# andreaskoepf/faster-rcnn.torch

Hardware: AMD Instinct MI355X
Metric: images/sec (vgg_small 800x450 fwd+bwd) (higher is better)
Workload: dtype f32 (conv / Linear(13824,1024) operands as 2 x fp16 split planes: 22 significand bits, 3 MFMA partial products; fp32 accumulate)

## Files before the change

### faster-rcnn.torch_amd/_lib.py

```python
import ctypes as C
import os

_HERE = os.path.dirname(os.path.abspath(__file__))
SO_PATH = os.environ.get("FRCNN_LIB_PATH") or os.path.join(_HERE, "libfrcnn_hip.so")

KC_NAMES = ["conv_igemm_k3", "conv_igemm_other", "conv_wgrad_k3", "conv_wgrad_other", "gemm", "elemwise",
            "roi", "rpn", "nms", "optim", "image", "conv_x3", "conv_wgradx", "topk"]


class FrcnnError(RuntimeError):
    pass


class ModelDesc(C.Structure):
    _fields_ = [
        ("nblocks", C.c_int),
        ("filters", C.c_int * 8), ("ksize", C.c_int * 8), ("pad", C.c_int * 8), ("conv_steps", C.c_int * 8),
        ("dropout", C.c_float * 8),
        ("nheads", C.c_int),
        ("head_k", C.c_int * 8), ("head_n", C.c_int * 8), ("head_input", C.c_int * 8),
        ("ncls", C.c_int),
        ("cls_n", C.c_int * 8), ("cls_bn", C.c_int * 8),
        ("cls_dropout", C.c_float * 8),
        ("class_count", C.c_int),
        ("kh", C.c_int), ("kw", C.c_int),
    ]


vp = C.c_void_p
_SIGS = {
    "frcnn_version": ([], C.c_int),
    "frcnn_set_option": ([C.c_char_p, C.c_int], C.c_int),
    "frcnn_get_option": ([C.c_char_p, C.POINTER(C.c_int)], C.c_int),
    "frcnn_last_error": ([], C.c_char_p),
    "frcnn_device_count": ([C.POINTER(C.c_int)], C.c_int),
    "frcnn_set_device": ([C.c_int], C.c_int),
    "frcnn_device_name": ([C.c_char_p, C.c_int], C.c_int),
    "frcnn_malloc": ([C.POINTER(vp), C.c_size_t], C.c_int),
    "frcnn_free": ([vp], C.c_int),
    "frcnn_host_alloc": ([C.POINTER(vp), C.c_size_t], C.c_int),
    "frcnn_host_free": ([vp], C.c_int),
    "frcnn_memcpy_h2d": ([vp, vp, C.c_size_t, vp], C.c_int),
    "frcnn_memcpy_d2h": ([vp, vp, C.c_size_t, vp], C.c_int),
    "frcnn_memcpy_d2d": ([vp, vp, C.c_size_t, vp], C.c_int),
    "frcnn_stream_sync": ([vp], C.c_int),
    "frcnn_zero": ([vp, C.c_size_t, vp], C.c_int),
    "frcnn_scale": ([vp, C.c_longlong, C.c_float, vp], C.c_int),
    "frcnn_add": ([vp, vp, C.c_longlong, vp], C.c_int),
    "frcnn_prof_enable": ([C.c_int], C.c_int),
    "frcnn_prof_collect": ([vp, vp, vp, vp], C.c_int),
    "frcnn_nms_workspace_bytes": ([C.c_int], C.c_size_t),
    "frcnn_nms_device": ([vp, C.c_int, C.c_int, C.c_float, C.c_int, C.c_int, vp, vp, vp, C.c_size_t, vp], C.c_int),
    "frcnn_nms_device_classes": ([vp, C.c_int, C.c_int, C.c_float, C.c_int, C.c_int, vp, vp, vp, vp, C.c_size_t, vp], C.c_int),
    "frcnn_nms_device_n": ([vp, C.c_int, vp, C.c_int, C.c_float, C.c_int, C.c_int, vp, vp, vp, vp, C.c_size_t, vp], C.c_int),
    "frcnn_nms_batch_workspace_bytes": ([C.c_int, C.c_int], C.c_size_t),
    "frcnn_nms_device_batch": ([vp, C.c_int, C.c_longlong, C.c_int, vp, C.c_int, C.c_float, C.c_int, C.c_int, vp, vp, vp, vp, C.c_size_t,
                               vp], C.c_int),
    "frcnn_topk_select_workspace_bytes": ([C.c_int, C.c_int], C.c_size_t),
    "frcnn_topk_select": ([vp, C.c_int, C.c_longlong, C.c_int, vp, C.c_int, vp, C.c_longlong, vp, vp, C.c_size_t, vp], C.c_int),
    "frcnn_rpn_gather_rows": ([vp, vp, vp, vp, C.c_int, C.c_longlong, C.c_int, vp, C.c_longlong, vp, C.c_int, vp, vp, vp, vp, vp, vp,
                              C.c_longlong, vp], C.c_int),
    "frcnn_detect_gather_batch": ([vp, vp, C.c_int, C.c_int, vp, vp, vp, vp, vp, C.c_longlong, vp, vp, vp, vp, vp], C.c_int),
    "frcnn_roi_windows": ([vp, vp, C.c_int, vp, C.c_int, C.c_int, C.c_int, vp, vp], C.c_int),
    "frcnn_detect_post": ([vp, vp, vp, vp, vp, C.c_int, C.c_int, C.c_double, vp, vp, vp, vp, vp, vp], C.c_int),
    "frcnn_detect_gather": ([vp, vp, C.c_int, vp, vp, vp, vp, vp, vp, vp, vp, vp, vp], C.c_int),
    "frcnn_nms_host": ([vp, C.c_int, C.c_int, C.c_float, C.c_int, C.c_int, vp, vp], C.c_int),
    "frcnn_conv2d_forward": ([vp, C.c_int, C.c_int, C.c_int, vp, vp, vp, vp, C.c_int, C.c_int, C.c_int, vp, vp], C.c_int),
    "frcnn_conv2d_backward_input": ([vp, C.c_int, C.c_int, C.c_int, vp, C.c_int, C.c_int, C.c_int, vp, C.c_int, vp], C.c_int),
    "frcnn_conv2d_backward_weight": ([vp, C.c_int, C.c_int, C.c_int, vp, vp, vp, C.c_int, C.c_int, C.c_int, vp, vp, vp], C.c_int),
    "frcnn_maxpool_act_forward": ([vp, C.c_int, C.c_int, C.c_int, vp, vp, vp, vp, vp], C.c_int),
    "frcnn_maxpool_act_backward": ([vp, vp, vp, C.c_int, C.c_int, C.c_int, vp, vp, vp, vp, vp, vp], C.c_int),
    "frcnn_act_forward": ([vp, C.c_int, C.c_longlong, vp, vp, vp, vp], C.c_int),
    "frcnn_act_backward": ([vp, vp, C.c_int, C.c_longlong, vp, vp, vp, vp, vp, vp], C.c_int),
    "frcnn_roi_pool_forward": ([vp, C.c_int, C.c_int, C.c_int, vp, C.c_int, C.c_int, C.c_int, vp, vp, vp], C.c_int),
    "frcnn_roi_pool_backward": ([vp, C.c_int, C.c_int, C.c_int, vp, vp, C.c_int, C.c_int, C.c_int, vp], C.c_int),
    "frcnn_roi_align_forward": ([vp, C.c_int, C.c_int, C.c_int, vp, vp, C.c_int, C.c_double, C.c_double, C.c_int, C.c_int, C.c_int, vp,
                                 vp], C.c_int),
    "frcnn_roi_align_backward": ([vp, C.c_int, C.c_int, C.c_int, vp, vp, vp, C.c_int, C.c_double, C.c_double, C.c_int, C.c_int, C.c_int,
                                  vp], C.c_int),
    "frcnn_rpn_scan_workspace_bytes": ([vp, vp], C.c_size_t),
    "frcnn_rpn_scan": ([vp, vp, vp, vp, vp, C.c_double, C.c_double, C.c_double, C.c_int, vp, vp, vp, vp, vp, vp, C.c_size_t, vp], C.c_int),
    "frcnn_rpn_scan_batch_workspace_bytes": ([vp, vp, C.c_int], C.c_size_t),
    "frcnn_rpn_scan_batch": ([vp, vp, vp, C.c_int, C.c_longlong, vp, vp, C.c_double, C.c_double, C.c_double, C.c_int, vp, vp, vp, vp, vp,
                             vp, C.c_size_t, vp], C.c_int),
    "frcnn_rpn_loss": ([vp, vp, vp, vp, vp, vp, vp, vp, C.c_int, C.c_int, C.c_int, vp, vp, vp, vp], C.c_int),
    "frcnn_loss_accumulate": ([vp, C.c_int, vp, vp], C.c_int),
    "frcnn_linear_forward": ([vp, C.c_int, C.c_int, vp, vp, C.c_int, vp, vp], C.c_int),
    "frcnn_linear_backward": ([vp, vp, C.c_int, C.c_int, vp, C.c_int, vp, vp, vp, vp], C.c_int),
    "frcnn_rmsprop": ([vp, vp, vp, C.c_longlong, C.c_float, C.c_float, C.c_float, vp], C.c_int),
    "frcnn_scale_rmsprop": ([vp, vp, C.c_float, vp, C.c_longlong, C.c_float, C.c_float, C.c_float, vp], C.c_int),
    "frcnn_scale_rmsprop_dev": ([vp, vp, vp, vp, C.c_longlong, C.c_float, C.c_float, C.c_float, vp], C.c_int),
    "frcnn_scale_rmsprop_slice": ([vp, vp, C.c_float, vp, C.c_longlong, C.c_longlong, C.c_float, C.c_float, C.c_float, vp], C.c_int),
    "frcnn_sgd": ([vp, vp, vp, C.c_longlong, C.c_float, vp, C.c_float, C.c_float, C.c_float, C.c_float, C.c_int, C.c_int, vp], C.c_int),
    "frcnn_sgd_slice": ([vp, vp, vp, C.c_longlong, C.c_longlong, C.c_float, C.c_float, C.c_float, C.c_float, C.c_float, C.c_int, C.c_int,
                         vp], C.c_int),
    "frcnn_nag": ([vp, vp, vp, C.c_longlong, C.c_float, vp, C.c_float, C.c_float, C.c_float, C.c_int, vp], C.c_int),
    "frcnn_nag_slice": ([vp, vp, vp, C.c_longlong, C.c_longlong, C.c_float, C.c_float, C.c_float, C.c_float, C.c_int, vp], C.c_int),
    "frcnn_scale_rmsprop_slice_dev": ([vp, vp, vp, vp, C.c_longlong, C.c_longlong, C.c_float, C.c_float, C.c_float, vp], C.c_int),
    "frcnn_sgd_slice_dev": ([vp, vp, vp, C.c_longlong, C.c_longlong, vp, C.c_float, C.c_float, C.c_float, C.c_float, C.c_int, C.c_int,
                            vp], C.c_int),
    "frcnn_nag_slice_dev": ([vp, vp, vp, C.c_longlong, C.c_longlong, vp, C.c_float, C.c_float, C.c_float, C.c_int, vp], C.c_int),
    "frcnn_grad_clip_workspace_bytes": ([C.c_longlong], C.c_size_t),
    "frcnn_grad_clip": ([vp, C.c_longlong, vp, C.c_int, C.c_double, vp, C.c_double, vp, vp, C.c_size_t, vp], C.c_int),
    "frcnn_nag_lookahead": ([vp, vp, C.c_longlong, C.c_float, vp], C.c_int),
    "frcnn_nag_lookahead_slice": ([vp, vp, C.c_longlong, C.c_longlong, C.c_float, vp], C.c_int),
    "frcnn_model_update_stream": ([vp, C.POINTER(vp)], C.c_int),
    "frcnn_model_update_fork": ([vp, vp], C.c_int),
    "frcnn_model_update_join": ([vp, vp], C.c_int),
    "frcnn_pnet_wait_backward_begun": ([vp, vp], C.c_int),
    "frcnn_pnet_wait_heads_done": ([vp, vp], C.c_int),
    "frcnn_pnet_wait_block_done": ([vp, C.c_int, vp], C.c_int),
    "frcnn_pnet_refresh_packs": ([vp, vp, C.c_int, vp], C.c_int),
    "frcnn_pnet_invalidate_packs": ([vp], C.c_int),
    "frcnn_model_create": ([C.POINTER(ModelDesc), C.POINTER(vp)], C.c_int),
    "frcnn_model_destroy": ([vp], C.c_int),
    "frcnn_model_param_count": ([vp, C.POINTER(C.c_longlong), C.POINTER(C.c_longlong)], C.c_int),
    "frcnn_model_param_table": ([vp, vp, C.c_int, C.POINTER(C.c_int)], C.c_int),
    "frcnn_model_localizer_layers": ([vp, C.c_int, vp, C.c_int, C.POINTER(C.c_int)], C.c_int),
    "frcnn_model_set_trainable": ([vp, C.c_int, C.c_int, C.c_int], C.c_int),
    "frcnn_model_get_trainable": ([vp, C.POINTER(C.c_int), C.POINTER(C.c_int), C.POINTER(C.c_int)], C.c_int),
    "frcnn_model_debug_buffer": ([vp, C.c_int, C.c_int, C.POINTER(vp), C.POINTER(C.c_longlong)], C.c_int),
    "frcnn_pnet_forward": ([vp, vp, vp, C.c_int, C.c_int, C.c_int, vp, C.c_ulonglong, vp], C.c_int),
    "frcnn_pnet_forward_async_heads": ([vp, vp, vp, C.c_int, C.c_int, vp, C.c_ulonglong, vp], C.c_int),
    "frcnn_pnet_output": ([vp, C.c_int, C.POINTER(vp), C.POINTER(C.c_int), C.POINTER(C.c_int), C.POINTER(C.c_int)], C.c_int),
    "frcnn_pnet_delta": ([vp, C.c_int, C.POINTER(vp)], C.c_int),
    "frcnn_pnet_set_sparse_deltas": ([vp, C.c_int, vp, C.c_int], C.c_int),
    "frcnn_pnet_zero_deltas": ([vp, vp], C.c_int),
    "frcnn_pnet_backward_heads_begin": ([vp, vp, vp, vp], C.c_int),
    "frcnn_pnet_anchor_loss_begin": ([vp, vp, vp, vp, vp, vp, vp, C.c_int, C.c_int, C.c_int, vp, vp, vp, vp, vp], C.c_int),
    "frcnn_pnet_anchor_loss_wait": ([vp, vp], C.c_int),
    "frcnn_pnet_backward_heads_join": ([vp, vp, C.POINTER(C.c_int)], C.c_int),
    "frcnn_pnet_backward": ([vp, vp, vp, vp], C.c_int),
    "frcnn_pnet_wait_block_gradients": ([vp, C.c_int, vp], C.c_int),
    "frcnn_cnet_forward": ([vp, vp, vp, C.c_int, C.c_int, vp, C.c_ulonglong, vp, vp, vp, vp], C.c_int),
    "frcnn_cnet_backward": ([vp, vp, vp, vp, vp, vp, vp], C.c_int),
    "frcnn_cnet_backward_join": ([vp, vp], C.c_int),
    "frcnn_cnet_losses": ([vp, vp, vp, vp, C.c_int, C.c_int, C.c_int, vp, vp, vp, vp], C.c_int),
    "frcnn_cnet_decode": ([vp, C.c_int, C.c_int, vp, vp, vp], C.c_int),
    "frcnn_anchors_create": ([vp, vp, vp, vp, C.c_int, C.c_int, C.POINTER(vp)], C.c_int),
    "frcnn_anchors_destroy": ([vp], C.c_int),
    "frcnn_anchors_assemble": ([vp, vp, C.c_int, C.c_double, C.c_double, C.c_double, C.c_double, C.c_int, C.c_int, C.c_int, vp,
                               C.POINTER(C.c_int), vp, vp, C.c_int, C.POINTER(C.c_int), C.POINTER(C.c_int)], C.c_int),
    "frcnn_comm_get_unique_id": ([vp], C.c_int),
    "frcnn_comm_exchange_id_file": ([C.c_char_p, C.c_int, vp, C.c_int], C.c_int),
    "frcnn_comm_init_rank": ([C.POINTER(vp), C.c_int, C.c_int, vp], C.c_int),
    "frcnn_comm_init_rank_timeout": ([C.POINTER(vp), C.c_int, C.c_int, vp, C.c_int], C.c_int),
    "frcnn_comm_init_rank_file": ([C.POINTER(vp), C.c_int, C.c_int, C.c_char_p, C.c_int], C.c_int),
    "frcnn_comm_destroy": ([vp], C.c_int),
    "frcnn_comm_info": ([vp, C.POINTER(C.c_int), C.POINTER(C.c_int)], C.c_int),
    "frcnn_comm_query": ([vp, C.POINTER(C.c_int), C.POINTER(C.c_int), C.POINTER(C.c_int)], C.c_int),
    "frcnn_allreduce_f32": ([vp, vp, C.c_longlong, vp], C.c_int),
    "frcnn_allreduce_f64": ([vp, vp, C.c_longlong, vp], C.c_int),
    "frcnn_broadcast_f32": ([vp, vp, C.c_longlong, C.c_int, vp], C.c_int),
    "frcnn_image_rgb2yuv": ([vp, vp, C.c_int, C.c_int, vp], C.c_int),
    "frcnn_image_rgb2hsv": ([vp, vp, C.c_int, C.c_int, vp], C.c_int),
    "frcnn_image_rgb2lab": ([vp, vp, C.c_int, C.c_int, vp], C.c_int),
    "frcnn_image_scale": ([vp, C.c_int, C.c_int, C.c_int, vp, C.c_int, C.c_int, vp, C.c_int, vp], C.c_int),
    "frcnn_image_scale_u8": ([vp, C.c_int, C.c_int, vp, C.c_int, C.c_int, vp, C.c_int, vp], C.c_int),
    "frcnn_image_crop_flip": ([vp, C.c_int, C.c_int, C.c_int, C.c_int, C.c_int, C.c_int, C.c_int, C.c_int, C.c_int, vp, vp], C.c_int),
    "frcnn_image_normalize_workspace_bytes": ([C.c_int], C.c_size_t),
    "frcnn_image_normalize": ([vp, C.c_int, C.c_int, C.c_int, C.c_int, C.c_int, vp, C.c_size_t, vp], C.c_int),
    "frcnn_image_contrastive_norm": ([vp, C.c_int, C.c_int, vp, C.c_int, C.c_float, vp, vp, vp], C.c_int),
}

_lib = None


def exported_symbols():
    return sorted(_SIGS.keys())


def load():
    global _lib
    if _lib is not None:
        return _lib
    if not os.path.exists(SO_PATH):
        raise FrcnnError(
            "libfrcnn_hip.so not found at %s -- build it with `python -c 'import __graft_entry__ as g; g.build()'` "
            "(there is no CPU fallback for the product path)" % SO_PATH)
    try:
        import torch
    except ImportError:
        pass
    L = C.CDLL(SO_PATH)
    for name, (args, res) in _SIGS.items():
        fn = getattr(L, name)
        fn.argtypes = args
        fn.restype = res
    _lib = L
    return L


def check(rc):
    if rc != 0:
        raise FrcnnError("libfrcnn_hip: %s (code %d)" % (load().frcnn_last_error().decode("utf-8", "replace"), rc))


def call(name, *args):
    check(getattr(load(), name)(*args))
```

### faster-rcnn.torch_amd/csrc/amax.h

```cpp
#pragma once
#include <hip/hip_runtime.h>

#include "kernels.h"

namespace frcnn {

__device__ __forceinline__ void amax_store_block(float m, float* rec) {
  __shared__ float amax_part[16];
#pragma unroll
  for (int o = 32; o > 0; o >>= 1) m = fmaxf(m, __shfl_xor(m, o));
  if ((threadIdx.x & 63) == 0) amax_part[threadIdx.x >> 6] = m;
  __syncthreads();
  if (threadIdx.x == 0) {
    const int nw = (blockDim.x + 63) >> 6;
    for (int i = 1; i < nw; ++i) m = fmaxf(m, amax_part[i]);
    rec[1 + blockIdx.x] = m;
    if (blockIdx.x == 0) rec[0] = __builtin_bit_cast(float, (int)gridDim.x);
  }
}

__device__ __forceinline__ float amax_load_block(const float* __restrict__ rec) {
  __shared__ float amax_all[16];
  const int n = __builtin_bit_cast(int, rec[0]);
  float m = 0.f;
  for (int i = threadIdx.x; i < n; i += blockDim.x) m = fmaxf(m, rec[1 + i]);
#pragma unroll
  for (int o = 32; o > 0; o >>= 1) m = fmaxf(m, __shfl_xor(m, o));
  if ((threadIdx.x & 63) == 0) amax_all[threadIdx.x >> 6] = m;
  __syncthreads();
  const int nw = (blockDim.x + 63) >> 6;
  m = amax_all[0];
  for (int i = 1; i < nw; ++i) m = fmaxf(m, amax_all[i]);
  __syncthreads();
  return m;
}

}
```

### faster-rcnn.torch_amd/csrc/api.cpp

```cpp
#include <cmath>
#include <cstring>
#include <vector>
#include <mutex>

#include "kernels.h"

namespace frcnn {

static thread_local std::string g_err;

void set_error(const char* fmt, ...) {
  char buf[1024];
  va_list ap;
  va_start(ap, fmt);
  vsnprintf(buf, sizeof(buf), fmt, ap);
  va_end(ap);
  g_err = buf;
}

struct ProfRec { int klass; double flops, bytes; hipEvent_t a, b; hipStream_t s; };
static hipEvent_t g_prof_base = nullptr;
static unsigned g_prof_mask = 0;
static std::vector<ProfRec> g_recs;
static std::vector<hipEvent_t> g_pool;
// ... 241 lines not shown
  (void)hipFree(wf);
  return rc;
}
int frcnn_conv2d_backward_input(const float* gout, int O, int Ho, int Wo, const float* weight, int C, int k,
                                int pad, float* gin, int accumulate, void* stream) {
  float* wd = nullptr;
  if (conv_x3_eligible(O, C, k)) {
    FR_HIP(hipMalloc((void**)&wd, conv_x3_pack_bytes(O, C, k)));
    float* am = nullptr;
    int rcx = x3_f16_records(&am);
    float* const amw = am ? am + AMAX_REC : nullptr;
    float* const aws = am ? am + 2 * AMAX_REC : nullptr;
    if (am && rcx == FRCNN_OK) {
      rcx = tensor_absmax(gout, (long)O * Ho * Wo, am, S(stream));
      if (rcx == FRCNN_OK) rcx = tensor_absmax(weight, (long)O * C * k * k, amw, S(stream));
    }
    if (rcx == FRCNN_OK) rcx = conv_x3_pack(weight, O, C, k, 1, wd, S(stream), Ho + 2 * (k - 1 - pad) - k + 1, Wo + 2 * (k - 1 - pad) - k + 1, amw, aws);
    if (rcx == FRCNN_OK) rcx = conv_x3(gout, O, Ho, Wo, nullptr, nullptr, wd, nullptr, C, k, k - 1 - pad, gin, accumulate ? OUT_ADD : OUT_STORE, 0, S(stream), 0, nullptr, am, aws);
    (void)hipStreamSynchronize(S(stream));
    (void)hipFree(wd); (void)hipFree(am);
    return rcx;
  }
  FR_HIP(hipMalloc((void**)&wd, conv_pack_floats(O, C, k) * 4));
  int rc = conv_pack_weights(weight, O, C, k, nullptr, wd, S(stream));
  if (rc == FRCNN_OK)
    rc = conv_igemm(gout, O, Ho, Wo, nullptr, nullptr, wd, nullptr, C, k, k - 1 - pad, gin,
                    accumulate ? OUT_ADD : OUT_STORE, 0, S(stream));
  (void)hipStreamSynchronize(S(stream));
  (void)hipFree(wd);
  return rc;
}
int frcnn_conv2d_backward_weight(const float* in, int C, int H, int W, const float* in_slope,
                                 const float* in_scale, const float* gout, int O, int k, int pad,
                                 float* gweight, float* gbias, void* stream) {
  size_t wsb = conv_wgrad_workspace_bytes(C, H, W, O, k, pad);
  void* ws = nullptr;
  FR_HIP(hipMalloc(&ws, wsb));
  int rc = FRCNN_OK;
  float* am = nullptr;
  bool unit = true;
  rc = scale_fits_f16_form(in_scale, C, S(stream), &unit);
  if (rc == FRCNN_OK && unit && k == 3 && conv_wgradx_eligible(C, O, k)) rc = x3_f16_records(&am);
  if (am && rc == FRCNN_OK) {
    rc = tensor_absmax(in, (long)C * H * W, am, S(stream));
    if (rc == FRCNN_OK) rc = tensor_absmax(gout, (long)O * (H + 2 * pad - k + 1) * (W + 2 * pad - k + 1), am + AMAX_REC, S(stream));
  }
  if (rc == FRCNN_OK)
    rc = conv_wgrad(in, C, H, W, in_slope, in_scale, gout, O, k, pad, gweight, ws, wsb, S(stream), nullptr, am, am ? am + AMAX_REC : nullptr);
  (void)hipStreamSynchronize(S(stream));
  (void)hipFree(ws); (void)hipFree(am);
  FR_TRY(rc);
  if (gbias) {
    int Ho = H + 2 * pad - k + 1, Wo = W + 2 * pad - k + 1;
    FR_TRY(channel_sum(gout, O, (long)Ho * Wo, gbias, S(stream)));
  }
  return FRCNN_OK;
}

int frcnn_maxpool_act_forward(const float* x, int C, int H, int W, const float* slope, const float* scale,
                              float* out, unsigned char* idx, void* stream) {
  return maxpool_act_forward(x, C, H, W, slope, scale, out, idx, S(stream));
}
int frcnn_maxpool_act_backward(const float* gpool, const unsigned char* idx, const float* x, int C, int H, int W,
                               const float* slope, const float* scale, float* gx, float* gbias, float* gslope,
                               void* stream) {
  return maxpool_act_backward(gpool, idx, x, C, H, W, slope, scale, gx, gbias, gslope, S(stream));
}
int frcnn_act_forward(const float* x, int C, long long hw, const float* slope, const float* scale, float* y,
                      void* stream) {
  return act_forward(x, C, hw, slope, scale, y, S(stream));
}
int frcnn_act_backward(const float* gy, const float* x, int C, long long hw, const float* slope,
                       const float* scale, float* gx, float* gbias, float* gslope, void* stream) {
  return act_backward(gy, x, C, hw, slope, scale, gx, gbias, gslope, S(stream));
}

int frcnn_roi_pool_forward(const float* fmap, int C, int H, int W, const int* wins, int R, int kh, int kw,
                           float* out, int* idx, void* stream) {
  return roi_pool_forward(fmap, C, H, W, wins, R, kh, kw, out, idx, S(stream));
}
int frcnn_roi_pool_backward(float* gmap, int C, int H, int W, const float* gout, const int* idx, int R, int kh,
                            int kw, void* stream) {
  return roi_pool_backward(gmap, C, H, W, gout, idx, R, kh, kw, S(stream));
}

static int roi_align_check(const char* who, const void* map, int C, int H, int W, const void* rows, const double* rect, int kh, int kw,
                           int g) {
  FR_CHECK(map && rows && rect, "%s: NULL argument", who);
  FR_CHECK(C >= 1 && H >= 1 && W >= 1 && kh >= 1 && kw >= 1, "%s: map %d x %d x %d, grid %d x %d", who, C, H, W, kh, kw);
  FR_CHECK((long)H * W < (1L << 31), "%s: a plane of %d x %d cells", who, H, W);
  FR_CHECK(g >= 1 && g <= 4, "%s: sampling ratio %d outside 1..4", who, g);
  return FRCNN_OK;
}
int frcnn_roi_align_forward(const float* fmap, int C, int H, int W, const double* rect, const long long* pick, int R, double inv_sx,
                            double inv_sy, int kh, int kw, int g, float* out, void* stream) {
  if (R <= 0) return FRCNN_OK;
  FR_TRY(roi_align_check("frcnn_roi_align_forward", fmap, C, H, W, out, rect, kh, kw, g));
  return roi_align_forward(fmap, C, H, W, rect, pick, R, inv_sx, inv_sy, kh, kw, g, out, S(stream));
}
int frcnn_roi_align_backward(float* gmap, int C, int H, int W, const float* gout, const double* rect, const long long* pick, int R,
                             double inv_sx, double inv_sy, int kh, int kw, int g, void* stream) {
  if (R <= 0) return FRCNN_OK;
  FR_TRY(roi_align_check("frcnn_roi_align_backward", gmap, C, H, W, gout, rect, kh, kw, g));
  return roi_align_backward(gmap, C, H, W, gout, rect, pick, R, inv_sx, inv_sy, kh, kw, g, S(stream));
}

static void to_layers(const float* const* maps, const int* H, const int* W, RpnLayers* L) {
  for (int l = 0; l < 4; ++l) { L->map[l] = maps ? maps[l] : nullptr; L->H[l] = H[l]; L->W[l] = W[l]; }
}
size_t frcnn_rpn_scan_workspace_bytes(const int* H, const int* W) {
  RpnLayers L;
  to_layers(nullptr, H, W, &L);
  return rpn_scan_workspace_bytes(L);
}
int frcnn_rpn_scan(const float* const* maps, const int* H, const int* W, const float* anchor_w,
                   const float* anchor_h, double img_w, double img_h, double p_threshold, int cap,
                   float* match_p, int* match_idx, double* match_rect, float* match_box, int* count,
                   void* ws, size_t ws_bytes, void* stream) {
  RpnLayers L;
  to_layers(maps, H, W, &L);
  return rpn_scan(L, anchor_w, anchor_h, img_w, img_h, p_threshold, cap, match_p, match_idx, match_rect,
                  match_box, count, ws, ws_bytes, S(stream));
}
size_t frcnn_rpn_scan_batch_workspace_bytes(const int* H, const int* W, int B) {
  RpnLayers L;
  to_layers(nullptr, H, W, &L);
  return rpn_scan_batch_workspace_bytes(L, B);
}
int frcnn_rpn_scan_batch(const float* const* maps, const int* H, const int* W, int B, long long slot_stride, const float* anchor_w,
                         const float* anchor_h, double img_w, double img_h, double p_threshold, int cap, float* match_p,
                         int* match_idx, double* match_rect, float* match_box, int* count, void* ws, size_t ws_bytes,
                         void* stream) {
  FR_CHECK(maps && H && W, "frcnn_rpn_scan_batch: NULL argument");
  RpnLayers L;
  to_layers(maps, H, W, &L);
  return rpn_scan_batch(L, B, (long)slot_stride, anchor_w, anchor_h, img_w, img_h, p_threshold, cap, match_p, match_idx,
                        match_rect, match_box, count, ws, ws_bytes, S(stream));
}
int frcnn_rpn_loss(const float* const* maps, float* const* deltas, const int* H, const int* W, const int* ex_idx,
                   const double* ex_anchor, const double* ex_roi, const int* ex_class, int npos, int nneg,
                   int bgclass, double* ex_loss, float* crtarget, float* cctarget, void* stream) {
  RpnLayers L;
  to_layers(maps, H, W, &L);
  return rpn_loss(L, deltas, ex_idx, ex_anchor, ex_roi, ex_class, npos, nneg, bgclass, ex_loss, crtarget,
                  cctarget, S(stream));
}

int frcnn_loss_accumulate(const double* ex_loss, int E, double* acc, void* stream) {
  return loss_accumulate(ex_loss, E, acc, S(stream));
}

int frcnn_linear_forward(const float* x, int R, int I, const float* weight, const float* bias, int O, float* y,
                         void* stream) {
  if (linear_x_eligible(1, R, I, O)) {
    void* xp = nullptr;
    FR_HIP(hipMalloc(&xp, (size_t)3 * R * I * 2));
    float* am = nullptr;
    int rc = x3_f16_records(&am);
    if (am && rc == FRCNN_OK) {
      rc = tensor_absmax(x, (long)R * I, am, S(stream));
      if (rc == FRCNN_OK) rc = tensor_absmax(weight, (long)O * I, am + AMAX_REC, S(stream));
    }
    if (rc == FRCNN_OK) rc = split_planes(x, R, I, xp, nullptr, S(stream), am);
    if (rc == FRCNN_OK) rc = linear_x_forward(xp, R, I, weight, bias, O, y, S(stream), 0, nullptr, am, am ? am + AMAX_REC : nullptr);
    (void)hipStreamSynchronize(S(stream));
    (void)hipFree(xp); (void)hipFree(am);
// ... 151 lines not shown
```

### faster-rcnn.torch_amd/csrc/cnet.hip

```cpp
#include "kernels.h"

namespace frcnn {

#define BN_EPS 1e-5
#define BN_MOM 0.1

#define BN_CB 16
#define BN_RG 64
template <int CB = BN_CB, int RG = BN_RG>
__device__ __forceinline__ double bn_reduce(double v, double* sh, int tx, int ty) {
  sh[ty * CB + tx] = v;
  __syncthreads();
  for (int stride = RG / 2; stride > 0; stride >>= 1) {
    if (ty < stride) sh[ty * CB + tx] += sh[(ty + stride) * CB + tx];
    __syncthreads();
  }
  const double s = sh[tx];
  __syncthreads();
  return s;
}
template <int NV>
__device__ __forceinline__ void fb_reduce(double (&v)[NV], double* sh, int tx, int ty) {
  const int tid = ty * 4 + tx, lane = tid & 63, wave = tid >> 6;
#pragma unroll
  for (int k = 0; k < NV; ++k) {
#pragma unroll
    for (int o = 4; o < 64; o <<= 1) v[k] += __shfl_xor(v[k], o, 64);
    if (lane < 4) sh[(k * 16 + wave) * 4 + lane] = v[k];
  }
  __syncthreads();
#pragma unroll
  for (int k = 0; k < NV; ++k) {
    double t = 0.0;
#pragma unroll
    for (int w = 0; w < 16; ++w) t += sh[(k * 16 + w) * 4 + tx];
    v[k] = t;
  }
  __syncthreads();
}
#define FB_CB 4
#define FB_RG 256
#define FB_KEEP 4

__global__ __launch_bounds__(1024) void bn_forward_kernel(const float* __restrict__ x, int R, int n,
                                                          const float* __restrict__ gamma, const float* __restrict__ beta,
                                                          float* running, int training, float* __restrict__ xhat,
                                                          float* __restrict__ invstd, float* __restrict__ y) {
  __shared__ double sh[BN_RG * BN_CB];
  const int tx = threadIdx.x, ty = threadIdx.y;
  const int j = blockIdx.x * BN_CB + tx;
  const bool ok = j < n;
  double mean, var;
  if (training) {
    double s = 0.0;
    if (ok) for (int r = ty; r < R; r += BN_RG) s += x[(size_t)r * n + j];
    mean = bn_reduce(s, sh, tx, ty) / R;
    double q = 0.0;
    if (ok) for (int r = ty; r < R; r += BN_RG) { double d = x[(size_t)r * n + j] - mean; q += d * d; }
    var = bn_reduce(q, sh, tx, ty);
    const double unb = R > 1 ? var / (R - 1) : var / R;
    var /= R;
    if (running && ok && ty == 0) {
      running[j] = (float)((1.0 - BN_MOM) * running[j] + BN_MOM * mean);
      running[n + j] = (float)((1.0 - BN_MOM) * running[n + j] + BN_MOM * unb);
    }
  } else {
    mean = ok ? running[j] : 0.0;
    var = ok ? running[n + j] : 1.0;
  }
  if (!ok) return;
  const double is = 1.0 / sqrt(var + BN_EPS);
  if (ty == 0) invstd[j] = (float)is;
  const double g = gamma[j], b = beta[j];
  for (int r = ty; r < R; r += BN_RG) {
    const double xh = (x[(size_t)r * n + j] - mean) * is;
    xhat[(size_t)r * n + j] = (float)xh;
    y[(size_t)r * n + j] = (float)(xh * g + b);
  }
}
int bn_forward(const float* x, int R, int n, const float* gamma, const float* beta, float* running,
               int training, float* xhat, float* invstd, float* y, hipStream_t s) {
  FR_CHECK(training || running, "bn_forward: evaluate mode needs running statistics");
  FR_LAUNCH(KC_ELEMWISE, 0, (double)R * n * 16.0, s, bn_forward_kernel, dim3(cdiv(n, BN_CB)), dim3(BN_CB, BN_RG), 0, x, R, n,
// ... 111 lines not shown
    }
    if (!ok) return;
    is = 1.0 / sqrt(var + BN_EPS);
    if (ty == 0) invstd[j] = (float)is;
    g = gamma[j]; b = beta[j];
  }
  if (!ok) return;
  const float a = *slope;
  auto emit = [&](size_t idx, float y) {
    if (bn) {
      const double xh = ((double)y - mean) * is;
      xhat[idx] = (float)xh;
      y = (float)(xh * g + b);
      pre[idx] = y;
    }
    y = y > 0.f ? y : a * y;
    if (GEN) {
      const float mk = frcnn_keep_mask(seed, (unsigned long long)idx, p);
      mask[idx] = mk;
      y = y * (mk * inv_keep);
    } else if (mask) {
      y = y * (mask[idx] * inv_keep);
    }
    post[idx] = y;
  };
  if (keep) {
#pragma unroll
    for (int i = 0; i < FB_KEEP; ++i)
      if (ty + i * FB_RG < R) emit((size_t)(ty + i * FB_RG) * n + j, xv[i]);
  } else {
    for (int r = ty; r < R; r += FB_RG) emit((size_t)r * n + j, v[(size_t)r * n + j]);
  }
}
template <bool GEN>
__global__ void cnet_act_forward_flat_kernel(const float* __restrict__ x, GemmFold src, long total, int n, float* __restrict__ lin,
                                             const float* slope, float* __restrict__ mask, float inv_keep, float p,
                                             unsigned long long seed, float* __restrict__ post) {
  const float a = *slope;
  for (long i = (long)blockIdx.x * blockDim.x + threadIdx.x; i < total; i += (long)gridDim.x * blockDim.x) {
    float y = fold_value(x, src, (size_t)total, (size_t)i, (int)(i % n));
    if (src.nSplit) lin[i] = y;
    y = y > 0.f ? y : a * y;
    if (GEN) {
      const float mk = frcnn_keep_mask(seed, (unsigned long long)i, p);
      mask[i] = mk;
      y = y * (mk * inv_keep);
    } else if (mask) {
      y = y * (mask[i] * inv_keep);
    }
    post[i] = y;
  }
}
int cnet_act_forward(const float* x, GemmFold src, int R, int n, const float* gamma, const float* beta, float* running,
                     int training, float* lin, float* xhat, float* invstd, float* pre, const float* slope, float* mask, bool gen,
                     float inv_keep, float p, unsigned long long seed, float* post, hipStream_t s) {
  FR_CHECK(!gamma || training || running, "cnet_act_forward: evaluate mode needs running statistics");
  if (!gamma) {
    const long total = (long)R * n;
    const int grid = (int)std::min<long>(std::max<long>(1, cdivl(total, 256)), 2048);
    if (gen)
      FR_LAUNCH(KC_ELEMWISE, 0, total * 16.0, s, cnet_act_forward_flat_kernel<true>, dim3(grid), dim3(256), 0, x, src, total, n, lin, slope,
                mask, inv_keep, p, seed, post);
    else
      FR_LAUNCH(KC_ELEMWISE, 0, total * 16.0, s, cnet_act_forward_flat_kernel<false>, dim3(grid), dim3(256), 0, x, src, total, n, lin, slope,
                mask, inv_keep, p, seed, post);
    FR_LAUNCH_CHECK();
    return FRCNN_OK;
  }
  if (gen)
    FR_LAUNCH(KC_ELEMWISE, 0, (double)R * n * 20.0, s, cnet_act_forward_kernel<true>, dim3(cdiv(n, FB_CB)), dim3(FB_CB, FB_RG), 0, x,
              src, R, n, gamma, beta, running, training, lin, xhat, invstd, pre, slope, mask, inv_keep, p, seed, post);
  else
    FR_LAUNCH(KC_ELEMWISE, 0, (double)R * n * 20.0, s, cnet_act_forward_kernel<false>, dim3(cdiv(n, FB_CB)), dim3(FB_CB, FB_RG), 0, x,
              src, R, n, gamma, beta, running, training, lin, xhat, invstd, pre, slope, mask, inv_keep, p, seed, post);
  FR_LAUNCH_CHECK();
  return FRCNN_OK;
}

__global__ __launch_bounds__(1024) void cnet_act_bn_backward_kernel(const float* __restrict__ gy, GemmFold src,
                                                                    const float* __restrict__ pre, const float* __restrict__ xhat,
                                                                    const float* __restrict__ invstd, const float* __restrict__ gamma,
                                                                    const float* slope, const float* __restrict__ mask, float inv_keep,
                                                                    int R, int n, int training, float* __restrict__ gx, float* ggamma,
                                                                    float* gbeta, float* gslope, float* part) {
  __shared__ double sh[FB_RG * FB_CB];
  __shared__ float shs[16];
  const int tx = threadIdx.x, ty = threadIdx.y;
  const int j = blockIdx.x * FB_CB + tx;
  const bool ok = j < n;
  const size_t total = (size_t)R * n;
  const float a = *slope;
  double sg = 0.0, sgx = 0.0;
  float sa = 0.f;
  const bool keep = R <= FB_RG * FB_KEEP;
  float tv[FB_KEEP], xh[FB_KEEP];
  auto first = [&](size_t idx, float& t, float& xhv) {
    float g = fold_value(gy, src, total, idx, j);
    if (mask) g = g * (mask[idx] * inv_keep);
    const float xv = pre[idx];
    t = g;
    if (!(xv > 0.f)) { t = a * g; sa += xv * g; }
    xhv = xhat[idx];
    sg += t;
    sgx += (double)t * xhv;
  };
  if (ok && keep) {
#pragma unroll
    for (int i = 0; i < FB_KEEP; ++i) {
      tv[i] = 0.f; xh[i] = 0.f;
      if (ty + i * FB_RG < R) first((size_t)(ty + i * FB_RG) * n + j, tv[i], xh[i]);
    }
  } else if (ok) {
    for (int r = ty; r < R; r += FB_RG) {
      const size_t idx = (size_t)r * n + j;
      float t, xhv;
      first(idx, t, xhv);
      gx[idx] = t;
    }
  }
  { double t[2] = {sg, sgx}; fb_reduce(t, sh, tx, ty); sg = t[0]; sgx = t[1]; }
  {
    const int tid = ty * FB_CB + tx;
#pragma unroll
    for (int o = 32; o > 0; o >>= 1) sa += __shfl_down(sa, o, 64);
    if ((tid & 63) == 0) shs[tid >> 6] = sa;
    __syncthreads();
    if (tid == 0) {
      float t = 0.f;
      for (int i = 0; i < 16; ++i) t += shs[i];
      if (part) part[blockIdx.x] = t; else unsafeAtomicAdd(gslope, t);
    }
  }
  if (!ok) return;
  if (ty == 0) {
    ggamma[j] = (float)((double)ggamma[j] + sgx);
    gbeta[j] = (float)((double)gbeta[j] + sg);
  }
  const double is = invstd[j], gm = gamma[j];
  auto second = [&](size_t idx, double g, double xhv) {
    const double v = training ? (g - sg / R - xhv * sgx / R) * gm * is : g * gm * is;
    gx[idx] = (float)v;
  };
  if (keep) {
#pragma unroll
    for (int i = 0; i < FB_KEEP; ++i)
      if (ty + i * FB_RG < R) second((size_t)(ty + i * FB_RG) * n + j, tv[i], xh[i]);
  } else {
    for (int r = ty; r < R; r += FB_RG) {
      const size_t idx = (size_t)r * n + j;
      second(idx, gx[idx], xhat[idx]);
    }
  }
}
__global__ void slope_fold_kernel(const float* __restrict__ part, int n, float* gslope);
int cnet_act_bn_backward(const float* gy, GemmFold src, const float* pre, const float* xhat, const float* invstd,
                         const float* gamma, const float* slope, const float* mask, float inv_keep, int R, int n, int training,
                         float* gx, float* ggamma, float* gbeta, float* gslope, hipStream_t s) {
  const int grid = cdiv(n, FB_CB);
  float* part = nullptr;
  if (deterministic()) FR_TRY(det_workspace(s, (size_t)grid, &part));
  FR_LAUNCH(KC_ELEMWISE, 0, (double)R * n * 28.0, s, cnet_act_bn_backward_kernel, dim3(grid), dim3(FB_CB, FB_RG), 0, gy, src, pre, xhat,
            invstd, gamma, slope, mask, inv_keep, R, n, training, gx, ggamma, gbeta, gslope, part);
  if (part) FR_LAUNCH(KC_ELEMWISE, 0, grid * 4.0, s, slope_fold_kernel, dim3(1), dim3(1), 0, (const float*)part, grid, gslope);
  FR_LAUNCH_CHECK();
  return FRCNN_OK;
}

template <bool GEN>
__global__ void prelu_dropout_forward_kernel(const float* __restrict__ x, long n, const float* slope,
                                             float* __restrict__ mask, float inv_keep, float p,
                                             unsigned long long seed, float* __restrict__ y) {
  const float a = *slope;
  for (long i = (long)blockIdx.x * blockDim.x + threadIdx.x; i < n; i += (long)gridDim.x * blockDim.x) {
    float v = x[i];
    v = v > 0.f ? v : a * v;
    if (GEN) {
      const float mk = frcnn_keep_mask(seed, (unsigned long long)i, p);
      mask[i] = mk;
      v = v * (mk * inv_keep);
    } else if (mask) {
      v = v * (mask[i] * inv_keep);
    }
    y[i] = v;
  }
}
int prelu_dropout_forward(const float* x, long n, const float* slope, const float* mask, float inv_keep,
                          float* y, hipStream_t s) {
  int grid = (int)std::min<long>(std::max<long>(1, cdivl(n, 256)), 1024);
  FR_LAUNCH(KC_ELEMWISE, 0, n * 12.0, s, prelu_dropout_forward_kernel<false>, dim3(grid), dim3(256), 0, x, n, slope,
            const_cast<float*>(mask), inv_keep, 0.f, 0ull, y);
  FR_LAUNCH_CHECK();
  return FRCNN_OK;
}
int prelu_dropout_forward_gen(const float* x, long n, const float* slope, float* mask_out, float p,
                              unsigned long long seed, float* y, hipStream_t s) {
  int grid = (int)std::min<long>(std::max<long>(1, cdivl(n, 256)), 1024);
  FR_LAUNCH(KC_ELEMWISE, 0, n * 12.0, s, prelu_dropout_forward_kernel<true>, dim3(grid), dim3(256), 0, x, n, slope,
            mask_out, 1.0f / (1.0f - p), p, seed, y);
  FR_LAUNCH_CHECK();
  return FRCNN_OK;
}

__global__ void prelu_dropout_backward_kernel(const float* __restrict__ gy, const float* __restrict__ x, long n,
                                              const float* slope, const float* __restrict__ mask,
                                              float inv_keep, float* __restrict__ gx, float* gslope, float* part) {
  __shared__ float sh[4];
  const float a = *slope;
  float sa = 0.f;
  for (long i = (long)blockIdx.x * blockDim.x + threadIdx.x; i < n; i += (long)gridDim.x * blockDim.x) {
    float g = gy[i];
    if (mask) g = g * (mask[i] * inv_keep);
    const float xv = x[i];
    float r = g;
    if (!(xv > 0.f)) { r = a * g; sa += xv * g; }
    gx[i] = r;
  }
#pragma unroll
  for (int o = 32; o > 0; o >>= 1) sa += __shfl_down(sa, o, 64);
  if ((threadIdx.x & 63) == 0) sh[threadIdx.x >> 6] = sa;
  __syncthreads();
  if (threadIdx.x == 0) {
    const float t = sh[0] + sh[1] + sh[2] + sh[3];
    if (part) part[blockIdx.x] = t;
    else unsafeAtomicAdd(gslope, t);
  }
}
__global__ void slope_fold_kernel(const float* __restrict__ part, int n, float* gslope) {
  float v = 0.f;
  for (int i = 0; i < n; ++i) v += part[i];
  *gslope += v;
}
int prelu_dropout_backward(const float* gy, const float* x, long n, const float* slope,
                           const float* mask, float inv_keep, float* gx, float* gslope, hipStream_t s) {
  int grid = (int)std::min<long>(std::max<long>(1, cdivl(n, 256)), 256);
  float* part = nullptr;
  if (deterministic()) FR_TRY(det_workspace(s, (size_t)grid, &part));
  FR_LAUNCH(KC_ELEMWISE, 0, n * 16.0, s, prelu_dropout_backward_kernel, dim3(grid), dim3(256), 0, gy, x, n,
            slope, mask, inv_keep, gx, gslope, part);
  if (part) FR_LAUNCH(KC_ELEMWISE, 0, grid * 4.0, s, slope_fold_kernel, dim3(1), dim3(1), 0, (const float*)part, grid, gslope);
  FR_LAUNCH_CHECK();
  return FRCNN_OK;
}

__device__ __forceinline__ double wave_sum_f64(double v) {
#pragma unroll
  for (int o = 32; o > 0; o >>= 1) v += __shfl_xor(v, o, 64);
  return v;
}
__device__ __forceinline__ double wave_max_f64(double v) {
#pragma unroll
  for (int o = 32; o > 0; o >>= 1) { const double w = __shfl_xor(v, o, 64); v = w > v ? w : v; }
  return v;
}
__global__ void log_softmax_rows_fold_kernel(float* __restrict__ x, GemmFold src, int R, int n, float* __restrict__ y,
                                             float* __restrict__ y2) {
  const int r = blockIdx.x * (blockDim.x >> 6) + (threadIdx.x >> 6), lane = threadIdx.x & 63;
  if (r >= R) return;
  float* xr = x + (size_t)r * n;
  const size_t total = (size_t)R * n;
  if (src.nSplit)
    for (int i = lane; i < n; i += 64) xr[i] = fold_value(x, src, total, (size_t)r * n + i, i);
  double m = -1.0e300;
  for (int i = lane; i < n; i += 64) m = xr[i] > m ? (double)xr[i] : m;
  m = wave_max_f64(m);
  double s = 0.0;
  for (int i = lane; i < n; i += 64) s += exp((double)xr[i] - m);
  s = wave_sum_f64(s);
  const double lse = m + log(s);
  for (int i = lane; i < n; i += 64) {
    const float v = (float)((double)xr[i] - lse);
    y[(size_t)r * n + i] = v;
    if (y2) y2[(size_t)r * n + i] = v;
  }
}
int log_softmax_rows_fold(const float* x, GemmFold src, int R, int n, float* y, float* y2, hipStream_t s) {
  if (R <= 0) return FRCNN_OK;
  FR_LAUNCH(KC_ELEMWISE, 0, (double)R * n * 8.0, s, log_softmax_rows_fold_kernel, dim3(cdiv(R, 4)), dim3(256), 0, const_cast<float*>(x),
            src, R, n, y, y2);
  FR_LAUNCH_CHECK();
  return FRCNN_OK;
}

__global__ void log_softmax_rows_kernel(const float* __restrict__ x, int R, int n, float* __restrict__ y) {
  const int r = blockIdx.x * (blockDim.x >> 6) + (threadIdx.x >> 6), lane = threadIdx.x & 63;
  if (r >= R) return;
  const float* xr = x + (size_t)r * n;
  double m = -1.0e300;
  for (int i = lane; i < n; i += 64) m = xr[i] > m ? (double)xr[i] : m;
  m = wave_max_f64(m);
  double s = 0.0;
  for (int i = lane; i < n; i += 64) s += exp((double)xr[i] - m);
  s = wave_sum_f64(s);
  const double lse = m + log(s);
  for (int i = lane; i < n; i += 64) y[(size_t)r * n + i] = (float)((double)xr[i] - lse);
}
int log_softmax_rows(const float* x, int R, int n, float* y, hipStream_t s) {
  if (R <= 0) return FRCNN_OK;
  FR_LAUNCH(KC_ELEMWISE, 0, (double)R * n * 8.0, s, log_softmax_rows_kernel, dim3(cdiv(R, 4)), dim3(256), 0, x, R,
            n, y);
  FR_LAUNCH_CHECK();
  return FRCNN_OK;
}

#define HEADS_PITCH 33
__global__ __launch_bounds__(256) void cnet_heads_forward_kernel(const float* __restrict__ x, int R, int nf, const float* __restrict__ Wb,
                                                                 const float* __restrict__ bb, const float* __restrict__ Wc,
                                                                 const float* __restrict__ bc, int nc, float* __restrict__ bbox_out,
                                                                 float* __restrict__ logits, float* __restrict__ lsm,
                                                                 float* __restrict__ cls_out) {
  extern __shared__ float wt[];
  float* xs = wt + (size_t)nf * HEADS_PITCH + (threadIdx.x >> 6) * nf;
  const int no = 4 + nc;
  for (int k = threadIdx.x; k < nf; k += 256) {
    float* d = wt + k * HEADS_PITCH;
#pragma unroll
    for (int n = 0; n < 4; ++n) d[n] = Wb[(size_t)n * nf + k];
#pragma unroll 8
    for (int n = 0; n < nc; ++n) d[4 + n] = Wc[(size_t)n * nf + k];
  }
  __syncthreads();
  const int lane = threadIdx.x & 63, n = lane & 31, h = lane >> 5;
  const bool isb = n < 4, isc = n >= 4 && n < no;
  const int nn = n < no ? n : 0, kh = nf / 2;
  for (int r = blockIdx.x * 4 + (threadIdx.x >> 6); r < R; r += gridDim.x * 4) {
    for (int k = lane * 4; k < nf; k += 256) *reinterpret_cast<float4*>(xs + k) = *reinterpret_cast<const float4*>(x + (size_t)r * nf + k);
    __builtin_amdgcn_wave_barrier();
    const float* xr = xs + h * kh;
    const float* wk = wt + (size_t)(h * kh) * HEADS_PITCH + nn;
    float a0 = 0.f, a1 = 0.f, a2 = 0.f, a3 = 0.f;
#pragma unroll 4
    for (int k = 0; k < kh; k += 4) {
      const float4 xv = *reinterpret_cast<const float4*>(xr + k);
      a0 = fmaf(xv.x, wk[(k + 0) * HEADS_PITCH], a0); a1 = fmaf(xv.y, wk[(k + 1) * HEADS_PITCH], a1);
      a2 = fmaf(xv.z, wk[(k + 2) * HEADS_PITCH], a2); a3 = fmaf(xv.w, wk[(k + 3) * HEADS_PITCH], a3);
    }
    float v = (a0 + a1) + (a2 + a3);
    v += __shfl_xor(v, 32, 64);
    v += isb ? bb[n] : isc ? bc[n - 4] : 0.f;
    if (isb && h == 0) bbox_out[(size_t)r * 4 + n] = v;
    const bool mine = isc && h == 0;
    double m = mine ? (double)v : -1.0e300;
    m = wave_max_f64(m);
    double e = mine ? exp((double)v - m) : 0.0;
    e = wave_sum_f64(e);
    const double lse = m + log(e);
    if (mine) {
      const size_t o = (size_t)r * nc + n - 4;
      const float l = (float)((double)v - lse);
      logits[o] = v; lsm[o] = l;
      if (cls_out) cls_out[o] = l;
    }
  }
}
__global__ __launch_bounds__(256) void cnet_heads_backward_kernel(const float* __restrict__ g_bbox, const float* __restrict__ g_cls,
                                                                  const float* __restrict__ lsm, int R, int nf,
                                                                  const float* __restrict__ Wb, const float* __restrict__ Wc, int nc,
                                                                  float* __restrict__ glog, float* __restrict__ gfeat, HeadsPostAct post) {
  extern __shared__ float wt[];
  __shared__ float shs[4];
  const float pa = post.pre ? *post.slope : 1.f;
  float sa = 0.f;
  const int no = 4 + nc;
  for (int k = threadIdx.x; k < nf; k += 256) {
#pragma unroll
    for (int n = 0; n < 4; ++n) wt[n * nf + k] = Wb[(size_t)n * nf + k];
#pragma unroll 8
    for (int n = 0; n < nc; ++n) wt[(4 + n) * nf + k] = Wc[(size_t)n * nf + k];
  }
  __syncthreads();
  const int lane = threadIdx.x & 63, wave = threadIdx.x >> 6;
  float* sg = wt + (size_t)no * nf + wave * 64;
  const bool isb = lane < 4, isc = lane >= 4 && lane < no;
  for (int r = blockIdx.x * 4 + wave; r < R; r += gridDim.x * 4) {
    const size_t o = (size_t)r * nc + (isc ? lane - 4 : 0);
    const double gy = isc ? (double)g_cls[o] : 0.0;
    const double sum = wave_sum_f64(gy);
    float g = 0.f;
    if (isc) {
      g = (float)(gy - exp((double)lsm[o]) * sum);
      glog[o] = g;
    } else if (isb) {
      g = g_bbox[(size_t)r * 4 + lane];
    }
    sg[lane] = g;
    __builtin_amdgcn_wave_barrier();
    for (int k = lane; k < nf; k += 64) {
      float a0 = 0.f, a1 = 0.f;
      int n = 0;
      for (; n + 2 <= no; n += 2) {
        a0 = fmaf(sg[n], wt[n * nf + k], a0);
        a1 = fmaf(sg[n + 1], wt[(n + 1) * nf + k], a1);
      }
      if (n < no) a0 = fmaf(sg[n], wt[n * nf + k], a0);
      float g = a0 + a1;
      if (post.pre) {
        const size_t idx = (size_t)r * nf + k;
        if (post.mask) g = g * (post.mask[idx] * post.inv_keep);
        const float xv = post.pre[idx];
        if (!(xv > 0.f)) { sa += xv * g; g = pa * g; }
      }
      gfeat[(size_t)r * nf + k] = g;
    }
    __builtin_amdgcn_wave_barrier();
  }
  if (post.pre) {
#pragma unroll
    for (int o = 32; o > 0; o >>= 1) sa += __shfl_down(sa, o, 64);
    if (lane == 0) shs[wave] = sa;
    __syncthreads();
    if (threadIdx.x == 0) unsafeAtomicAdd(post.gslope, (shs[0] + shs[1]) + (shs[2] + shs[3]));
  }
}
bool cnet_heads_fused_eligible(int nf, int nc) { return 4 + nc <= 32 && nf % 8 == 0 && nf <= 1024; }
int cnet_heads_forward(const float* x, int R, int nf, const float* Wb, const float* bb, const float* Wc, const float* bc, int nc,
                       float* bbox_out, float* logits, float* lsm, float* cls_out, hipStream_t s) {
  if (R <= 0) return FRCNN_OK;
  FR_CHECK(cnet_heads_fused_eligible(nf, nc), "cnet_heads_forward: %d classes", nc);
  FR_CHECK(((uintptr_t)x & 15) == 0, "cnet_heads_forward: input alignment");
  const size_t lds = ((size_t)nf * HEADS_PITCH + 4 * (size_t)nf) * 4;
  static bool attr_set = false;
  if (!attr_set) {
    FR_HIP(hipFuncSetAttribute(reinterpret_cast<const void*>(cnet_heads_forward_kernel), hipFuncAttributeMaxDynamicSharedMemorySize, 160 * 1024));
    attr_set = true;
  }
  FR_LAUNCH(KC_ELEMWISE, 0, (double)R * nf * 4.0, s, cnet_heads_forward_kernel, dim3(std::min(cdiv(R, 4), 256)), dim3(256), lds, x, R, nf, Wb,
            bb, Wc, bc, nc, bbox_out, logits, lsm, cls_out);
  FR_LAUNCH_CHECK();
  return FRCNN_OK;
}
int cnet_heads_backward(const float* g_bbox, const float* g_cls, const float* lsm, int R, int nf, const float* Wb, const float* Wc,
                        int nc, float* glog, float* gfeat, hipStream_t s, const HeadsPostAct* post) {
  if (R <= 0) return FRCNN_OK;
  FR_CHECK(cnet_heads_fused_eligible(nf, nc), "cnet_heads_backward: %d classes", nc);
  const size_t lds = ((size_t)(4 + nc) * nf + 256) * 4;
  static size_t attr_lds = 0;
  if (lds > attr_lds) {
    FR_HIP(hipFuncSetAttribute(reinterpret_cast<const void*>(cnet_heads_backward_kernel), hipFuncAttributeMaxDynamicSharedMemorySize, (int)lds));
    attr_lds = lds;
  }
  FR_LAUNCH(KC_ELEMWISE, 0, (double)R * nf * 4.0, s, cnet_heads_backward_kernel, dim3(std::min(cdiv(R, 4), 256)), dim3(256), lds, g_bbox, g_cls,
            lsm, R, nf, Wb, Wc, nc, glog, gfeat, post ? *post : HeadsPostAct{});
  FR_LAUNCH_CHECK();
  return FRCNN_OK;
}

__global__ void log_softmax_backward_kernel(const float* __restrict__ gy, const float* __restrict__ lsm, int R,
                                            int n, float* __restrict__ gx) {
  const int r = blockIdx.x * (blockDim.x >> 6) + (threadIdx.x >> 6), lane = threadIdx.x & 63;
  if (r >= R) return;
  double sum = 0.0;
  for (int i = lane; i < n; i += 64) sum += gy[(size_t)r * n + i];
  sum = wave_sum_f64(sum);
  for (int i = lane; i < n; i += 64)
    gx[(size_t)r * n + i] = (float)((double)gy[(size_t)r * n + i] - exp((double)lsm[(size_t)r * n + i]) * sum);
}
int log_softmax_backward(const float* gy, const float* lsm, int R, int n, float* gx, hipStream_t s) {
  if (R <= 0) return FRCNN_OK;
  FR_LAUNCH(KC_ELEMWISE, 0, (double)R * n * 12.0, s, log_softmax_backward_kernel, dim3(cdiv(R, 4)), dim3(256), 0,
            gy, lsm, R, n, gx);
  FR_LAUNCH_CHECK();
  return FRCNN_OK;
}

__global__ void cnet_losses_kernel(float* __restrict__ crout, const float* __restrict__ crtarget,
                                   const float* __restrict__ ccout, const float* __restrict__ cctarget, int R,
                                   int npos, int ncls, float* __restrict__ crdelta, float* __restrict__ ccdelta,
                                   double* loss2) {
  __shared__ double shr[256], shc[256];
  double sr = 0.0, sc = 0.0;
  for (int i = threadIdx.x; i < R * 4; i += blockDim.x) {
    float v = crout[i];
    if (i >= npos * 4) { v = 0.f; crout[i] = 0.f; }
    const float z = v - crtarget[i];
    const float az = fabsf(z);
    sr += az < 1.0f ? 0.5 * (double)z * (double)z : (double)az - 0.5;
    crdelta[i] = (az < 1.0f ? z : (z > 0.f ? 1.0f : -1.0f)) * 10.0f;
  }
  for (int i = threadIdx.x; i < R * ncls; i += blockDim.x) ccdelta[i] = 0.f;
  __syncthreads();
  for (int r = threadIdx.x; r < R; r += blockDim.x) {
    const int t = (int)cctarget[r] - 1;
    sc -= (double)ccout[(size_t)r * ncls + t];
    ccdelta[(size_t)r * ncls + t] = (float)(-1.0 / R);
  }
  shr[threadIdx.x] = sr;
  shc[threadIdx.x] = sc;
  __syncthreads();
// ... 38 lines not shown
```

### faster-rcnn.torch_amd/csrc/kernels.h

```cpp
#pragma once
#include <algorithm>

#include "common.h"

namespace frcnn {

int conv_cc(int k);
int conv_mpad(int M);
size_t conv_pack_floats(int Kchan, int M, int k);
int conv_pack_weights(const float* w, int O, int C, int k, float* wf, float* wd, hipStream_t s);
struct PackJob { long w_off; long total; float* dst; int O, C, k, mode, Mpad, blk_begin, nblk; };
PackJob conv_pack_job(long w_off, int O, int C, int k, int mode, float* dst);
int conv_pack_assign_blocks(PackJob* jobs, int njobs, int total_blocks);
int conv_pack_weights_multi(const float* weights, const PackJob* jobs_dev, int njobs, int grid, hipStream_t s);

enum { OUT_STORE = 0, OUT_ADD = 1 };
struct IgemmPool { float* out; unsigned char* idx; const float* slope; const float* scale; float* amax = nullptr; };
int conv_igemm(const float* in, int Cin, int H, int W, const float* in_slope, const float* in_scale,
               const float* wp, const float* bias, int M, int k, int pad, float* out, int out_mode,
               double algo_flops, hipStream_t s, int ws_slot = 0,
               const IgemmPool* pool = nullptr, bool* pool_fused = nullptr);

void set_split_bf16(int on);
int get_split_bf16();
// ... 63 lines not shown
int maxpool_act_backward(const float* gpool, const unsigned char* idx, const float* x, int C, int H,
                         int W, const float* slope, const float* scale, float* gx, float* gbias,
                         float* gslope, hipStream_t s, float* amax = nullptr);
int act_backward(const float* gy, const float* x, int C, long hw, const float* slope,
                 const float* scale, float* gx, float* gbias, float* gslope, hipStream_t s, float* amax = nullptr);
int channel_sum(const float* g, int C, long hw, float* gbias, hipStream_t s);
int channel_sum_cols(const float* g, int R, int O, float* gb, hipStream_t s);
int gather_positions(const float* src, int C, long hw, const int* pos, int P, float* dst, const float* slope,
                     float* dst_act, hipStream_t s);
int im2col_positions(const float* X, int C, int H, int W, int k, int Wo, const int* pos, int P, float* col, hipStream_t s);
int col2im_positions_add(const float* col, int C, int H, int W, int k, int Wo, const int* pos, int P, float* gX,
                         hipStream_t s);
int dropout_channel_mask(float* scale, int C, float p, unsigned long long seed, hipStream_t s);
int fill_value(float* x, long n, float v, hipStream_t s);
int rmsprop_step(float* x, float* g, float* m, long n, float lr, float alpha, float eps, float gscale,
                 bool scale_first, hipStream_t s, const double* gcount_dev = nullptr);
int rmsprop_slice(float* x, float* g, float* m, long lo, long hi, float lr, float alpha, float eps, float gscale, bool scale_first,
                  hipStream_t s, const double* gcount_dev = nullptr);
int sgd_update(float* x, float* g, float* v, long lo, long hi, bool slice, float gscale, const double* gcount_dev, float clr,
               float wd, float mom, float one_minus_damp, bool nesterov, bool first, hipStream_t s);
int nag_update(float* x, float* g, float* v, long lo, long hi, bool slice, float gscale, const double* gcount_dev, float clr,
               float wd, float mom, bool first, hipStream_t s);
int nag_lookahead(float* x, const float* v, long n, float mom, hipStream_t s);
constexpr int GRAD_CLIP_MAX_RANGES = 16;
size_t grad_clip_workspace_bytes(long n);
int grad_clip(float* g, long n, const long long* ranges_host, int nranges, double divisor, const double* divisor_dev, double clip_norm,
              double* record, void* workspace, size_t workspace_bytes, hipStream_t s);
int nag_lookahead_slice(float* x, const float* v, long lo, long hi, float mom, hipStream_t s);

#define FRCNN_HEAD_OUT 18
struct HeadJob {
  int Cin, H, W, k, Ho, Wo, n;
  int P; const int* pos;
  const float* in; float* gin;
  const float *bias3, *slope, *bias1;
  float *gbias3, *gslope, *gbias1;
  float* out; const float* delta;
  float *COL, *HX, *HY, *OUT, *D, *GH, *DX;
  const float* hx_slab; int hx_splits;
};
struct HeadJobs { HeadJob j[4]; int n; };
int heads_im2col(const HeadJobs& g, hipStream_t s);
int heads_bias_act(const HeadJobs& g, hipStream_t s);
int heads_scatter(const HeadJobs& g, hipStream_t s);
int heads_gather_delta(const HeadJobs& g, hipStream_t s);
int heads_act_backward(const HeadJobs& g, hipStream_t s);
int heads_col2im(const HeadJobs& g, hipStream_t s);

struct GemmFold;
#define GEMM_GROUP_MAX 4
struct GemmJob {
  const float* A; long sAm, sAk; const float* B; long sBk, sBn; float* C; long ldc;
  int M, N, K, out_mode;
  int splits = 1;
  int kPerSplit = 0;
};
int gemm_f32_group(GemmJob* jobs, int n, hipStream_t s);
int gemm_f32(const float* A, long sAm, long sAk, const float* B, long sBk, long sBn, float* C,
             long ldc, int M, int N, int K, int out_mode, const float* bias_n, hipStream_t s, int ws_slot = 0,
             GemmFold* defer = nullptr);
int gemm_workspace_get(size_t need, float** out, int slot);
struct GemmFold {
  const float* slab = nullptr;
  int nSplit = 0;
  const float* bias = nullptr;
};
int gemm_reduce_slabs(const float* slab, int nSplit, int M, int N, const float* bias, float* C, long ldc, bool accumulate,
                      hipStream_t s);
void set_gemm_x_roles(int mask);
int get_gemm_x_roles();
bool linear_x_eligible(int role, int R, int I, int O);
int linear_x_rows_padded(int R);
int split_planes(const float* src, int R, int C, void* P , void* PT ,
                 hipStream_t s, const float* amax = nullptr);
int linear_x_forward(const void* Xp, int R, int I, const float* W, const float* bias, int O, float* y, hipStream_t s, int ws_slot = 0,
                     GemmFold* defer = nullptr, const float* amax_x = nullptr, const float* amax_w = nullptr);
int linear_x_dgrad(const void* Gp, int R, int O, const float* W, int I, float* gx, int out_mode, hipStream_t s, int ws_slot = 0,
                   GemmFold* defer = nullptr, const float* amax_g = nullptr, const float* amax_w = nullptr);
int linear_x_wgrad(const void* GpT, const void* XpT, int R, int O, int I, float* gw, hipStream_t s, int ws_slot = 0,
                   const float* amax_g = nullptr, const float* amax_x = nullptr);


int roi_pool_forward(const float* fmap, int C, int H, int W, const int* wins, int R, int kh, int kw,
                     float* out, int* idx, hipStream_t s);
int roi_pool_backward(float* gmap, int C, int H, int W, const float* gout, const int* idx, int R,
                      int kh, int kw, hipStream_t s);

int roi_align_forward(const float* fmap, int C, int H, int W, const double* rect, const long long* pick, int R, double inv_sx,
                      double inv_sy, int kh, int kw, int g, float* out, hipStream_t s);
int roi_align_backward(float* gmap, int C, int H, int W, const float* gout, const double* rect, const long long* pick, int R,
                       double inv_sx, double inv_sy, int kh, int kw, int g, hipStream_t s);

struct RpnLayers {
  const float* map[4];
  int H[4], W[4];
};
int rpn_scan(const RpnLayers& L, const float* anchor_w, const float* anchor_h, double img_w,
             double img_h, double p_threshold, int cap, float* match_p, int* match_idx,
             double* match_rect, float* match_box, int* count, void* ws, size_t ws_bytes,
             hipStream_t s);
size_t rpn_scan_workspace_bytes(const RpnLayers& L);
int rpn_scan_batch(const RpnLayers& L, int B, long slot_stride, const float* anchor_w, const float* anchor_h, double img_w,
                   double img_h, double p_threshold, int cap, float* match_p, int* match_idx, double* match_rect,
                   float* match_box, int* count, void* ws, size_t ws_bytes, hipStream_t s);
size_t rpn_scan_batch_workspace_bytes(const RpnLayers& L, int B);
int rpn_loss(const RpnLayers& L, float* const* delta, const int* ex_idx, const double* ex_anchor,
             const double* ex_roi, const int* ex_class, int npos, int nneg, int bgclass,
             double* ex_loss, float* crtarget, float* cctarget, hipStream_t s);

int loss_accumulate(const double* ex_loss, int E, double* acc, hipStream_t s);

size_t nms_workspace_bytes(int n);
int nms_device(const float* boxes, int n, int ncols, float overlap, int key_mode, int key_col,
               long long* pick, int* count, void* ws, size_t ws_bytes, hipStream_t s, const int* cls = nullptr,
               const int* n_dev = nullptr);
size_t nms_batch_workspace_bytes(int B, int n);
int nms_device_batch(const float* boxes, int B, long row_stride, int n, const int* n_dev, int ncols, float overlap, int key_mode,
                     int key_col, const int* cls, long long* pick, int* count, void* ws, size_t ws_bytes, hipStream_t s);
size_t topk_select_workspace_bytes(int B, int n_cap);
int topk_select(const float* score, int B, long stride, int n_cap, const int* n_dev, int K, int* sel_row, long sel_stride,
                int* k_dev, void* ws, size_t ws_bytes, hipStream_t s);
int rpn_gather_rows(const float* p, const int* idx, const double* rect, const float* box, int B, long src_stride, int src_rows,
                    const int* sel_row, long sel_stride, const int* k_dev, int k_cap, float* dst_p, int* dst_idx,
                    double* dst_rect, float* dst_box, float* box5, int* row, long dst_stride, hipStream_t s);
int roi_windows(const double* rect, const long long* pick, int k, const int* layers, int nlayers, int fmH, int fmW, int* wins,
                hipStream_t s);
int detect_post(const int* cls, const float* conf, const float* bbox, const double* rect, const long long* pick, int R,
                int bgclass, double min_conf, float* bb, int* kc, int* keep_row, double* r2, int* K_dev, hipStream_t s);
int detect_gather(const long long* wpick, const int* nwin_dev, int cap, const int* keep_row, const int* kc, const float* bb,
                  const double* r2, const long long* pick, const float* mp, const double* rect, const int* midx, double* rec,
                  hipStream_t s);
int detect_gather_batch(const long long* wpick, const int* counts, int B, int row_stride, const int* keep_row, const int* kc,
                        const float* bb, const double* r2, const long long* pick, long match_stride, const float* mp,
                        const double* rect, const int* midx, double* rec, hipStream_t s);

int bn_forward(const float* x, int R, int n, const float* gamma, const float* beta, float* running,
               int training, float* xhat, float* invstd, float* y, hipStream_t s);
int bn_backward(const float* gy, const float* xhat, const float* invstd, const float* gamma, int R,
                int n, int training, float* gx, float* ggamma, float* gbeta, hipStream_t s);
int prelu_dropout_forward(const float* x, long n, const float* slope, const float* mask, float inv_keep,
                          float* y, hipStream_t s);
int prelu_dropout_forward_gen(const float* x, long n, const float* slope, float* mask_out, float p,
                              unsigned long long seed, float* y, hipStream_t s);
int prelu_dropout_backward(const float* gy, const float* x, long n, const float* slope,
                           const float* mask, float inv_keep, float* gx, float* gslope, hipStream_t s);
int cnet_act_forward(const float* x, GemmFold src, int R, int n, const float* gamma, const float* beta, float* running,
                     int training, float* lin, float* xhat, float* invstd, float* pre, const float* slope, float* mask, bool gen,
                     float inv_keep, float p, unsigned long long seed, float* post, hipStream_t s);
int cnet_act_bn_backward(const float* gy, GemmFold src, const float* pre, const float* xhat, const float* invstd,
                         const float* gamma, const float* slope, const float* mask, float inv_keep, int R, int n, int training,
                         float* gx, float* ggamma, float* gbeta, float* gslope, hipStream_t s);
bool cnet_heads_fused_eligible(int nf, int nc);
int cnet_heads_forward(const float* x, int R, int nf, const float* Wb, const float* bb, const float* Wc, const float* bc, int nc,
                       float* bbox_out, float* logits, float* lsm, float* cls_out, hipStream_t s);
struct HeadsPostAct {
  const float* pre = nullptr;
  const float* mask = nullptr;
  float inv_keep = 1.f;
  const float* slope = nullptr;
  float* gslope = nullptr;
};
int cnet_heads_backward(const float* g_bbox, const float* g_cls, const float* lsm, int R, int nf, const float* Wb, const float* Wc,
                        int nc, float* glog, float* gfeat, hipStream_t s, const HeadsPostAct* post = nullptr);
int log_softmax_rows_fold(const float* x, GemmFold src, int R, int n, float* y, float* y2, hipStream_t s);
int dropout_mask(float* mask, long n, float p, unsigned long long seed, hipStream_t s);
struct DropoutJobs { float* ptr[8]; int C[8]; float p[8]; unsigned long long seed[8]; int n; };
int dropout_channel_masks(const DropoutJobs& j, hipStream_t s);
int log_softmax_rows(const float* x, int R, int n, float* y, hipStream_t s);
int cnet_losses(float* crout, const float* crtarget, const float* ccout, const float* cctarget, int R,
                int npos, int ncls, float* crdelta, float* ccdelta, double* loss2, hipStream_t s);
int log_softmax_backward(const float* gy, const float* lsm, int R, int n, float* gx, hipStream_t s);
int cnet_decode(const float* cls_lsm, int R, int ncls, int* cls_out, float* conf_out, hipStream_t s);

int image_rgb2yuv(const float* rgb, float* yuv, int H, int W, hipStream_t s);
int image_rgb2hsv(const float* rgb, float* hsv, int H, int W, hipStream_t s);
int image_rgb2lab(const float* rgb, float* lab, int H, int W, hipStream_t s);
int image_scale(const float* src, int C, int H, int W, float* dst, int dH, int dW, float* tmp, int rgb2yuv,
                hipStream_t s);
int image_scale_u8(const unsigned char* src_hwc, int H, int W, float* dst, int dH, int dW, float* tmp, int rgb2yuv,
                   hipStream_t s);
int image_crop_flip(const float* src, int C, int H, int W, int x0, int y0, int w, int h, int hflip, int vflip,
                    float* dst, hipStream_t s);
size_t image_normalize_workspace_bytes(int C);
int image_normalize(float* img, int C, int H, int W, int centering, int scaling, void* ws, size_t ws_bytes,
                    hipStream_t s);
int image_contrastive_norm(const float* in, int H, int W, const float* kernel_host, int K, float threshold, float* out,
                           float* tmp, hipStream_t s);

}
```

### faster-rcnn.torch_amd/csrc/net.cpp

```cpp
#include <array>
#include <vector>
#include <cmath>
#include <cstring>

#include "kernels.h"

namespace frcnn {

static const int HEAD_OUT = 18;
static const int SPARSE_MAX_POS = 512;

struct DevBuf {
  void* p = nullptr;
  size_t bytes = 0;
  bool owned = true;
  void view(void* ptr, size_t n) { p = ptr; bytes = n; owned = false; }
  int ensure(size_t need) {
    if (need <= bytes) return FRCNN_OK;
    if (p && owned) (void)hipFree(p);
    owned = true;
    p = nullptr; bytes = 0;
    FR_HIP(hipMalloc(&p, need + 64));
    bytes = need;
    return FRCNN_OK;
// ... 72 lines not shown
  if (!pool[slot]) FR_HIP(hipStreamCreateWithFlags(&pool[slot], hipStreamNonBlocking));
  *out = pool[slot];
  return FRCNN_OK;
}

static int g_sparse_heads = -1;
static int sparse_heads_on() {
  if (g_sparse_heads < 0) g_sparse_heads = getenv("FRCNN_SPARSE_HEADS") ? (atoi(getenv("FRCNN_SPARSE_HEADS")) != 0) : 1;
  return g_sparse_heads;
}
static int g_static_weights = 0;
static long g_static_gen = 0;

struct frcnn_model {
  frcnn_model_desc d;
  std::vector<Conv> convs;
  std::vector<Block> blocks;
  std::vector<Head> heads;
  std::vector<ClsLayer> cls;
  long pnet_params = 0, total_params = 0;
  long bbox_w_off = 0, bbox_b_off = 0, clsw_off = 0, clsb_off = 0;
  int H = 0, W = 0;
  int training = 0;
  DevBuf delta_last;
  DevBuf zero_arena;
  size_t delta_bytes = 0, gpool_bytes = 0;
  DevBuf pack_jobs;
  DevBuf x3_jobs;
  DevBuf amax, amax_ws, amax_jobs;
  int n_amax = 0, n_amax_jobs = 0, amax_grid = 0;
  float* rec(int id) const { return (float*)amax.p + (size_t)id * AMAX_REC; }
  bool f16_packed = false;
  long eval_packs_gen = -1;
  const float* eval_packs_w = nullptr;
  int n_x3_all = 0, n_x3_fwd = 0, x3_grid_all = 0, x3_grid_fwd = 0;
  int n_pack_fwd = 0, n_pack_all = 0, n_pack_heads = 0, pack_grid_fwd = 0, pack_grid_all = 0, pack_grid_heads = 0;
  bool head_packs_fresh = false;
  struct PackGroup { int pk_off = 0, pk_n = 0, pk_grid = 0, am_off = 0, am_n = 0, am_grid = 0, x3_off = 0, x3_off16 = 0, x3_n = 0, x3_grid = 0; };
  std::vector<PackGroup> groups;
  unsigned fresh_mask = 0;
  const float* fresh_w = nullptr;
  bool fresh_f16 = false;
  static const int DC_RING = 4;
  char* dc_pin = nullptr; DevBuf dc_dev; size_t dc_slot_bytes = 0, dc_idx_off = 0; unsigned dc_step = 0;
  hipEvent_t dc_ev[DC_RING] = {};
  std::vector<PackXJob> x3_host, x3_host16;
  std::vector<int> x3_conv;
  DevBuf dbg_expand;
  std::vector<hipEvent_t> block_rd_ev;
  hipStream_t side = nullptr;
  hipStream_t cw = nullptr;
  hipEvent_t cw_fork = nullptr, cw_done = nullptr;
  bool cw_pending = false;
  std::vector<hipEvent_t> cw_ev;
  std::vector<hipEvent_t> fork_ev;
  hipEvent_t join_ev = nullptr;
  bool update_armed = false;
  hipEvent_t bwd_ev = nullptr;
  hipEvent_t upd_ev = nullptr, upd_join_ev = nullptr;
  bool head_x3_fresh = true;
  int am_bb_off = 0, am_bb_n = 0, am_bb_grid = 0;
  int pk_bb_off = 0, pk_bb_n = 0, pk_bb_grid = 0;
  bool heads_deferred = false;
  bool heads_sparse_fwd = false;
  const float* last_w = nullptr;
  hipEvent_t heads_gin_ev = nullptr;
  bool heads_gin = false;
  bool heads_begun = false;
  bool heads_joined = false;
  bool side_busy = false;
  hipEvent_t loss_ev = nullptr;
  hipEvent_t chain_ev = nullptr;
  std::vector<hipEvent_t> block_ev;
  bool block_ev_valid = false;
  bool loss_pending = false;
  DevBuf wg_ws;
  DevBuf wg_ws_first;
  DevBuf img;
  int frozen_blocks = 0;
  int train_heads = 1, train_cnet = 1;
  int R = 0, D = 0;
  const float* cnet_x = nullptr;
  DevBuf feat_g, logits, lsm, glog, gtmp;
  std::vector<std::array<long long, 4>> table;
};

static int pool_out(int n) { return (n - 2 + 1) / 2 + 1; }
static int refresh_group(frcnn_model* m, const float* w, int group, hipStream_t s);

static void build_layout(frcnn_model* m) {
  const frcnn_model_desc& d = m->d;
  long off = 0;
  int cin = 3;
  for (int b = 0; b < d.nblocks; ++b) {
    Block blk;
    blk.first_conv = (int)m->convs.size();
    blk.nconv = d.conv_steps[b];
    blk.has_drop = d.dropout[b] > 0.f;
    blk.p_drop = d.dropout[b];
    for (int s = 0; s < d.conv_steps[b]; ++s) {
      Conv c;
      c.Cin = cin; c.Cout = d.filters[b]; c.k = d.ksize[b]; c.pad = d.pad[b];
      c.block = b; c.step = s;
      long wsz = (long)c.Cout * c.Cin * c.k * c.k;
      c.w_off = off; c.b_off = off + wsz; c.a_off = off + wsz + c.Cout;
      m->table.push_back({c.w_off, wsz, 0, (long long)c.k * c.k * c.Cout});
      m->table.push_back({c.b_off, c.Cout, 1, 0});
      m->table.push_back({c.a_off, 1, 2, 0});
      off += wsz + c.Cout + 1;
      cin = c.Cout;
      m->convs.push_back(std::move(c));
    }
    m->blocks.push_back(std::move(blk));
  }
  for (int h = 0; h < d.nheads; ++h) {
    Head hd;
    hd.input = d.head_input[h] - 1;
    Conv& a = hd.c3;
    a.Cin = d.filters[hd.input]; a.Cout = d.head_n[h]; a.k = d.head_k[h]; a.pad = 0;
    a.block = -1; a.step = 0;
    long wsz = (long)a.Cout * a.Cin * a.k * a.k;
    a.w_off = off; a.b_off = off + wsz; a.a_off = off + wsz + a.Cout;
    m->table.push_back({a.w_off, wsz, 0, (long long)a.k * a.k * a.Cout});
    m->table.push_back({a.b_off, a.Cout, 1, 0});
    m->table.push_back({a.a_off, 1, 2, 0});
    off += wsz + a.Cout + 1;
    Conv& c = hd.c1;
    c.Cin = a.Cout; c.Cout = HEAD_OUT; c.k = 1; c.pad = 0; c.block = -1; c.step = 1;
    long w1 = (long)HEAD_OUT * c.Cin;
    c.w_off = off; c.b_off = off + w1; c.a_off = -1;
    m->table.push_back({c.w_off, w1, 0, (long long)HEAD_OUT});
    m->table.push_back({c.b_off, HEAD_OUT, 1, 0});
    off += w1 + HEAD_OUT;
    m->heads.push_back(std::move(hd));
  }
  m->pnet_params = off;
  int in = d.kh * d.kw * d.filters[d.nblocks - 1];
  m->D = in;
  for (int l = 0; l < d.ncls; ++l) {
    ClsLayer L;
    L.in = in; L.n = d.cls_n[l]; L.bn = d.cls_bn[l] != 0; L.p_drop = d.cls_dropout[l];
    L.w_off = off; L.b_off = off + (long)in * L.n;
    m->table.push_back({L.w_off, (long long)in * L.n, 3, in});
    m->table.push_back({L.b_off, L.n, 4, in});
    off += (long)in * L.n + L.n;
    L.bnw_off = L.bnb_off = -1;
    if (L.bn) {
      L.bnw_off = off; L.bnb_off = off + L.n;
      m->table.push_back({L.bnw_off, L.n, 5, 0});
      m->table.push_back({L.bnb_off, L.n, 6, 0});
      off += 2L * L.n;
    }
    L.a_off = off;
    m->table.push_back({L.a_off, 1, 2, 0});
    off += 1;
    in = L.n;
    m->cls.push_back(std::move(L));
  }
  m->bbox_w_off = off; m->bbox_b_off = off + (long)in * 4;
  m->table.push_back({m->bbox_w_off, (long long)in * 4, 3, in});
  m->table.push_back({m->bbox_b_off, 4, 4, in});
  off += (long)in * 4 + 4;
  int nc = d.class_count + 1;
  m->clsw_off = off; m->clsb_off = off + (long)in * nc;
  m->table.push_back({m->clsw_off, (long long)in * nc, 3, in});
  m->table.push_back({m->clsb_off, nc, 4, in});
// ... 745 lines not shown
    int heavy = -1;
    for (size_t i = 0; i < m->heads.size(); ++i)
      if ((!use_side || m->heads[i].input == last) && (heavy < 0 || m->heads[i].c3.k > m->heads[heavy].c3.k)) heavy = (int)i;
    if (async_heads) heavy = -1;
    if (use_side) FR_TRY(ensure_side(m));
    for (size_t i = 0; use_side && i < m->heads.size(); ++i) {
      if (m->heads[i].input != last || (int)i == heavy) continue;
      FR_TRY(fork_to(m, s, head_stream(m, i), 16 + i));
      FR_TRY(head_forward(m, m->heads[i], w, head_stream(m, i), head_slot(m, i)));
    }
    for (size_t i = 0; i < m->heads.size(); ++i)
      if ((int)i == heavy || (!use_side)) FR_TRY(head_forward(m, m->heads[i], w, s, 0));
  }
  if (use_side && !async_heads) FR_TRY(join_side(m, s));
  return FRCNN_OK;
}

int frcnn_pnet_forward(frcnn_model* m, const float* w, const float* img, int H, int W, int training,
                       const float* const* drop_masks, unsigned long long seed, void* stream) {
  return pnet_forward_impl(m, w, img, H, W, training, drop_masks, seed, stream, false);
}

int frcnn_pnet_forward_async_heads(frcnn_model* m, const float* w, const float* img, int H, int W,
                                   const float* const* drop_masks, unsigned long long seed, void* stream) {
  return pnet_forward_impl(m, w, img, H, W, 1, drop_masks, seed, stream, true);
}

int frcnn_pnet_output(frcnn_model* m, int i, float** ptr, int* C, int* H, int* W) {
  FR_CHECK(m->H > 0, "pnet_output: call frcnn_pnet_forward first");
  FR_CHECK(i >= 1 && i <= (int)m->heads.size() + 1, "pnet_output: index %d out of range", i);
  if (i <= (int)m->heads.size()) {
    Head& h = m->heads[i - 1];
    *ptr = h.c1.x.f(); *C = HEAD_OUT; *H = h.c1.Ho; *W = h.c1.Wo;
  } else {
    Block& b = m->blocks.back();
    *ptr = b.pooled.f(); *C = m->d.filters[m->d.nblocks - 1]; *H = b.Hp; *W = b.Wp;
  }
  return FRCNN_OK;
}

int frcnn_model_debug_buffer(frcnn_model* m, int kind, int index, void** ptr, long long* bytes) {
  FR_CHECK(m && ptr && bytes, "frcnn_model_debug_buffer: NULL argument");
  const DevBuf* b = nullptr;
  size_t n = 0;
  switch (kind) {
    case 0: {
      FR_CHECK(index >= 0 && index < (int)m->convs.size() && m->H > 0, "debug_buffer: backbone convolution %d (after a forward pass)", index);
      const Conv& c = m->convs[index]; b = &c.x; n = (size_t)c.Cout * c.Ho * c.Wo * 4;
      const Block& k = m->blocks[c.block];
      if (k.dc_on && c.step == 0) {
        FR_HIP(hipDeviceSynchronize());
        FR_TRY(m->dbg_expand.ensure(n));
        FR_HIP(hipMemset(m->dbg_expand.p, 0, n));
        std::vector<int> idx(c.Cout);
        FR_HIP(hipMemcpy(idx.data(), k.dc_idx, (size_t)c.Cout * 4, hipMemcpyDeviceToHost));
        const size_t row = (size_t)c.Ho * c.Wo * 4;
        for (int i = 0; i < k.nk; ++i)
          FR_HIP(hipMemcpy((char*)m->dbg_expand.p + (size_t)idx[i] * row, (const char*)c.x.p + (size_t)i * row, row, hipMemcpyDeviceToDevice));
        b = &m->dbg_expand;
      }
    } break;
    case 4: {
      FR_CHECK(index >= 0 && index < (int)m->blocks.size() && m->H > 0 && m->blocks[index].has_drop, "debug_buffer: block %d has no dropout", index);
      const Block& k = m->blocks[index]; b = &k.scale; n = (size_t)m->d.filters[index] * 4;
    } break;
    case 1: {
      FR_CHECK(index >= 0 && index < (int)m->blocks.size() && m->H > 0, "debug_buffer: block %d (after a forward pass)", index);
      const Block& k = m->blocks[index]; b = &k.pidx; n = (size_t)m->d.filters[index] * k.Hp * k.Wp;
    } break;
    case 2: {
      FR_CHECK(index >= 0 && index < (int)m->heads.size() && m->H > 0, "debug_buffer: anchor net %d (after a forward pass)", index);
      const Conv& c = m->heads[index].c3; b = &c.x; n = (size_t)c.Cout * c.Ho * c.Wo * 4;
      if ((m->heads_sparse_fwd || m->heads_deferred) && m->last_w) {
        FR_HIP(hipDeviceSynchronize());
        if (!m->head_x3_fresh) { FR_TRY(refresh_group(m, m->last_w, (int)m->blocks.size(), nullptr)); m->head_x3_fresh = true; }
        FR_TRY(head_forward(m, m->heads[index], m->last_w, nullptr, 0));
        FR_HIP(hipDeviceSynchronize());
      }
    } break;
    case 3: {
      FR_CHECK(index >= 0 && index < (int)m->cls.size() && m->R > 0, "debug_buffer: classification layer %d (after frcnn_cnet_forward)", index);
      const ClsLayer& L = m->cls[index]; b = L.bn ? &L.pre : &L.lin; n = (size_t)m->R * L.n * 4;
    } break;
    default: FR_CHECK(false, "debug_buffer: unknown kind %d", kind);
  }
  FR_CHECK(b->p && b->bytes >= n, "debug_buffer: buffer not allocated yet");
  *ptr = b->p; *bytes = (long long)n;
  return FRCNN_OK;
}

int frcnn_pnet_delta(frcnn_model* m, int i, float** ptr) {
  FR_CHECK(m->H > 0, "pnet_delta: call frcnn_pnet_forward first");
  FR_CHECK(i >= 1 && i <= (int)m->heads.size() + 1, "pnet_delta: index %d out of range", i);
  *ptr = i <= (int)m->heads.size() ? m->heads[i - 1].delta.f() : m->delta_last.f();
  return FRCNN_OK;
}

int frcnn_pnet_set_sparse_deltas(frcnn_model* m, int head, const int* positions, int count) {
  FR_CHECK(head >= 1 && head <= (int)m->heads.size(), "pnet_set_sparse_deltas: head %d out of range", head);
  m->heads[head - 1].sp_pos = positions;
  m->heads[head - 1].sp_count = count;
  return FRCNN_OK;
}

int frcnn_pnet_zero_deltas(frcnn_model* m, void* stream) {
  FR_CHECK(m->H > 0, "pnet_zero_deltas: call frcnn_pnet_forward first");
  FR_TRY(fill_zero(m->zero_arena.p, m->delta_bytes, S(stream)));
  return FRCNN_OK;
}

static bool head_is_sparse(const Head& h) { return h.sp_count >= 0 && h.sp_count <= SPARSE_MAX_POS; }
static bool head_needs_gin(const frcnn_model* m, const Head& h) { return h.input >= m->frozen_blocks; }
static bool backbone_trained(const frcnn_model* m) { return m->frozen_blocks < (int)m->blocks.size(); }

static int backward_head(frcnn_model* m, Head& h, const float* w, float* grad, hipStream_t s, int ws_slot) {
  Block& in = m->blocks[h.input];
  Conv &a = h.c3, &c = h.c1;
  const long hw1 = (long)c.Ho * c.Wo;
  if (head_is_sparse(h)) {
    const int P = h.sp_count;
    const int* pos = h.sp_pos;
    h.sp_count = -1; h.sp_pos = nullptr;
    if (P == 0) return FRCNN_OK;
    const int n = a.Cout, ckk = a.Cin * a.k * a.k;
    FR_TRY(h.spD.ensure((size_t)HEAD_OUT * SPARSE_MAX_POS * 4));
    FR_TRY(h.spHX.ensure((size_t)n * SPARSE_MAX_POS * 4));
    FR_TRY(h.spHY.ensure((size_t)n * SPARSE_MAX_POS * 4));
    FR_TRY(h.spGH.ensure((size_t)n * SPARSE_MAX_POS * 4));
    FR_TRY(h.spCol.ensure((size_t)ckk * SPARSE_MAX_POS * 4));
    FR_TRY(h.spDX.ensure((size_t)ckk * SPARSE_MAX_POS * 4));
    float *D = h.spD.f(), *HX = h.spHX.f(), *HY = h.spHY.f(), *GH = h.spGH.f(), *COL = h.spCol.f(), *DX = h.spDX.f();
    FR_TRY(gather_positions(h.delta.f(), HEAD_OUT, hw1, pos, P, D, nullptr, nullptr, s));
    FR_TRY(gather_positions(a.x.f(), n, hw1, pos, P, HX, w + a.a_off, HY, s));
    FR_TRY(gemm_f32(w + c.w_off, 1, n, D, P, 1, GH, P, n, P, HEAD_OUT, OUT_STORE, nullptr, s, ws_slot));
    FR_TRY(act_backward(GH, HX, n, P, w + a.a_off, nullptr, GH, grad + a.b_off, grad + a.a_off, s));
    if (head_needs_gin(m, h)) {
      FR_TRY(gemm_f32(GH, 1, P, w + a.w_off, ckk, 1, DX, ckk, P, ckk, n, OUT_STORE, nullptr, s, ws_slot));
      FR_TRY(col2im_positions_add(DX, a.Cin, a.H, a.W, a.k, a.Wo, pos, P, in.gpooled.f(), s));
    }
    if (h.stream && s == h.stream) {
      if (!h.gin_done) FR_HIP(hipEventCreateWithFlags(&h.gin_done, hipEventDisableTiming));
      FR_HIP(hipEventRecord(h.gin_done, s));
      h.gin_recorded = true;
    }
    FR_TRY(gemm_f32(D, P, 1, HY, 1, P, grad + c.w_off, n, HEAD_OUT, n, P, OUT_ADD, nullptr, s, ws_slot));
    FR_TRY(channel_sum(D, HEAD_OUT, P, grad + c.b_off, s));
    FR_TRY(im2col_positions(in.pooled.f(), a.Cin, a.H, a.W, a.k, a.Wo, pos, P, COL, s));
    FR_TRY(gemm_f32(GH, P, 1, COL, ckk, 1, grad + a.w_off, ckk, n, ckk, P, OUT_ADD, nullptr, s, ws_slot));
    return FRCNN_OK;
  }
  h.sp_count = -1; h.sp_pos = nullptr;
  if (!m->head_packs_fresh) {
    FR_TRY(conv_pack_weights_multi(w, (const PackJob*)m->pack_jobs.p + m->n_pack_all + m->n_pack_fwd, m->n_pack_heads,
                                   m->pack_grid_heads, s));
    m->head_packs_fresh = true;
  }
  FR_TRY(conv_wgrad(a.x.f(), c.Cin, c.H, c.W, w + a.a_off, nullptr, h.delta.f(), HEAD_OUT, 1, 0, grad + c.w_off, m->wg_ws.p, m->wg_ws.bytes, s));
  FR_TRY(channel_sum(h.delta.f(), HEAD_OUT, hw1, grad + c.b_off, s));
  double f1 = 2.0 * HEAD_OUT * c.Cin * (double)hw1;
  FR_TRY(conv_igemm(h.delta.f(), HEAD_OUT, c.Ho, c.Wo, nullptr, nullptr, c.wd.f(), nullptr, c.Cin, 1, 0, a.gx.f(),
                    OUT_STORE, f1, s, ws_slot));
  FR_TRY(act_backward(a.gx.f(), a.x.f(), a.Cout, (long)a.Ho * a.Wo, w + a.a_off, nullptr, a.gx.f(),
                      grad + a.b_off, grad + a.a_off, s));
  FR_TRY(conv_wgrad(in.pooled.f(), a.Cin, a.H, a.W, nullptr, nullptr, a.gx.f(), a.Cout, a.k, 0, grad + a.w_off, m->wg_ws.p, m->wg_ws.bytes, s));
  if (!head_needs_gin(m, h)) return FRCNN_OK;
  double f3 = 2.0 * a.Cout * a.Cin * a.k * a.k * (double)a.Ho * a.Wo;
// ... 439 lines not shown
        FR_HIP(hipStreamWaitEvent(s, m->join_ev, 0));
      } else {
        FR_TRY(conv_wgrad(in, wg_cin, c.H, c.W, in_slope, in_scale, c.gx.f(), wg_o, c.k, c.pad, grad + c.w_off, m->wg_ws.p, m->wg_ws.bytes, ws,
                          fused_here ? grad + c.b_off : nullptr, wa_in, wa_g, dc ? &wmap : nullptr));
      }
      if (st == 0) {
        while (m->block_ev.size() < (size_t)nb) {
          hipEvent_t e;
          FR_HIP(hipEventCreateWithFlags(&e, hipEventDisableTiming));
          m->block_ev.push_back(e);
        }
        FR_HIP(hipEventRecord(m->block_ev[b], on_caller ? s : ws));
      }
      if (b == fb && st == 0) {
        FR_TRY(record_block_read(m, b, s));
        break;
      }
      float* gin = st > 0 ? m->convs[blk.first_conv + st - 1].gx.f() : m->blocks[b - 1].gpooled.f();
      const int gmode = st > 0 ? OUT_STORE : OUT_ADD;
      const float* ag = nullptr;
      const float* aw = nullptr;
      if (c.x_d && m->f16_packed) { ag = m->rec(c.am + 1); aw = m->amax_ws.f() + c.am; }
      const int dg_k = (dc && st == 0) ? blk.nkK : c.Cout, dg_m = (dc && st == 1) ? blk.nkM : c.Cin;
      const double fl = 2.0 * dg_k * dg_m * c.k * c.k * (double)c.Ho * c.Wo;
      if (c.x_d && st > 0 && fuse_act && c.k == 3) {
        Conv& pc = m->convs[blk.first_conv + st - 1];
        X3PostAct post{pc.x.f(), w + pc.a_off, (st - 1 == 0 && blk.has_drop && !dc) ? blk.scale.f() : nullptr, grad + pc.a_off};
        FR_TRY(conv_x3(c.gx.f(), dg_k, c.Ho, c.Wo, nullptr, nullptr, c.wxd.p, nullptr, dg_m, c.k, c.k - 1 - c.pad, gin, gmode, fl, s, 0, &post, ag, aw,
                       (pc.x_d && m->f16_packed) ? m->rec(pc.am + 1) : nullptr));
        act_done = true;
      } else if (c.x_d)
        FR_TRY(conv_x3(c.gx.f(), dg_k, c.Ho, c.Wo, nullptr, nullptr, c.wxd.p, nullptr, dg_m, c.k, c.k - 1 - c.pad, gin, gmode, fl, s, 0, nullptr, ag, aw));
      else
        FR_TRY(conv_igemm(c.gx.f(), c.Cout, c.Ho, c.Wo, nullptr, nullptr, c.wd.f(), nullptr, c.Cin, c.k,
                          c.k - 1 - c.pad, gin, gmode, fl, s));
      if (st == 0) FR_TRY(record_block_read(m, b, s));
    }
  }
  m->block_ev_valid = true;
  if (heads_tail && !m->heads_gin) FR_TRY(join_heads(m, s));
  FR_TRY(cw_join(m, s));
  if (use_side) {
    FR_HIP(hipEventRecord(m->join_ev, ws));
    FR_HIP(hipStreamWaitEvent(s, m->join_ev, 0));
    m->side_busy = false;
  }
  return FRCNN_OK;
}

static bool cnet_fuse() {
  const char* e = getenv("FRCNN_CNET_FUSE");
  return !(e && atoi(e) == 0);
}
static bool gemm_f16_on() {
  static const bool env_on = !(getenv("FRCNN_GEMM_F16") && atoi(getenv("FRCNN_GEMM_F16")) == 0);
  return env_on && get_x3_f16();
}
static int ensure_cnet(frcnn_model* m, int R) {
  for (auto& L : m->cls) {
    size_t n = (size_t)R * L.n * 4;
    FR_TRY(L.lin.ensure(n));
    if (L.bn) { FR_TRY(L.pre.ensure(n)); FR_TRY(L.xhat.ensure(n)); FR_TRY(L.invstd.ensure((size_t)L.n * 4)); }
    FR_TRY(L.post.ensure(n));
    FR_TRY(L.g.ensure(n));
    FR_TRY(L.gin.ensure((size_t)R * L.in * 4));
    if (L.p_drop > 0.f) FR_TRY(L.mask.ensure(n));
    L.x_form = 0;
    for (int role : {1, 2, 4}) if (linear_x_eligible(role, R, L.in, L.n)) L.x_form |= role;
    const size_t Rp = (size_t)linear_x_rows_padded(R);
    if (L.x_form & 1) FR_TRY(L.xp.ensure((size_t)3 * R * L.in * 2));
    if (L.x_form & 2) FR_TRY(L.gp.ensure((size_t)3 * R * L.n * 2));
    if (L.x_form & 4) { FR_TRY(L.xpT.ensure((size_t)3 * L.in * Rp * 2)); FR_TRY(L.gpT.ensure((size_t)3 * L.n * Rp * 2)); }
    if (L.x_form & 7) FR_TRY(L.am.ensure((size_t)5 * AMAX_REC * 4));
  }
  int nc = m->d.class_count + 1;
  int nf = m->cls.empty() ? m->D : m->cls.back().n;
  FR_TRY(m->feat_g.ensure((size_t)R * nf * 4));
  FR_TRY(m->logits.ensure((size_t)R * nc * 4));
  FR_TRY(m->lsm.ensure((size_t)R * nc * 4));
  FR_TRY(m->glog.ensure((size_t)R * nc * 4));
  return FRCNN_OK;
}

int frcnn_cnet_forward(frcnn_model* m, const float* weights, const float* x, int R, int training,
                       const float* const* drop_masks, unsigned long long seed, float* bn_running,
                       float* bbox_out, float* cls_out, void* stream) {
  hipStream_t s = S(stream);
  FR_CHECK(R > 0, "cnet_forward: empty batch");
  FR_TRY(cw_join(m, s));
  FR_TRY(ensure_cnet(m, R));
  m->R = R; m->cnet_x = x; m->training = training;
  const float* w = weights;
  const float* cur = x;
  float* bnr = bn_running;
  for (size_t l = 0; l < m->cls.size(); ++l) {
    ClsLayer& L = m->cls[l];
    GemmFold fold;
    GemmFold* defer = cnet_fuse() ? &fold : nullptr;
    if ((L.x_form & 3) && gemm_f16_on()) {
      float* rw = L.am.f() + 2 * AMAX_REC;
      const bool have = !training && g_static_weights && L.am_w_gen == g_static_gen && L.am_w_of == w;
      if (!have) FR_TRY(tensor_absmax(w + L.w_off, (long)L.n * L.in, rw, s));
      L.am_w_of = w; L.am_w_gen = training ? -1 : g_static_gen;
    } else {
      L.am_w_of = nullptr;
    }
    if ((L.x_form & 1) && gemm_f16_on()) {
      float* rx = L.am.f();
      FR_TRY(tensor_absmax(cur, (long)R * L.in, rx, s));
      FR_TRY(split_planes(cur, R, L.in, L.xp.p, nullptr, s, rx));
      FR_TRY(linear_x_forward(L.xp.p, R, L.in, w + L.w_off, w + L.b_off, L.n, L.lin.f(), s, 0, defer, rx, rx + 2 * AMAX_REC));
    } else if (L.x_form & 1) {
      FR_TRY(split_planes(cur, R, L.in, L.xp.p, nullptr, s));
      FR_TRY(linear_x_forward(L.xp.p, R, L.in, w + L.w_off, w + L.b_off, L.n, L.lin.f(), s, 0, defer));
    } else {
      FR_TRY(gemm_f32(cur, L.in, 1, w + L.w_off, 1, L.in, L.lin.f(), L.n, R, L.n, L.in, OUT_STORE, w + L.b_off, s, 0, defer));
    }
    if (L.bn) FR_CHECK(training || bnr, "cnet_forward: evaluate mode needs bn_running");
    const float* mask = nullptr;
    float inv_keep = 1.f;
    bool draw = false;
    if (training && L.p_drop > 0.f) {
      inv_keep = 1.0f / (1.0f - L.p_drop);
      if (drop_masks && drop_masks[l])
        FR_HIP(hipMemcpyAsync(L.mask.p, drop_masks[l], (size_t)R * L.n * 4, hipMemcpyDeviceToDevice, s));
      else
        draw = true;
      mask = L.mask.f();
    }
    if (defer) {
      FR_TRY(cnet_act_forward(L.lin.f(), fold, R, L.n, L.bn ? w + L.bnw_off : nullptr, L.bn ? w + L.bnb_off : nullptr, L.bn ? bnr : nullptr,
                              training, L.lin.f(), L.xhat.f(), L.invstd.f(), L.pre.f(), w + L.a_off, const_cast<float*>(mask), draw,
                              inv_keep, L.p_drop, seed * 977 + l + 17, L.post.f(), s));
      if (L.bn && bnr) bnr += 2 * L.n;
      cur = L.post.f();
      continue;
    }
    const float* pre = L.lin.f();
    if (L.bn) {
      FR_TRY(bn_forward(L.lin.f(), R, L.n, w + L.bnw_off, w + L.bnb_off, bnr, training, L.xhat.f(), L.invstd.f(),
                        L.pre.f(), s));
      if (bnr) bnr += 2 * L.n;
      pre = L.pre.f();
    }
    if (draw)
      FR_TRY(prelu_dropout_forward_gen(pre, (long)R * L.n, w + L.a_off, L.mask.f(), L.p_drop, seed * 977 + l + 17,
                                       L.post.f(), s));
    else
      FR_TRY(prelu_dropout_forward(pre, (long)R * L.n, w + L.a_off, mask, inv_keep, L.post.f(), s));
    cur = L.post.f();
  }
  const int nf = m->cls.empty() ? m->D : m->cls.back().n;
  const int nc = m->d.class_count + 1;
  if (cnet_fuse() && cnet_heads_fused_eligible(nf, nc)) {
    return cnet_heads_forward(cur, R, nf, w + m->bbox_w_off, w + m->bbox_b_off, w + m->clsw_off, w + m->clsb_off, nc, bbox_out,
                              m->logits.f(), m->lsm.f(), cls_out, s);
  }
  FR_TRY(gemm_f32(cur, nf, 1, w + m->bbox_w_off, 1, nf, bbox_out, 4, R, 4, nf, OUT_STORE, w + m->bbox_b_off, s));
  if (cnet_fuse()) {
    GemmFold fold;
    FR_TRY(gemm_f32(cur, nf, 1, w + m->clsw_off, 1, nf, m->logits.f(), nc, R, nc, nf, OUT_STORE, w + m->clsb_off, s, 0, &fold));
    FR_TRY(log_softmax_rows_fold(m->logits.f(), fold, R, nc, m->lsm.f(), cls_out, s));
    return FRCNN_OK;
  }
  FR_TRY(gemm_f32(cur, nf, 1, w + m->clsw_off, 1, nf, m->logits.f(), nc, R, nc, nf, OUT_STORE, w + m->clsb_off, s));
  FR_TRY(log_softmax_rows(m->logits.f(), R, nc, m->lsm.f(), s));
  FR_HIP(hipMemcpyAsync(cls_out, m->lsm.p, (size_t)R * nc * 4, hipMemcpyDeviceToDevice, s));
  return FRCNN_OK;
}

int frcnn_cnet_backward(frcnn_model* m, const float* weights, const float* g_bbox, const float* g_cls, float* gx,
                        float* grad, void* stream) {
  hipStream_t s = S(stream);
  FR_CHECK(m->R > 0, "cnet_backward: call frcnn_cnet_forward first");
  const int R = m->R;
  const float* w = weights;
  const int nf = m->cls.empty() ? m->D : m->cls.back().n;
  const int nc = m->d.class_count + 1;
  const float* feat = m->cls.empty() ? m->cnet_x : m->cls.back().post.f();
  if (m->frozen_blocks >= (int)m->blocks.size()) gx = nullptr;
  FR_TRY(cw_join(m, s));
  const bool async = g_cnet_wgrad_async && !deterministic();
  if (async && !m->cw) {
    FR_TRY(pool_stream(1, &m->cw));
    FR_HIP(hipEventCreateWithFlags(&m->cw_done, hipEventDisableTiming));
  }
  while (async && m->cw_ev.size() < m->cls.size() + 1) {
    hipEvent_t e;
    FR_HIP(hipEventCreateWithFlags(&e, hipEventDisableTiming));
    m->cw_ev.push_back(e);
  }
  hipStream_t ws = async ? m->cw : s;
  const int wslot = async ? 7 : 0;
  size_t nfork = 0;
  auto fork = [&]() -> int {
    if (!async) return FRCNN_OK;
    FR_HIP(hipEventRecord(m->cw_ev[nfork], s));
    FR_HIP(hipStreamWaitEvent(ws, m->cw_ev[nfork], 0));
    ++nfork;
    return FRCNN_OK;
  };
  bool top_act_done = false;
  if (cnet_fuse() && cnet_heads_fused_eligible(nf, nc)) {
    HeadsPostAct post;
    float* dst = m->feat_g.f();
    if (!m->cls.empty() && !m->cls.back().bn && !deterministic()) {
      ClsLayer& T = m->cls.back();
      const bool drop = m->training && T.p_drop > 0.f;
      post.pre = T.lin.f(); post.mask = drop ? T.mask.f() : nullptr; post.inv_keep = drop ? 1.0f / (1.0f - T.p_drop) : 1.f;
      post.slope = w + T.a_off; post.gslope = grad + T.a_off;
      dst = T.g.f();
      top_act_done = true;
    }
    FR_TRY(cnet_heads_backward(g_bbox, g_cls, m->lsm.f(), R, nf, w + m->bbox_w_off, w + m->clsw_off, nc, m->glog.f(), dst, s,
                               top_act_done ? &post : nullptr));
    FR_TRY(fork());
  } else {
    FR_TRY(log_softmax_backward(g_cls, m->lsm.f(), R, nc, m->glog.f(), s));
    FR_TRY(fork());
    FR_TRY(gemm_f32(g_bbox, 4, 1, w + m->bbox_w_off, nf, 1, m->feat_g.f(), nf, R, nf, 4, OUT_STORE, nullptr, s));
    FR_TRY(gemm_f32(m->glog.f(), nc, 1, w + m->clsw_off, nf, 1, m->feat_g.f(), nf, R, nf, nc, OUT_ADD, nullptr, s));
  }
  FR_TRY(gemm_f32(g_bbox, 1, 4, feat, nf, 1, grad + m->bbox_w_off, nf, 4, nf, R, OUT_ADD, nullptr, ws, wslot));
  FR_TRY(channel_sum_cols(g_bbox, R, 4, grad + m->bbox_b_off, ws));
  FR_TRY(gemm_f32(m->glog.f(), 1, nc, feat, nf, 1, grad + m->clsw_off, nf, nc, nf, R, OUT_ADD, nullptr, ws, wslot));
  FR_TRY(channel_sum_cols(m->glog.f(), R, nc, grad + m->clsb_off, ws));
  const float* g = m->feat_g.f();
  GemmFold gfold;
  for (int l = (int)m->cls.size() - 1; l >= 0; --l) {
    ClsLayer& L = m->cls[l];
    const float* pre = L.bn ? L.pre.f() : L.lin.f();
    const bool drop = m->training && L.p_drop > 0.f;
    if (top_act_done && l == (int)m->cls.size() - 1) {
    } else if (L.bn && cnet_fuse()) {
      FR_TRY(cnet_act_bn_backward(g, gfold, pre, L.xhat.f(), L.invstd.f(), w + L.bnw_off, w + L.a_off, drop ? L.mask.f() : nullptr,
                                  drop ? 1.0f / (1.0f - L.p_drop) : 1.f, R, L.n, m->training, L.g.f(), grad + L.bnw_off,
                                  grad + L.bnb_off, grad + L.a_off, s));
    } else {
      FR_TRY(prelu_dropout_backward(g, pre, (long)R * L.n, w + L.a_off, drop ? L.mask.f() : nullptr,
                                    drop ? 1.0f / (1.0f - L.p_drop) : 1.f, L.g.f(), grad + L.a_off, s));
      if (L.bn)
        FR_TRY(bn_backward(L.g.f(), L.xhat.f(), L.invstd.f(), w + L.bnw_off, R, L.n, m->training, L.g.f(),
                           grad + L.bnw_off, grad + L.bnb_off, s));
    }
    gfold = GemmFold{};
    GemmFold* gdefer = (cnet_fuse() && async && l > 0 && m->cls[l - 1].bn) ? &gfold : nullptr;
    FR_TRY(fork());
    const float* in = l == 0 ? m->cnet_x : m->cls[l - 1].post.f();
    float* gin = l == 0 ? gx : L.gin.f();
    const bool xw = (L.x_form & 4) != 0, xd = (L.x_form & 2) != 0 && gin;
    if (xd && gemm_f16_on() && L.am_w_of == w) {
      float* rg = L.am.f() + AMAX_REC;
      FR_TRY(tensor_absmax(L.g.f(), (long)R * L.n, rg, s));
      FR_TRY(split_planes(L.g.f(), R, L.n, L.gp.p, nullptr, s, rg));
      FR_TRY(linear_x_dgrad(L.gp.p, R, L.n, w + L.w_off, L.in, gin, OUT_STORE, s, 0, gdefer, rg, L.am.f() + 2 * AMAX_REC));
    } else if (xd) {
      FR_TRY(split_planes(L.g.f(), R, L.n, L.gp.p, nullptr, s));
      FR_TRY(linear_x_dgrad(L.gp.p, R, L.n, w + L.w_off, L.in, gin, OUT_STORE, s, 0, gdefer));
    } else if (gin) {
      FR_TRY(gemm_f32(L.g.f(), L.n, 1, w + L.w_off, L.in, 1, gin, L.in, R, L.in, L.n, OUT_STORE, nullptr, s, 0, gdefer));
    }
    static const bool wgrad_f16 = !(getenv("FRCNN_GEMM_WGRAD_F16") && atoi(getenv("FRCNN_GEMM_WGRAD_F16")) == 0);
    if (xw && wgrad_f16 && gemm_f16_on() && L.am.bytes >= (size_t)5 * AMAX_REC * 4) {
      float *rgT = L.am.f() + 3 * AMAX_REC, *rxT = L.am.f() + 4 * AMAX_REC;
      FR_TRY(tensor_absmax(L.g.f(), (long)R * L.n, rgT, ws));
      if ((L.x_form & 1) && L.am_w_of == w) rxT = L.am.f();
      else FR_TRY(tensor_absmax(in, (long)R * L.in, rxT, ws));
      FR_TRY(split_planes(L.g.f(), R, L.n, nullptr, L.gpT.p, ws, rgT));
      FR_TRY(split_planes(in, R, L.in, nullptr, L.xpT.p, ws, rxT));
      FR_TRY(linear_x_wgrad(L.gpT.p, L.xpT.p, R, L.n, L.in, grad + L.w_off, ws, wslot, rgT, rxT));
    } else if (xw) {
      FR_TRY(split_planes(L.g.f(), R, L.n, nullptr, L.gpT.p, ws));
      FR_TRY(split_planes(in, R, L.in, nullptr, L.xpT.p, ws));
      FR_TRY(linear_x_wgrad(L.gpT.p, L.xpT.p, R, L.n, L.in, grad + L.w_off, ws, wslot));
    } else {
      FR_TRY(gemm_f32(L.g.f(), 1, L.n, in, L.in, 1, grad + L.w_off, L.in, L.n, L.in, R, OUT_ADD, nullptr, ws, wslot));
    }
    FR_TRY(channel_sum_cols(L.g.f(), R, L.n, grad + L.b_off, ws));
    g = gin;
  }
  if (m->cls.empty() && gx) FR_HIP(hipMemcpyAsync(gx, g, (size_t)R * m->D * 4, hipMemcpyDeviceToDevice, s));
  if (async) {
    FR_HIP(hipEventRecord(m->cw_done, ws));
    m->cw_pending = true;
  }
  return FRCNN_OK;
}

}
```

### faster-rcnn.torch_amd/csrc/roi.hip

```cpp
#include "kernels.h"
#include "roi_fix.h"

namespace frcnn {

__global__ void roi_pool_forward_kernel(const float* __restrict__ fmap, int C, int H, int W,
                                        const int* __restrict__ wins, int R, int kh, int kw,
                                        float* __restrict__ out, int* __restrict__ idx) {
  const long total = (long)R * C * kh * kw;
  for (long t = (long)blockIdx.x * blockDim.x + threadIdx.x; t < total; t += (long)gridDim.x * blockDim.x) {
    int j = (int)(t % kw);
    long q = t / kw;
    int i = (int)(q % kh);
    q /= kh;
    int c = (int)(q % C);
    int r = (int)(q / C);
    const int* wn = wins + 4 * r;
    const int r0 = wn[0] - 1, c0 = wn[2] - 1;
    const int h = wn[1] - wn[0] + 1, w = wn[3] - wn[2] + 1;
    const int ys = (i * h) / kh, ye = ((i + 1) * h + kh - 1) / kh;
    const int xs = (j * w) / kw, xe = ((j + 1) * w + kw - 1) / kw;
    const float* ip = fmap + (size_t)c * H * W;
    float best = -3.402823466e+38f;
    int bi = -1;
    for (int y = ys; y < ye; ++y)
      for (int x = xs; x < xe; ++x) {
        float v = ip[(size_t)(r0 + y) * W + (c0 + x)];
        if (v > best) { best = v; bi = (r0 + y) * W + (c0 + x); }
      }
    out[t] = best;
    if (idx) idx[t] = bi;
  }
}

__global__ __launch_bounds__(256) void roi_pool_forward_cells_kernel(const float* __restrict__ fmap, int C, int H, int W,
                                                                     const int* __restrict__ wins, int kh, int kw,
                                                                     float* __restrict__ out, int* __restrict__ idx) {
  const int r = blockIdx.x, cells = kh * kw, groups = blockDim.x / cells;
  const int tid = threadIdx.x;
  if (tid >= groups * cells) return;
  const int cg = tid / cells, cell = tid - cg * cells;
  const int i = cell / kw, j = cell - i * kw;
  const int* wn = wins + 4 * r;
  const int r0 = wn[0] - 1, c0 = wn[2] - 1;
  const int h = wn[1] - wn[0] + 1, w = wn[3] - wn[2] + 1;
  const int ys = (i * h) / kh, ye = ((i + 1) * h + kh - 1) / kh;
  const int xs = (j * w) / kw, xe = ((j + 1) * w + kw - 1) / kw;
  const int HW = H * W;
  const int base = (r0 + ys) * W + c0 + xs, nx = xe - xs, ny = ye - ys;
  if (HW >= 4) {
    for (int c = blockIdx.y * groups + cg; c < C; c += gridDim.y * groups) {
      const float* ip = fmap + (size_t)c * HW;
      float best = -3.402823466e+38f;
      int bi = -1;
      for (int y = 0, o = base; y < ny; ++y, o += W)
        for (int x = 0; x < nx; x += 4) {
          const int q = min(o + x, HW - 4);
          float v[4];
          __builtin_memcpy(v, ip + q, 16);
#pragma unroll
          for (int e = 0; e < 4; ++e) {
            const int at = q + e;
            if (at >= o && at < o + nx && v[e] > best) { best = v[e]; bi = at; }
          }
        }
      const size_t t = ((size_t)r * C + c) * cells + cell;
      out[t] = best;
      if (idx) idx[t] = bi;
    }
    return;
  }
  for (int c = blockIdx.y * groups + cg; c < C; c += gridDim.y * groups) {
    const float* ip = fmap + (size_t)c * HW;
    float best = -3.402823466e+38f;
    int bi = -1;
    for (int y = 0, o = base; y < ny; ++y, o += W)
      for (int x = 0; x < nx; ++x) {
        const float v = ip[o + x];
        if (v > best) { best = v; bi = o + x; }
      }
    const size_t t = ((size_t)r * C + c) * cells + cell;
    out[t] = best;
    if (idx) idx[t] = bi;
  }
}

int roi_pool_forward(const float* fmap, int C, int H, int W, const int* wins, int R, int kh, int kw,
                     float* out, int* idx, hipStream_t s) {
  if (R <= 0) return FRCNN_OK;
  long total = (long)R * C * kh * kw;
  if (kh * kw <= 256) {
    const int groups = 256 / (kh * kw);
    const int slices = std::max(1, std::min(cdiv(C, groups), (int)cdivl(4096, R)));
    FR_LAUNCH(KC_ROI, 0, total * 8.0, s, roi_pool_forward_cells_kernel, dim3(R, slices), dim3(256), 0, fmap, C, H, W,
              wins, kh, kw, out, idx);
    FR_LAUNCH_CHECK();
    return FRCNN_OK;
  }
  int grid = (int)std::min<long>(cdivl(total, 256), 4096);
  FR_LAUNCH(KC_ROI, 0, total * 8.0, s, roi_pool_forward_kernel, dim3(grid), dim3(256), 0, fmap, C, H, W,
            wins, R, kh, kw, out, idx);
  FR_LAUNCH_CHECK();
  return FRCNN_OK;
}

__global__ void roi_pool_backward_lds_kernel(float* __restrict__ gmap, int C, int HW, const float* __restrict__ gout,
                                             const int* __restrict__ idx, int R, int cell) {
  extern __shared__ float plane[];
  const int c = blockIdx.x;
  for (int i = threadIdx.x; i < HW; i += blockDim.x) plane[i] = 0.f;
  __syncthreads();
  const long D = (long)C * cell;
  const int total = R * cell;
  for (int e = threadIdx.x; e < total; e += blockDim.x) {
    const int r = e / cell, j = e - r * cell;
    const long t = (long)r * D + (long)c * cell + j;
    const int bi = idx[t];
    const float g = gout[t];
    if (bi >= 0 && g != 0.f) atomicAdd(&plane[bi], g);
  }
  __syncthreads();
  float* gp = gmap + (size_t)c * HW;
  for (int i = threadIdx.x; i < HW; i += blockDim.x) {
    const float v = plane[i];
    if (v != 0.f) gp[i] += v;
  }
}

__global__ void roi_pool_backward_lds_det_kernel(float* __restrict__ gmap, int C, int HW, const float* __restrict__ gout,
                                                 const int* __restrict__ idx, int R, int cell) {
  extern __shared__ unsigned long long fplane[];
  const int c = blockIdx.x;
  for (int i = threadIdx.x; i < HW; i += blockDim.x) fplane[i] = 0ull;
  __syncthreads();
  const long D = (long)C * cell;
  const int total = R * cell;
  for (int e = threadIdx.x; e < total; e += blockDim.x) {
    const int r = e / cell, j = e - r * cell;
    const long t = (long)r * D + (long)c * cell + j;
    const int bi = idx[t];
    const float g = gout[t];
    if (bi >= 0 && g != 0.f) atomicAdd(&fplane[bi], (unsigned long long)roi_to_fix(g));
  }
  __syncthreads();
  float* gp = gmap + (size_t)c * HW;
  for (int i = threadIdx.x; i < HW; i += blockDim.x) {
    const long long v = (long long)fplane[i];
    if (v != 0) gp[i] += (float)((double)v / ROI_FIX_SCALE);
  }
}
__global__ void roi_pool_backward_det_kernel(unsigned long long* __restrict__ fix, int C, long HW,
                                             const float* __restrict__ gout, const int* __restrict__ idx,
                                             long total, int cell) {
  for (long t = (long)blockIdx.x * blockDim.x + threadIdx.x; t < total; t += (long)gridDim.x * blockDim.x) {
    int c = (int)((t / cell) % C);
    int bi = idx[t];
    float g = gout[t];
    if (bi >= 0 && g != 0.f) atomicAdd(fix + (size_t)c * HW + bi, (unsigned long long)roi_to_fix(g));
  }
}
__global__ void roi_fix_apply_kernel(const unsigned long long* __restrict__ fix, long n, float* __restrict__ gmap) {
  for (long t = (long)blockIdx.x * blockDim.x + threadIdx.x; t < n; t += (long)gridDim.x * blockDim.x) {
    const long long v = (long long)fix[t];
    if (v != 0) gmap[t] += (float)((double)v / ROI_FIX_SCALE);
  }
}

int roi_fix_apply(const unsigned long long* fix, long n, float* gmap, hipStream_t s) {
  FR_LAUNCH(KC_ROI, 0, n * 16.0, s, roi_fix_apply_kernel, dim3((int)std::min<long>(cdivl(n, 256), 4096)), dim3(256), 0, fix, n, gmap);
  FR_LAUNCH_CHECK();
  return FRCNN_OK;
}

__global__ void roi_pool_backward_kernel(float* __restrict__ gmap, int C, long HW,
                                         const float* __restrict__ gout, const int* __restrict__ idx,
                                         long total, int cell) {
  for (long t = (long)blockIdx.x * blockDim.x + threadIdx.x; t < total; t += (long)gridDim.x * blockDim.x) {
    int c = (int)((t / cell) % C);
    int bi = idx[t];
    float g = gout[t];
    if (bi >= 0 && g != 0.f) unsafeAtomicAdd(gmap + (size_t)c * HW + bi, g);
  }
}

int roi_pool_backward(float* gmap, int C, int H, int W, const float* gout, const int* idx, int R,
                      int kh, int kw, hipStream_t s) {
  if (R <= 0) return FRCNN_OK;
  long total = (long)R * C * kh * kw;
  if (deterministic()) {
    if ((size_t)H * W * 8 <= 64 * 1024) {
      FR_LAUNCH(KC_ROI, 0, total * 12.0, s, roi_pool_backward_lds_det_kernel, dim3(C), dim3(256), (size_t)H * W * 8, gmap, C,
                H * W, gout, idx, R, kh * kw);
    } else {
      float* ws = nullptr;
      const long n = (long)C * H * W;
      FR_TRY(det_workspace(s, (size_t)n * 2, &ws));
      FR_HIP(hipMemsetAsync(ws, 0, (size_t)n * 8, s));
      int grid = (int)std::min<long>(cdivl(total, 256), 4096);
      FR_LAUNCH(KC_ROI, 0, total * 12.0, s, roi_pool_backward_det_kernel, dim3(grid), dim3(256), 0, (unsigned long long*)ws, C,
                (long)H * W, gout, idx, total, kh * kw);
      FR_LAUNCH_CHECK();
      return roi_fix_apply((const unsigned long long*)ws, n, gmap, s);
    }
    FR_LAUNCH_CHECK();
    return FRCNN_OK;
  }
  if ((size_t)H * W * 4 <= 64 * 1024) {
    FR_LAUNCH(KC_ROI, 0, total * 12.0, s, roi_pool_backward_lds_kernel, dim3(C), dim3(1024), (size_t)H * W * 4, gmap, C,
              H * W, gout, idx, R, kh * kw);
    FR_LAUNCH_CHECK();
    return FRCNN_OK;
  }
  int grid = (int)std::min<long>(cdivl(total, 256), 4096);
  FR_LAUNCH(KC_ROI, 0, total * 12.0, s, roi_pool_backward_kernel, dim3(grid), dim3(256), 0, gmap, C,
            (long)H * W, gout, idx, total, kh * kw);
  FR_LAUNCH_CHECK();
  return FRCNN_OK;
}

}
```

### faster-rcnn.torch_amd/model_utilities.py

```python
import ctypes as C

import numpy as np

from . import _lib
from .tensor import DeviceTensor, ptr, stream_ptr, to_device


class _Node(object):

    def __init__(self, layers):
        self.layers = layers


class _OutNode(object):
    def __init__(self, children):
        self.children = children


class NativeModel(object):

    def __init__(self, cfg, layers, anchor_nets, class_layers):
        d = _lib.ModelDesc()
        d.nblocks = len(layers)
        for i, l in enumerate(layers):
# ... 138 lines not shown
        _lib.call("frcnn_pnet_anchor_loss_begin", nat.h, ptr(nat.weights), ptr(nat.gradient), C.c_void_p(d_idx),
                  C.c_void_p(d_anchor), C.c_void_p(d_roi), C.c_void_p(d_class), npos, nneg, bgclass, ptr(ex_loss),
                  ptr(crtarget), ptr(cctarget), ptr(acc), stream_ptr())

    def anchor_loss_wait(self):
        _lib.call("frcnn_pnet_anchor_loss_wait", self.native.h, stream_ptr())

    def backward_heads_join(self):
        joined = C.c_int(0)
        _lib.call("frcnn_pnet_backward_heads_join", self.native.h, stream_ptr(), C.byref(joined))
        return bool(joined.value)

    def block_param_range(self, b):
        d = self.native.desc
        first = sum(int(d.conv_steps[i]) for i in range(b))
        n = int(d.conv_steps[b])
        t = self.native.param_table
        last = t[3 * (first + n) - 1]
        return int(t[3 * first][0]), int(last[0]) + int(last[1])

    def wait_block_gradients(self, b):
        _lib.call("frcnn_pnet_wait_block_gradients", self.native.h, b + 1, stream_ptr())

    def heads_param_range(self):
        d = self.native.desc
        nconv = sum(int(d.conv_steps[b]) for b in range(d.nblocks))
        return int(self.native.param_table[3 * nconv][0]), int(self.native.pnet_params)

    def parameters(self):
        return _param_views(self.native, 0, self.native.pnet_params)


class ClassificationNet(object):

    def __init__(self, native):
        self.native = native
        self.train = True
        self.drop_masks = None
        self.output = None
        self._bufs = {}
        self._pending = None

    def _buf(self, name, shape):
        need = int(np.prod(shape)) * 4
        b = self._bufs.get(name)
        if b is None or b.nbytes < need:
            b = DeviceTensor.empty((max(need, 256),), np.uint8)
            self._bufs[name] = b
        return DeviceTensor(b.ptr, shape, np.float32, owner=b)

    def cuda(self):
        return self

    def training(self):
        self.train = True

    def evaluate(self):
        self.train = False

    def forward(self, cinput, out=None):
        nat = self.native
        cinput = to_device(cinput)
        R, D = cinput.shape
        nc = nat.desc.class_count + 1
        bbox, cls = out if out is not None else (self._buf("bbox", (R, 4)), self._buf("cls", (R, nc)))
        arr, keep = _mask_ptrs(self.drop_masks, nat.desc.ncls)
        nat.seed += 1
        self._input = cinput
        _lib.call("frcnn_cnet_forward", nat.h, ptr(nat.weights), ptr(cinput), R, 1 if self.train else 0,
                  C.cast(arr, C.c_void_p) if arr is not None else None, nat.seed, ptr(nat.bn_running), ptr(bbox),
                  ptr(cls), stream_ptr())
        self.output = [bbox, cls]
        return self.output

    def backward(self, cinput, grad_outputs):
        nat = self.native
        R, D = self._input.shape
        gx = self._buf("gx", (R, D))
        _lib.call("frcnn_cnet_backward", nat.h, ptr(nat.weights), ptr(grad_outputs[0]), ptr(grad_outputs[1]), ptr(gx),
                  ptr(nat.gradient), stream_ptr())
        self._pending = (self._input, grad_outputs[0], grad_outputs[1])
        return gx

    def join_backward(self):
        _lib.call("frcnn_cnet_backward_join", self.native.h, stream_ptr())
        self._pending = None

    def parameters(self):
        return _param_views(self.native, self.native.pnet_params, self.native.total_params)


def _param_views(native, lo, hi):
    if native.weights is None:
        raise _lib.FrcnnError("parameters() before combine_and_flatten_parameters()")
    ws, gs = [], []
    for off, cnt, kind, aux in native.param_table:
        if lo <= off < hi:
            ws.append(native.weights[off:off + cnt])
            gs.append(native.gradient[off:off + cnt])
    return ws, gs


def create_model(cfg, layers, anchor_nets, class_layers):
    native = NativeModel(cfg, layers, anchor_nets, class_layers)
    return dict(cfg=cfg, layers=layers, anchor_nets=anchor_nets, class_layers=class_layers,
                pnet=ProposalNet(native), cnet=ClassificationNet(native), native=native)
```

### faster-rcnn.torch_amd/objective.py

```python
import ctypes as C
import os
import sys

import numpy as np

from . import _lib
from .Anchors import Anchors
from .Localizer import Localizer
from .Rect import Rect
from .tensor import DeviceTensor, ptr, stream_ptr, to_device


def roi_window(input_rect, localizer, fm_h, fm_w):
    r = localizer.inputToFeatureRect(input_rect)
    r = r.clip(Rect(0, 0, fm_w, fm_h))
    return (int(min(r.minY + 1, r.maxY)), int(r.maxY), int(min(r.minX + 1, r.maxX)), int(r.maxX))


def roi_windows(rects, localizer, fm_h, fm_w):
    r = localizer.inputToFeatureRectBatch(rects)
    minX = np.minimum(np.maximum(r[:, 0], 0), fm_w); minY = np.minimum(np.maximum(r[:, 1], 0), fm_h)
    maxX = np.maximum(np.minimum(r[:, 2], fm_w), 0); maxY = np.maximum(np.minimum(r[:, 3], fm_h), 0)
    return np.stack([np.minimum(minY + 1, maxY), maxY, np.minimum(minX + 1, maxX), maxX], 1).astype(np.int32)

# ... 336 lines not shown
                eager = None
        if eager is not None:
            from .synthetic import clean_examples, output_map_sizes
            x0 = batch[0]
            held0 = prepared.get(id(x0))
            if held0 is not None and held0[0] is x0:
                n_ex = len(held0[1]["p"]) + len(held0[1]["n"])
            else:
                sizes0 = output_map_sizes(model, x0["img"].shape[1], x0["img"].shape[2])
                n_ex = len(clean_examples(x0["positive"], sizes0)) + len(clean_examples(x0["negative"], sizes0))
            eager["gscale"] = (1.0 / n_ex) if n_ex > 0 else 1.0
            eager["done"] = []
            eager["ranges"] = ranges
            us = C.c_void_p()
            _lib.call("frcnn_model_update_stream", native.h, C.byref(us))
            nblk = int(native.desc.nblocks)

            def eager_slice(lo, hi, on, group=None):
                eager["update"](weights, gradient, lo, hi, eager["gscale"], on)
                eager["done"].append((int(lo), int(hi)))
                if group is not None:
                    _lib.call("frcnn_pnet_refresh_packs", native.h, ptr(weights), group, on)
                    eager["groups"].add(group)
            eager["groups"] = set()
            eager["slice"] = eager_slice
        dev_tail = (dev_tail_ok and defer == "fold" and _dist() is not None and getattr(gradient, "is_cuda", False)
                    and ranges is None)
        c4 = None
        if dev_tail:
            from .synthetic import clean_examples, output_map_sizes
            c4 = [0.0, 0.0, 0.0, 0.0]
            for x in batch:
                shp = x["img"].shape
                sizes = output_map_sizes(model, shp[1], shp[2])
                np_, nn_ = len(clean_examples(x["positive"], sizes)), len(clean_examples(x["negative"], sizes))
                c4[0] += np_ + nn_; c4[1] += np_; c4[2] += np_; c4[3] += 1
            init = np.array([0.0, 0.0, c4[0], c4[1], 0.0, 0.0, c4[2], c4[3]], dtype=np.float64)
            hinit, staged = pinned.stage(init.view(np.uint8))
            _lib.call("frcnn_memcpy_h2d", ptr(acc_dev), C.c_void_p(hinit), 64, s)
            staged()
        else:
            acc_dev.zero_()
        for bi, x in enumerate(batch):
            last = bi == len(batch) - 1
            held = prepared.pop(id(x), None)
            prep = held[1] if held is not None and held[0] is x else prepare_examples(x)
            img = to_device(x["img"])
            outputs = pnet.forward(img, async_heads=True)
            if prep["sizes"] != [tuple(o.shape[1:]) for o in outputs[:len(prep["sizes"])]] or prep["fm"] != tuple(outputs[-1].shape[1:]):
                raise _lib.FrcnnError("lossAndGradient: the example tables were packed for other map sizes than this image's")
            p, n = prep["p"], prep["n"]
            delta_outputs = pnet.delta_outputs(zero=True)
            npos, nneg = len(p), len(n)
            E = npos + nneg
            fm = outputs[-1]
            fmC, fmH, fmW = fm.shape
            if E > 0:
                ex_anchor, ex_roi, ex_idx, ex_class, wins, sp, blob = (prep[k] for k in ("ex_anchor", "ex_roi", "ex_idx", "ex_class", "wins", "sp", "blob"))
                dblob = scratch.get("blob", (blob.size,), np.uint8)
                hblob, staged = pinned.stage(blob)
                _lib.call("frcnn_memcpy_h2d", ptr(dblob), C.c_void_p(hblob), blob.nbytes, s)
                staged()
                o = 0
                d_anchor = dblob.ptr + o; o += ex_anchor.nbytes
                d_roi = dblob.ptr + o; o += ex_roi.nbytes
                d_idx = dblob.ptr + o; o += ex_idx.nbytes
                d_class = dblob.ptr + o; o += ex_class.nbytes
                if align:
                    o += -o % 8
                d_wins = dblob.ptr + o; o += wins.nbytes
                for l in range(4):
                    _lib.call("frcnn_pnet_set_sparse_deltas", native.h, l + 1, C.c_void_p(dblob.ptr + o), len(sp[l]))
                    o += sp[l].nbytes
                ex_loss = scratch.get("ex_loss", (E, 2), np.float64)
                crtarget = scratch.get("crtarget", (E, 4))
                cctarget = scratch.get("cctarget", (E,))
                pnet.anchor_loss_begin(d_idx, d_anchor, d_roi, d_class, npos, nneg, bgclass, ex_loss, crtarget,
                                       cctarget, acc_dev)
            if E > 0 and not classification:
                native.seed += 1
                pnet.anchor_loss_wait()
            elif E > 0:
                cinput = scratch.get("cinput", (E, D))
                if align:
                    debug["rects"] = wins
                    _lib.call("frcnn_roi_align_forward", ptr(fm), fmC, fmH, fmW, C.c_void_p(d_wins), None, E, inv_sx, inv_sy,
                              kh, kw, sampling, ptr(cinput), s)
                else:
                    pidx = scratch.get("pidx", (E, D), np.int32)
                    _lib.call("frcnn_roi_pool_forward", ptr(fm), fmC, fmH, fmW, C.c_void_p(d_wins), E, kh, kw,
                              ptr(cinput), ptr(pidx), s)
                coutputs = cnet.forward(cinput)
                crout, ccout = coutputs
                crdelta = scratch.get("crdelta", (E, 4))
                ccdelta = scratch.get("ccdelta", (E, ncls))
                pnet.anchor_loss_wait()
                _lib.call("frcnn_cnet_losses", ptr(crout), ptr(crtarget), ptr(ccout), ptr(cctarget), E, npos, ncls,
                          ptr(crdelta), ptr(ccdelta), C.c_void_p(acc_dev.ptr + 4 * 8), s)
                post_roi_delta = cnet.backward(cinput, [crdelta, ccdelta])
                if not trunk_frozen and align:
                    _lib.call("frcnn_roi_align_backward", ptr(delta_outputs[4]), fmC, fmH, fmW, ptr(post_roi_delta),
                              C.c_void_p(d_wins), None, E, inv_sx, inv_sy, kh, kw, sampling, s)
                elif not trunk_frozen:
                    _lib.call("frcnn_roi_pool_backward", ptr(delta_outputs[4]), fmC, fmH, fmW, ptr(post_roi_delta),
                              ptr(pidx), E, kh, kw, s)
            if E == 0:
                for l in range(4):
                    _lib.call("frcnn_pnet_set_sparse_deltas", native.h, l + 1, None, 0)
            if last and _dist() is not None:
                _lib.call("frcnn_cnet_backward_join", native.h, stream_ptr())
                if classification:
                    pending.append(allreduce_begin(gradient, native.pnet_params, gradient.numel()))
                side = C.c_int(0)
                _lib.call("frcnn_get_option", b"side_stream", C.byref(side))
                if len(batch) == 1 and side.value and proposal:
                    pnet.backward_heads_join()
                    lo, hi = pnet.heads_param_range()
                    pending.append(allreduce_begin(gradient, lo, hi))
            if last and probing:
                _lib.call("frcnn_cnet_backward_join", native.h, stream_ptr())
                _probe_mark("classification net", native.pnet_params, gradient.numel(), "frcnn_cnet_backward_join (its weight-gradient stream)")
                side = C.c_int(0)
                _lib.call("frcnn_get_option", b"side_stream", C.byref(side))
                if len(batch) == 1 and side.value:
                    pnet.backward_heads_join()
                    lo, hi = pnet.heads_param_range()
                    _probe_mark("anchor nets", lo, hi, "frcnn_pnet_backward_heads_join (the anchor nets' streams)")
            if last and defer and _dist() is None and not guarded:
                acc_pin.copy_(acc_t, non_blocking=True)
                acc_event.record()
                early_copy = True
            debug["E"] = E
            pnet.backward(img, delta_outputs)
            if eager is not None:
                _lib.call("frcnn_pnet_wait_backward_begun", native.h, us)
                if classification:
                    eager_slice(native.pnet_params, gradient.numel(), us)
                _lib.call("frcnn_pnet_wait_heads_done", native.h, us)
                lo, hi = pnet.heads_param_range()
                if proposal:
                    eager_slice(lo, hi, us, nblk)
                for b in range(nblk, max(frozen_blocks, 1), -1):
                    _lib.call("frcnn_pnet_wait_block_done", native.h, b, us)
                    lo, hi = pnet.block_param_range(b - 1)
                    eager_slice(lo, hi, us, b - 1)
                _lib.call("frcnn_model_update_join", native.h, stream_ptr())
            if last and _dist() is not None and early_blocks and getattr(gradient, "is_cuda", False):
                if aux_stream[0] is None:
                    aux_stream[0] = torch.cuda.Stream()
                for b in [b for b in early_blocks if b >= frozen_blocks]:
                    lo, hi = pnet.block_param_range(b)
                    with torch.cuda.stream(aux_stream[0]):
                        pnet.wait_block_gradients(b)
                        pending.append(allreduce_begin(gradient, lo, hi))
            if last and probing:
                covered = []
                if early_blocks:
                    if aux_stream[0] is None:
                        aux_stream[0] = torch.cuda.Stream()
                    for b in early_blocks:
                        lo, hi = pnet.block_param_range(b)
                        with torch.cuda.stream(aux_stream[0]):
                            pnet.wait_block_gradients(b)
                            _probe_mark("backbone block %d" % (b + 1), lo, hi, "frcnn_pnet_wait_block_gradients(%d) on an auxiliary stream" % (b + 1))
                        covered.append((lo, hi))
                _probe_mark("backward_end", 0, 0, "")
                lo_rest = 0
                hi_rest = min([c[0] for c in covered] + [pnet.heads_param_range()[0]])
                _probe_mark("rest of the backbone", lo_rest, hi_rest, "end of frcnn_pnet_backward on the caller's stream")
            reg_count += npos
            cls_count += npos + nneg
            creg_count += npos
            ccls_count += 1

        single = _dist() is None
        fold = single and defer == "fold" and cls_count > 0
        if single and cls_count > 0 and not fold:
            _lib.call("frcnn_scale", ptr(gradient), gradient.numel(), 1.0 / cls_count, stream_ptr())
        counts = (cls_count, reg_count, creg_count, ccls_count)
        if not single:
            pending[:] = allreduce_begin_rest(gradient, pending, ranges)
        if dev_tail:
            assert [float(v) for v in (cls_count, reg_count, creg_count, ccls_count)] == c4, "count bookkeeping diverged"
            acc_work = _dist().all_reduce(acc_t, async_op=True)
            for pnd in pending:
                pnd[2].wait()
            acc_work.wait()
            if not guarded:
# ... 124 lines not shown
```

### include/frcnn_hip.h

```cpp
#ifndef FRCNN_HIP_H
#define FRCNN_HIP_H

#include <stddef.h>

#ifdef __cplusplus
extern "C" {
#endif

#define FRCNN_OK 0
#define FRCNN_ERR_ARG 1
#define FRCNN_ERR_HIP 2
#define FRCNN_ERR_STATE 3

int frcnn_version(void);
const char *frcnn_last_error(void);
int frcnn_device_count(int *n);
int frcnn_set_device(int device);
int frcnn_device_name(char *buf_host, int len);
int frcnn_set_option(const char *name, int value);
int frcnn_get_option(const char *name, int *value_host);

int frcnn_malloc(void **ptr_out_host, size_t bytes);
int frcnn_free(void *ptr);
int frcnn_host_alloc(void **ptr_out_host, size_t bytes);
int frcnn_host_free(void *ptr_host);
int frcnn_memcpy_h2d(void *dst, const void *src_host, size_t bytes, void *stream);
int frcnn_memcpy_d2h(void *dst_host, const void *src, size_t bytes, void *stream);
int frcnn_memcpy_d2d(void *dst, const void *src, size_t bytes, void *stream);
int frcnn_stream_sync(void *stream);
int frcnn_zero(void *ptr, size_t bytes, void *stream);
int frcnn_scale(float *x, long long n, float s, void *stream);
int frcnn_add(float *y, const float *x, long long n, void *stream);

#define FRCNN_KC_CONV_IGEMM_K3 0
#define FRCNN_KC_CONV_IGEMM_OTHER 1
#define FRCNN_KC_CONV_WGRAD_K3 2
#define FRCNN_KC_CONV_WGRAD_OTHER 3
#define FRCNN_KC_GEMM 4
#define FRCNN_KC_ELEMWISE 5
#define FRCNN_KC_ROI 6
#define FRCNN_KC_RPN 7
#define FRCNN_KC_NMS 8
#define FRCNN_KC_OPTIM 9
#define FRCNN_KC_IMAGE 10
#define FRCNN_KC_CONV_X3 11
#define FRCNN_KC_CONV_WGRADX 12
#define FRCNN_KC_TOPK 13
#define FRCNN_KC_COUNT 14
int frcnn_prof_enable(int class_mask);
int frcnn_prof_collect(long long *launches_host, double *ms_host, double *flops_host,
                       double *bytes_host);

size_t frcnn_nms_workspace_bytes(int n);
int frcnn_nms_device(const float *boxes, int n, int ncols, float overlap, int key_mode,
                     int key_col, long long *pick, int *count, void *workspace,
                     size_t workspace_bytes, void *stream);
int frcnn_nms_device_classes(const float *boxes, int n, int ncols, float overlap, int key_mode, int key_col,
                             const int *cls, long long *pick, int *count, void *workspace,
                             size_t workspace_bytes, void *stream);
int frcnn_nms_device_n(const float *boxes, int n_cap, const int *n_dev, int ncols, float overlap, int key_mode, int key_col,
                       const int *cls, long long *pick, int *count, void *workspace, size_t workspace_bytes, void *stream);
size_t frcnn_nms_batch_workspace_bytes(int B, int n_cap);
int frcnn_nms_device_batch(const float *boxes, int B, long long row_stride, int n_cap, const int *n_dev, int ncols, float overlap,
                           int key_mode, int key_col, const int *cls, long long *pick, int *count, void *workspace,
                           size_t workspace_bytes, void *stream);
int frcnn_roi_windows(const double *rect, const long long *pick, int k, const int *layers_host, int nlayers, int fmH, int fmW,
                      int *wins, void *stream);
int frcnn_detect_post(const int *cls, const float *conf, const float *bbox, const double *rect, const long long *pick, int R,
                      int bgclass, double min_conf, float *bb, int *kc, int *keep_row, double *r2, int *K_dev, void *stream);
int frcnn_detect_gather(const long long *wpick, const int *nwin_dev, int cap, const int *keep_row, const int *kc,
                        const float *bb, const double *r2, const long long *pick, const float *match_p,
                        const double *match_rect, const int *match_idx, double *rec, void *stream);
int frcnn_detect_gather_batch(const long long *wpick, const int *counts, int B, int row_stride, const int *keep_row,
                              const int *kc, const float *bb, const double *r2, const long long *pick, long long match_stride,
                              const float *match_p, const double *match_rect, const int *match_idx, double *rec, void *stream);
int frcnn_nms_host(const float *boxes_host, int n, int ncols, float overlap, int key_mode,
                   int key_col, long long *pick_host, int *count_host);

int frcnn_conv2d_forward(const float *in, int C, int H, int W, const float *in_slope,
                         const float *in_scale, const float *weight, const float *bias, int O,
                         int k, int pad, float *out, void *stream);
int frcnn_conv2d_backward_input(const float *gout, int O, int Ho, int Wo, const float *weight,
                                int C, int k, int pad, float *gin, int accumulate, void *stream);
int frcnn_conv2d_backward_weight(const float *in, int C, int H, int W, const float *in_slope,
                                 const float *in_scale, const float *gout, int O, int k, int pad,
                                 float *gweight, float *gbias, void *stream);

int frcnn_maxpool_act_forward(const float *x, int C, int H, int W, const float *slope,
                              const float *scale, float *out, unsigned char *idx, void *stream);
int frcnn_maxpool_act_backward(const float *gpool, const unsigned char *idx, const float *x, int C,
                               int H, int W, const float *slope, const float *scale, float *gx,
                               float *gbias, float *gslope, void *stream);
int frcnn_act_forward(const float *x, int C, long long hw, const float *slope, const float *scale,
                      float *y, void *stream);
int frcnn_act_backward(const float *gy, const float *x, int C, long long hw, const float *slope,
                       const float *scale, float *gx, float *gbias, float *gslope, void *stream);

int frcnn_roi_pool_forward(const float *fmap, int C, int H, int W, const int *wins, int R, int kh,
                           int kw, float *out, int *idx, void *stream);
int frcnn_roi_pool_backward(float *gmap, int C, int H, int W, const float *gout, const int *idx,
                            int R, int kh, int kw, void *stream);

int frcnn_roi_align_forward(const float *fmap, int C, int H, int W, const double *rect, const long long *pick, int R,
                            double inv_sx, double inv_sy, int kh, int kw, int g, float *out, void *stream);
int frcnn_roi_align_backward(float *gmap, int C, int H, int W, const float *gout, const double *rect, const long long *pick,
                             int R, double inv_sx, double inv_sy, int kh, int kw, int g, void *stream);

size_t frcnn_rpn_scan_workspace_bytes(const int *H_host, const int *W_host);
int frcnn_rpn_scan(const float *const *maps_host, const int *H_host, const int *W_host,
                   const float *anchor_w, const float *anchor_h, double img_w, double img_h,
                   double p_threshold, int cap, float *match_p, int *match_idx,
                   double *match_rect, float *match_box, int *count, void *workspace,
                   size_t workspace_bytes, void *stream);
size_t frcnn_rpn_scan_batch_workspace_bytes(const int *H_host, const int *W_host, int B);
int frcnn_rpn_scan_batch(const float *const *maps_host, const int *H_host, const int *W_host, int B, long long slot_stride,
                         const float *anchor_w, const float *anchor_h, double img_w, double img_h, double p_threshold,
                         int cap, float *match_p, int *match_idx, double *match_rect, float *match_box, int *count,
                         void *workspace, size_t workspace_bytes, void *stream);

size_t frcnn_topk_select_workspace_bytes(int B, int n_cap);
int frcnn_topk_select(const float *score, int B, long long stride, int n_cap, const int *n_dev, int K, int *sel_row,
                      long long sel_stride, int *k_dev, void *workspace, size_t workspace_bytes, void *stream);
int frcnn_rpn_gather_rows(const float *match_p, const int *match_idx, const double *match_rect, const float *match_box, int B,
                          long long src_stride, int src_rows, const int *sel_row, long long sel_stride, const int *k_dev,
                          int k_cap, float *dst_p, int *dst_idx, double *dst_rect, float *dst_box, float *box5, int *row,
                          long long dst_stride, void *stream);

int frcnn_rpn_loss(const float *const *maps_host, float *const *deltas_host, const int *H_host,
                   const int *W_host, const int *ex_idx, const double *ex_anchor,
                   const double *ex_roi, const int *ex_class, int npos, int nneg, int bgclass,
                   double *ex_loss, float *crtarget, float *cctarget, void *stream);

int frcnn_loss_accumulate(const double *ex_loss, int E, double *acc, void *stream);

int frcnn_linear_forward(const float *x, int R, int I, const float *weight, const float *bias,
                         int O, float *y, void *stream);
int frcnn_linear_backward(const float *x, const float *gy, int R, int I, const float *weight,
                          int O, float *gx, float *gweight, float *gbias, void *stream);

int frcnn_rmsprop(float *x, const float *g, float *m, long long n, float lr, float alpha,
                  float eps, void *stream);
int frcnn_scale_rmsprop(float *x, float *g, float gscale, float *m, long long n, float lr, float alpha,
                        float eps, void *stream);
int frcnn_scale_rmsprop_dev(float *x, float *g, const double *gcount_dev, float *m, long long n, float lr,
                            float alpha, float eps, void *stream);
int frcnn_scale_rmsprop_slice(float *x, float *g, float gscale, float *m, long long lo, long long hi, float lr,
                              float alpha, float eps, void *stream);

int frcnn_sgd(float *x, float *g, float *v, long long n, float gscale, const double *gcount_dev, float clr, float wd,
              float mom, float one_minus_damp, int nesterov, int first, void *stream);
int frcnn_sgd_slice(float *x, float *g, float *v, long long lo, long long hi, float gscale, float clr, float wd, float mom,
                    float one_minus_damp, int nesterov, int first, void *stream);
int frcnn_nag(float *x, float *g, float *v, long long n, float gscale, const double *gcount_dev, float clr, float wd,
              float mom, int first, void *stream);
int frcnn_nag_slice(float *x, float *g, float *v, long long lo, long long hi, float gscale, float clr, float wd, float mom,
                    int first, void *stream);
int frcnn_scale_rmsprop_slice_dev(float *x, float *g, const double *gcount_dev, float *m, long long lo, long long hi,
                                  float lr, float alpha, float eps, void *stream);
int frcnn_sgd_slice_dev(float *x, float *g, float *v, long long lo, long long hi, const double *gcount_dev, float clr,
                        float wd, float mom, float one_minus_damp, int nesterov, int first, void *stream);
int frcnn_nag_slice_dev(float *x, float *g, float *v, long long lo, long long hi, const double *gcount_dev, float clr,
                        float wd, float mom, int first, void *stream);

size_t frcnn_grad_clip_workspace_bytes(long long n);
int frcnn_grad_clip(float *g, long long n, const long long *ranges_host, int nranges, double divisor,
                    const double *divisor_dev, double clip_norm, double *record_dev, void *workspace,
                    size_t workspace_bytes, void *stream);

int frcnn_nag_lookahead(float *x, const float *v, long long n, float mom, void *stream);
int frcnn_nag_lookahead_slice(float *x, const float *v, long long lo, long long hi, float mom, void *stream);

typedef struct {
  int nblocks;
  int filters[8], ksize[8], pad[8], conv_steps[8];
  float dropout[8];
  int nheads;
  int head_k[8], head_n[8], head_input[8];
  int ncls;
  int cls_n[8], cls_bn[8];
  float cls_dropout[8];
  int class_count;
  int kh, kw;
} frcnn_model_desc;

typedef struct frcnn_model frcnn_model;

int frcnn_model_create(const frcnn_model_desc *desc_host, frcnn_model **out_host);
int frcnn_model_destroy(frcnn_model *);
int frcnn_model_param_count(const frcnn_model *, long long *total_host, long long *pnet_host);
int frcnn_model_param_table(const frcnn_model *, long long *table_host, int cap, int *n_host);
int frcnn_model_localizer_layers(const frcnn_model *, int output_index, int *layers_host, int cap,
                                 int *n_host);
int frcnn_model_set_trainable(frcnn_model *, int frozen_blocks, int heads, int cnet);
int frcnn_model_get_trainable(const frcnn_model *, int *frozen_blocks_host, int *heads_host, int *cnet_host);

int frcnn_pnet_forward(frcnn_model *, const float *weights, const float *img, int H, int W,
                       int training, const float *const *drop_masks_host, unsigned long long seed,
                       void *stream);
int frcnn_pnet_forward_async_heads(frcnn_model *, const float *weights, const float *img, int H, int W,
                                   const float *const *drop_masks_host, unsigned long long seed,
                                   void *stream);
int frcnn_pnet_output(frcnn_model *, int i, float **ptr_host, int *C_host, int *H_host,
                      int *W_host);
int frcnn_model_debug_buffer(frcnn_model *, int kind, int index, void **ptr_host, long long *bytes_host);
int frcnn_pnet_delta(frcnn_model *, int i, float **ptr_host);
int frcnn_pnet_zero_deltas(frcnn_model *, void *stream);
int frcnn_pnet_set_sparse_deltas(frcnn_model *, int head, const int *positions, int count);
int frcnn_pnet_backward_heads_begin(frcnn_model *, const float *weights, float *grad, void *stream);
int frcnn_pnet_anchor_loss_begin(frcnn_model *, const float *weights, float *grad, const int *ex_idx,
                                 const double *ex_anchor, const double *ex_roi, const int *ex_class,
                                 int npos, int nneg, int bgclass, double *ex_loss, float *crtarget,
                                 float *cctarget, double *acc, void *stream);
int frcnn_pnet_anchor_loss_wait(frcnn_model *, void *stream);
int frcnn_pnet_backward_heads_join(frcnn_model *, void *stream, int *joined_host);
int frcnn_pnet_backward(frcnn_model *, const float *weights, float *grad, void *stream);

int frcnn_pnet_wait_block_gradients(frcnn_model *, int block, void *stream);

int frcnn_model_update_stream(frcnn_model *, void **stream_host);
int frcnn_model_update_fork(frcnn_model *, void *stream);
int frcnn_model_update_join(frcnn_model *, void *stream);
int frcnn_pnet_wait_backward_begun(frcnn_model *, void *stream);
int frcnn_pnet_wait_heads_done(frcnn_model *, void *stream);
int frcnn_pnet_wait_block_done(frcnn_model *, int block, void *stream);
int frcnn_pnet_refresh_packs(frcnn_model *, const float *weights, int group, void *stream);
int frcnn_pnet_invalidate_packs(frcnn_model *);

int frcnn_cnet_forward(frcnn_model *, const float *weights, const float *x, int R, int training,
                       const float *const *drop_masks_host, unsigned long long seed,
                       float *bn_running, float *bbox_out, float *cls_out, void *stream);
int frcnn_cnet_backward_join(frcnn_model *, void *stream);
int frcnn_cnet_backward(frcnn_model *, const float *weights, const float *g_bbox,
                        const float *g_cls, float *gx, float *grad, void *stream);
int frcnn_cnet_losses(float *crout, const float *crtarget, const float *ccout,
                      const float *cctarget, int R, int npos, int ncls, float *crdelta,
                      float *ccdelta, double *loss2, void *stream);
int frcnn_cnet_decode(const float *cls_out, int R, int ncls, int *cls, float *conf, void *stream);

int frcnn_image_rgb2yuv(const float *rgb, float *yuv, int H, int W, void *stream);
int frcnn_image_rgb2hsv(const float *rgb, float *hsv, int H, int W, void *stream);
int frcnn_image_rgb2lab(const float *rgb, float *lab, int H, int W, void *stream);
int frcnn_image_scale(const float *src, int C, int H, int W, float *dst, int dH, int dW, float *tmp,
                      int rgb2yuv, void *stream);
int frcnn_image_scale_u8(const unsigned char *src_hwc, int H, int W, float *dst, int dH, int dW,
                         float *tmp, int rgb2yuv, void *stream);
int frcnn_image_crop_flip(const float *src, int C, int H, int W, int x0, int y0, int w, int h, int hflip,
                          int vflip, float *dst, void *stream);
size_t frcnn_image_normalize_workspace_bytes(int C);
int frcnn_image_normalize(float *img, int C, int H, int W, int centering, int scaling, void *workspace,
                          size_t workspace_bytes, void *stream);
int frcnn_image_contrastive_norm(const float *in, int H, int W, const float *kernel_host, int K,
                                 float threshold, float *out, float *tmp, void *stream);

typedef struct frcnn_anchors frcnn_anchors;
int frcnn_anchors_create(const float *w_tab_host, const float *h_tab_host, const double *cx_host,
                         const double *cy_host, int nscales, int width, frcnn_anchors **out_host);
int frcnn_anchors_destroy(frcnn_anchors *);
int frcnn_anchors_assemble(frcnn_anchors *, const double *rois_host, int nroi, double img_w, double img_h,
                           double pos_thr, double neg_thr, int best_match, int nearby_aversion,
                           int negatives, unsigned int *mt_state_host, int *mt_index_host, int *ex_host,
                           double *ex_rect_host, int cap, int *npos_host, int *nneg_host);

#define FRCNN_COMM_ID_BYTES 128
typedef struct frcnn_comm frcnn_comm;
int frcnn_comm_get_unique_id(void *id_host);
int frcnn_comm_exchange_id_file(const char *path, int rank, void *id_host, int timeout_ms);
int frcnn_comm_init_rank(frcnn_comm **out_host, int nranks, int rank, const void *id_host);
int frcnn_comm_init_rank_timeout(frcnn_comm **out_host, int nranks, int rank, const void *id_host, int timeout_ms);
int frcnn_comm_init_rank_file(frcnn_comm **out_host, int nranks, int rank, const char *path, int timeout_ms);
int frcnn_comm_destroy(frcnn_comm *);
int frcnn_comm_info(const frcnn_comm *, int *nranks_host, int *rank_host);
int frcnn_comm_query(const frcnn_comm *, int *count_host, int *user_rank_host, int *device_host);
int frcnn_allreduce_f32(frcnn_comm *, float *buf, long long n, void *stream);
int frcnn_allreduce_f64(frcnn_comm *, double *buf, long long n, void *stream);
int frcnn_broadcast_f32(frcnn_comm *, float *buf, long long n, int root, void *stream);

#ifdef __cplusplus
}
#endif
#endif
```

Before: 499.2.

## Fuse ROI pooling with classifier net and fold magnitude records into producers

Adds pooled entry points that run ROI max-pooling inside the classification net's forward and backward. The pooling kernel writes the absolute-max record for the first fp16-split linear layer, so the separate tensor_absmax pass on the pooled input is skipped. In backward, the ROI pool scatter reads split-K GEMM slabs directly instead of a folded gradient, and the activation/BN backward kernels emit amax records as a by-product. This trims kernel launches and full-tensor passes, at the cost of more plumbing and a per-block reduction added to several kernels.

```diff
diff --git a/faster-rcnn.torch_amd/_lib.py b/faster-rcnn.torch_amd/_lib.py
--- a/faster-rcnn.torch_amd/_lib.py
+++ b/faster-rcnn.torch_amd/_lib.py
@@ -74,6 +74,8 @@
     "frcnn_act_backward": ([vp, vp, C.c_int, C.c_longlong, vp, vp, vp, vp, vp, vp], C.c_int),
     "frcnn_roi_pool_forward": ([vp, C.c_int, C.c_int, C.c_int, vp, C.c_int, C.c_int, C.c_int, vp, vp, vp], C.c_int),
     "frcnn_roi_pool_backward": ([vp, C.c_int, C.c_int, C.c_int, vp, vp, C.c_int, C.c_int, C.c_int, vp], C.c_int),
+    "frcnn_roi_pool_forward_rec": ([vp, C.c_int, C.c_int, C.c_int, vp, C.c_int, C.c_int, C.c_int, vp, vp, vp, vp], C.c_int),
+    "frcnn_roi_pool_backward_slabs": ([vp, C.c_int, C.c_int, C.c_int, vp, C.c_int, vp, C.c_int, C.c_int, C.c_int, vp], C.c_int),
     "frcnn_roi_align_forward": ([vp, C.c_int, C.c_int, C.c_int, vp, vp, C.c_int, C.c_double, C.c_double, C.c_int, C.c_int, C.c_int, vp,
                                  vp], C.c_int),
     "frcnn_roi_align_backward": ([vp, C.c_int, C.c_int, C.c_int, vp, vp, vp, C.c_int, C.c_double, C.c_double, C.c_int, C.c_int, C.c_int,
@@ -134,6 +136,9 @@
     "frcnn_pnet_wait_block_gradients": ([vp, C.c_int, vp], C.c_int),
     "frcnn_cnet_forward": ([vp, vp, vp, C.c_int, C.c_int, vp, C.c_ulonglong, vp, vp, vp, vp], C.c_int),
     "frcnn_cnet_backward": ([vp, vp, vp, vp, vp, vp, vp], C.c_int),
+    "frcnn_cnet_forward_pooled": ([vp, vp, vp, C.c_int, C.c_int, C.c_int, vp, C.c_int, C.c_int, C.c_int, vp, vp, C.c_int, vp,
+                                   C.c_ulonglong, vp, vp, vp, vp], C.c_int),
+    "frcnn_cnet_backward_pooled": ([vp, vp, vp, vp, vp, vp, C.c_int, C.c_int, C.c_int, vp, C.c_int, C.c_int, vp], C.c_int),
     "frcnn_cnet_backward_join": ([vp, vp], C.c_int),
     "frcnn_cnet_losses": ([vp, vp, vp, vp, C.c_int, C.c_int, C.c_int, vp, vp, vp, vp], C.c_int),
     "frcnn_cnet_decode": ([vp, C.c_int, C.c_int, vp, vp, vp], C.c_int),
diff --git a/faster-rcnn.torch_amd/csrc/amax.h b/faster-rcnn.torch_amd/csrc/amax.h
--- a/faster-rcnn.torch_amd/csrc/amax.h
+++ b/faster-rcnn.torch_amd/csrc/amax.h
@@ -19,6 +19,20 @@
   }
 }
 
+__device__ __forceinline__ void amax_store_block_at(float m, float* rec, int tid, int nthreads, int entry, int count) {
+  __shared__ float amax_part_at[16];
+#pragma unroll
+  for (int o = 32; o > 0; o >>= 1) m = fmaxf(m, __shfl_xor(m, o));
+  if ((tid & 63) == 0) amax_part_at[tid >> 6] = m;
+  __syncthreads();
+  if (tid == 0) {
+    const int nw = (nthreads + 63) >> 6;
+    for (int i = 1; i < nw; ++i) m = fmaxf(m, amax_part_at[i]);
+    rec[1 + entry] = m;
+    if (entry == 0) rec[0] = __builtin_bit_cast(float, count);
+  }
+}
+
 __device__ __forceinline__ float amax_load_block(const float* __restrict__ rec) {
   __shared__ float amax_all[16];
   const int n = __builtin_bit_cast(int, rec[0]);
diff --git a/faster-rcnn.torch_amd/csrc/api.cpp b/faster-rcnn.torch_amd/csrc/api.cpp
--- a/faster-rcnn.torch_amd/csrc/api.cpp
+++ b/faster-rcnn.torch_amd/csrc/api.cpp
@@ -347,6 +347,18 @@
 int frcnn_roi_pool_backward(float* gmap, int C, int H, int W, const float* gout, const int* idx, int R, int kh,
                             int kw, void* stream) {
   return roi_pool_backward(gmap, C, H, W, gout, idx, R, kh, kw, S(stream));
+}
+int frcnn_roi_pool_forward_rec(const float* fmap, int C, int H, int W, const int* wins, int R, int kh, int kw,
+                               float* out, int* idx, float* rec, void* stream) {
+  FR_CHECK(rec != nullptr, "frcnn_roi_pool_forward_rec: NULL record");
+  return roi_pool_forward(fmap, C, H, W, wins, R, kh, kw, out, idx, S(stream), rec);
+}
+int frcnn_roi_pool_backward_slabs(float* gmap, int C, int H, int W, const float* slabs, int nsplit, const int* idx, int R,
+                                  int kh, int kw, void* stream) {
+  FR_CHECK(slabs && nsplit >= 0, "frcnn_roi_pool_backward_slabs: %d slabs at %p", nsplit, (const void*)slabs);
+  GemmFold src;
+  src.slab = slabs; src.nSplit = nsplit;
+  return roi_pool_backward(gmap, C, H, W, slabs, idx, R, kh, kw, S(stream), &src);
 }
 
 static int roi_align_check(const char* who, const void* map, int C, int H, int W, const void* rows, const double* rect, int kh, int kw,
diff --git a/faster-rcnn.torch_amd/csrc/cnet.hip b/faster-rcnn.torch_amd/csrc/cnet.hip
--- a/faster-rcnn.torch_amd/csrc/cnet.hip
+++ b/faster-rcnn.torch_amd/csrc/cnet.hip
@@ -1,4 +1,5 @@
 #include "kernels.h"
+#include "amax.h"
 
 namespace frcnn {
 
@@ -276,7 +277,7 @@
                                                                     const float* __restrict__ invstd, const float* __restrict__ gamma,
                                                                     const float* slope, const float* __restrict__ mask, float inv_keep,
                                                                     int R, int n, int training, float* __restrict__ gx, float* ggamma,
-                                                                    float* gbeta, float* gslope, float* part) {
+                                                                    float* gbeta, float* gslope, float* part, float* rec) {
   __shared__ double sh[FB_RG * FB_CB];
   __shared__ float shs[16];
   const int tx = threadIdx.x, ty = threadIdx.y;
@@ -325,36 +326,41 @@
       if (part) part[blockIdx.x] = t; else unsafeAtomicAdd(gslope, t);
     }
   }
-  if (!ok) return;
-  if (ty == 0) {
-    ggamma[j] = (float)((double)ggamma[j] + sgx);
-    gbeta[j] = (float)((double)gbeta[j] + sg);
-  }
-  const double is = invstd[j], gm = gamma[j];
-  auto second = [&](size_t idx, double g, double xhv) {
-    const double v = training ? (g - sg / R - xhv * sgx / R) * gm * is : g * gm * is;
-    gx[idx] = (float)v;
-  };
-  if (keep) {
-#pragma unroll
-    for (int i = 0; i < FB_KEEP; ++i)
-      if (ty + i * FB_RG < R) second((size_t)(ty + i * FB_RG) * n + j, tv[i], xh[i]);
-  } else {
-    for (int r = ty; r < R; r += FB_RG) {
-      const size_t idx = (size_t)r * n + j;
-      second(idx, gx[idx], xhat[idx]);
-    }
-  }
+  float am = 0.f;
+  if (ok) {
+    if (ty == 0) {
+      ggamma[j] = (float)((double)ggamma[j] + sgx);
+      gbeta[j] = (float)((double)gbeta[j] + sg);
+    }
+    const double is = invstd[j], gm = gamma[j];
+    auto second = [&](size_t idx, double g, double xhv) {
+      const double v = training ? (g - sg / R - xhv * sgx / R) * gm * is : g * gm * is;
+      gx[idx] = (float)v;
+      am = fmaxf(am, fabsf((float)v));
+    };
+    if (keep) {
+#pragma unroll
+      for (int i = 0; i < FB_KEEP; ++i)
+        if (ty + i * FB_RG < R) second((size_t)(ty + i * FB_RG) * n + j, tv[i], xh[i]);
+    } else {
+      for (int r = ty; r < R; r += FB_RG) {
+        const size_t idx = (size_t)r * n + j;
+        second(idx, gx[idx], xhat[idx]);
+      }
+    }
+  }
+  if (rec) amax_store_block_at(am, rec, ty * FB_CB + tx, FB_CB * FB_RG, blockIdx.x, gridDim.x);
 }
 __global__ void slope_fold_kernel(const float* __restrict__ part, int n, float* gslope);
 int cnet_act_bn_backward(const float* gy, GemmFold src, const float* pre, const float* xhat, const float* invstd,
                          const float* gamma, const float* slope, const float* mask, float inv_keep, int R, int n, int training,
-                         float* gx, float* ggamma, float* gbeta, float* gslope, hipStream_t s) {
+                         float* gx, float* ggamma, float* gbeta, float* gslope, hipStream_t s, float* rec) {
   const int grid = cdiv(n, FB_CB);
+  FR_CHECK(!rec || grid <= AMAX_MAX_BLOCKS, "cnet_act_bn_backward: %d blocks do not fit a magnitude record", grid);
   float* part = nullptr;
   if (deterministic()) FR_TRY(det_workspace(s, (size_t)grid, &part));
   FR_LAUNCH(KC_ELEMWISE, 0, (double)R * n * 28.0, s, cnet_act_bn_backward_kernel, dim3(grid), dim3(FB_CB, FB_RG), 0, gy, src, pre, xhat,
-            invstd, gamma, slope, mask, inv_keep, R, n, training, gx, ggamma, gbeta, gslope, part);
+            invstd, gamma, slope, mask, inv_keep, R, n, training, gx, ggamma, gbeta, gslope, part, rec);
   if (part) FR_LAUNCH(KC_ELEMWISE, 0, grid * 4.0, s, slope_fold_kernel, dim3(1), dim3(1), 0, (const float*)part, grid, gslope);
   FR_LAUNCH_CHECK();
   return FRCNN_OK;
@@ -397,10 +403,11 @@
 
 __global__ void prelu_dropout_backward_kernel(const float* __restrict__ gy, const float* __restrict__ x, long n,
                                               const float* slope, const float* __restrict__ mask,
-                                              float inv_keep, float* __restrict__ gx, float* gslope, float* part) {
+                                              float inv_keep, float* __restrict__ gx, float* gslope, float* part,
+                                              float* rec) {
   __shared__ float sh[4];
   const float a = *slope;
-  float sa = 0.f;
+  float sa = 0.f, am = 0.f;
   for (long i = (long)blockIdx.x * blockDim.x + threadIdx.x; i < n; i += (long)gridDim.x * blockDim.x) {
     float g = gy[i];
     if (mask) g = g * (mask[i] * inv_keep);
@@ -408,7 +415,9 @@
     float r = g;
     if (!(xv > 0.f)) { r = a * g; sa += xv * g; }
     gx[i] = r;
-  }
+    am = fmaxf(am, fabsf(r));
+  }
+  if (rec) amax_store_block(am, rec);
 #pragma unroll
   for (int o = 32; o > 0; o >>= 1) sa += __shfl_down(sa, o, 64);
   if ((threadIdx.x & 63) == 0) sh[threadIdx.x >> 6] = sa;
@@ -425,12 +434,12 @@
   *gslope += v;
 }
 int prelu_dropout_backward(const float* gy, const float* x, long n, const float* slope,
-                           const float* mask, float inv_keep, float* gx, float* gslope, hipStream_t s) {
+                           const float* mask, float inv_keep, float* gx, float* gslope, hipStream_t s, float* rec) {
   int grid = (int)std::min<long>(std::max<long>(1, cdivl(n, 256)), 256);
   float* part = nullptr;
   if (deterministic()) FR_TRY(det_workspace(s, (size_t)grid, &part));
   FR_LAUNCH(KC_ELEMWISE, 0, n * 16.0, s, prelu_dropout_backward_kernel, dim3(grid), dim3(256), 0, gy, x, n,
-            slope, mask, inv_keep, gx, gslope, part);
+            slope, mask, inv_keep, gx, gslope, part, rec);
   if (part) FR_LAUNCH(KC_ELEMWISE, 0, grid * 4.0, s, slope_fold_kernel, dim3(1), dim3(1), 0, (const float*)part, grid, gslope);
   FR_LAUNCH_CHECK();
   return FRCNN_OK;
@@ -553,6 +562,7 @@
   extern __shared__ float wt[];
   __shared__ float shs[4];
   const float pa = post.pre ? *post.slope : 1.f;
+  float am = 0.f;
   float sa = 0.f;
   const int no = 4 + nc;
   for (int k = threadIdx.x; k < nf; k += 256) {
@@ -594,9 +604,11 @@
         if (!(xv > 0.f)) { sa += xv * g; g = pa * g; }
       }
       gfeat[(size_t)r * nf + k] = g;
+      am = fmaxf(am, fabsf(g));
     }
     __builtin_amdgcn_wave_barrier();
   }
+  if (post.rec) amax_store_block(am, post.rec);
   if (post.pre) {
 #pragma unroll
     for (int o = 32; o > 0; o >>= 1) sa += __shfl_down(sa, o, 64);
diff --git a/faster-rcnn.torch_amd/csrc/kernels.h b/faster-rcnn.torch_amd/csrc/kernels.h
--- a/faster-rcnn.torch_amd/csrc/kernels.h
+++ b/faster-rcnn.torch_amd/csrc/kernels.h
@@ -169,9 +169,9 @@
 
 
 int roi_pool_forward(const float* fmap, int C, int H, int W, const int* wins, int R, int kh, int kw,
-                     float* out, int* idx, hipStream_t s);
+                     float* out, int* idx, hipStream_t s, float* rec = nullptr);
 int roi_pool_backward(float* gmap, int C, int H, int W, const float* gout, const int* idx, int R,
-                      int kh, int kw, hipStream_t s);
+                      int kh, int kw, hipStream_t s, const GemmFold* src = nullptr);
 
 int roi_align_forward(const float* fmap, int C, int H, int W, const double* rect, const long long* pick, int R, double inv_sx,
                       double inv_sy, int kh, int kw, int g, float* out, hipStream_t s);
@@ -230,13 +230,14 @@
 int prelu_dropout_forward_gen(const float* x, long n, const float* slope, float* mask_out, float p,
                               unsigned long long seed, float* y, hipStream_t s);
 int prelu_dropout_backward(const float* gy, const float* x, long n, const float* slope,
-                           const float* mask, float inv_keep, float* gx, float* gslope, hipStream_t s);
+                           const float* mask, float inv_keep, float* gx, float* gslope, hipStream_t s,
+                           float* rec = nullptr);
 int cnet_act_forward(const float* x, GemmFold src, int R, int n, const float* gamma, const float* beta, float* running,
                      int training, float* lin, float* xhat, float* invstd, float* pre, const float* slope, float* mask, bool gen,
                      float inv_keep, float p, unsigned long long seed, float* post, hipStream_t s);
 int cnet_act_bn_backward(const float* gy, GemmFold src, const float* pre, const float* xhat, const float* invstd,
                          const float* gamma, const float* slope, const float* mask, float inv_keep, int R, int n, int training,
-                         float* gx, float* ggamma, float* gbeta, float* gslope, hipStream_t s);
+                         float* gx, float* ggamma, float* gbeta, float* gslope, hipStream_t s, float* rec = nullptr);
 bool cnet_heads_fused_eligible(int nf, int nc);
 int cnet_heads_forward(const float* x, int R, int nf, const float* Wb, const float* bb, const float* Wc, const float* bc, int nc,
                        float* bbox_out, float* logits, float* lsm, float* cls_out, hipStream_t s);
@@ -246,6 +247,7 @@
   float inv_keep = 1.f;
   const float* slope = nullptr;
   float* gslope = nullptr;
+  float* rec = nullptr;
 };
 int cnet_heads_backward(const float* g_bbox, const float* g_cls, const float* lsm, int R, int nf, const float* Wb, const float* Wc,
                         int nc, float* glog, float* gfeat, hipStream_t s, const HeadsPostAct* post = nullptr);
diff --git a/faster-rcnn.torch_amd/csrc/net.cpp b/faster-rcnn.torch_amd/csrc/net.cpp
--- a/faster-rcnn.torch_amd/csrc/net.cpp
+++ b/faster-rcnn.torch_amd/csrc/net.cpp
@@ -178,6 +178,7 @@
   int R = 0, D = 0;
   const float* cnet_x = nullptr;
   DevBuf feat_g, logits, lsm, glog, gtmp;
+  DevBuf gx_pooled;
   std::vector<std::array<long long, 4>> table;
 };
 
@@ -1089,6 +1090,11 @@
       FR_CHECK(index >= 0 && index < (int)m->cls.size() && m->R > 0, "debug_buffer: classification layer %d (after frcnn_cnet_forward)", index);
       const ClsLayer& L = m->cls[index]; b = L.bn ? &L.pre : &L.lin; n = (size_t)m->R * L.n * 4;
     } break;
+    case 5: {
+      FR_CHECK(index >= 0 && index < (int)m->cls.size() && m->R > 0, "debug_buffer: classification layer %d (after frcnn_cnet_forward)", index);
+      const ClsLayer& L = m->cls[index]; b = &L.am; n = (size_t)5 * AMAX_REC * 4;
+      FR_CHECK((L.x_form & 7) != 0, "debug_buffer: classification layer %d keeps no magnitude records at this size", index);
+    } break;
     default: FR_CHECK(false, "debug_buffer: unknown kind %d", kind);
   }
   FR_CHECK(b->p && b->bytes >= n, "debug_buffer: buffer not allocated yet");
@@ -1694,13 +1700,9 @@
   return FRCNN_OK;
 }
 
-int frcnn_cnet_forward(frcnn_model* m, const float* weights, const float* x, int R, int training,
-                       const float* const* drop_masks, unsigned long long seed, float* bn_running,
-                       float* bbox_out, float* cls_out, void* stream) {
-  hipStream_t s = S(stream);
-  FR_CHECK(R > 0, "cnet_forward: empty batch");
-  FR_TRY(cw_join(m, s));
-  FR_TRY(ensure_cnet(m, R));
+static int cnet_forward_run(frcnn_model* m, const float* weights, const float* x, int R, int training,
+                            const float* const* drop_masks, unsigned long long seed, float* bn_running,
+                            float* bbox_out, float* cls_out, hipStream_t s, bool x_rec) {
   m->R = R; m->cnet_x = x; m->training = training;
   const float* w = weights;
   const float* cur = x;
@@ -1719,7 +1721,7 @@
     }
     if ((L.x_form & 1) && gemm_f16_on()) {
       float* rx = L.am.f();
-      FR_TRY(tensor_absmax(cur, (long)R * L.in, rx, s));
+      if (!(x_rec && l == 0)) FR_TRY(tensor_absmax(cur, (long)R * L.in, rx, s));
       FR_TRY(split_planes(cur, R, L.in, L.xp.p, nullptr, s, rx));
       FR_TRY(linear_x_forward(L.xp.p, R, L.in, w + L.w_off, w + L.b_off, L.n, L.lin.f(), s, 0, defer, rx, rx + 2 * AMAX_REC));
     } else if (L.x_form & 1) {
@@ -1781,15 +1783,43 @@
   return FRCNN_OK;
 }
 
-int frcnn_cnet_backward(frcnn_model* m, const float* weights, const float* g_bbox, const float* g_cls, float* gx,
-                        float* grad, void* stream) {
+int frcnn_cnet_forward(frcnn_model* m, const float* weights, const float* x, int R, int training,
+                       const float* const* drop_masks, unsigned long long seed, float* bn_running,
+                       float* bbox_out, float* cls_out, void* stream) {
   hipStream_t s = S(stream);
+  FR_CHECK(R > 0, "cnet_forward: empty batch");
+  FR_TRY(cw_join(m, s));
+  FR_TRY(ensure_cnet(m, R));
+  return cnet_forward_run(m, weights, x, R, training, drop_masks, seed, bn_running, bbox_out, cls_out, s, false);
+}
+
+int frcnn_cnet_forward_pooled(frcnn_model* m, const float* weights, const float* fmap, int C, int H, int W, const int* wins, int R,
+                              int kh, int kw, float* x_out, int* idx_out, int training, const float* const* drop_masks,
+                              unsigned long long seed, float* bn_running, float* bbox_out, float* cls_out, void* stream) {
+  hipStream_t s = S(stream);
+  FR_CHECK(m && weights && fmap && wins && x_out && bbox_out && cls_out, "cnet_forward_pooled: NULL argument");
+  FR_CHECK(R > 0, "cnet_forward_pooled: empty batch");
+  FR_CHECK(C >= 1 && H >= 1 && W >= 1 && kh >= 1 && kw >= 1 && (long)C * kh * kw == m->D,
+           "cnet_forward_pooled: %d channels pooled to %d x %d are not the net's %d inputs", C, kh, kw, m->D);
+  FR_TRY(cw_join(m, s));
+  FR_TRY(ensure_cnet(m, R));
+  float* rec = (!m->cls.empty() && (m->cls[0].x_form & 1) && gemm_f16_on()) ? m->cls[0].am.f() : nullptr;
+  FR_TRY(roi_pool_forward(fmap, C, H, W, wins, R, kh, kw, x_out, idx_out, s, rec));
+  return cnet_forward_run(m, weights, x_out, R, training, drop_masks, seed, bn_running, bbox_out, cls_out, s, rec != nullptr);
+}
+
+static int cnet_backward_run(frcnn_model* m, const float* weights, const float* g_bbox, const float* g_cls, float* gx,
+                             float* grad, hipStream_t s, GemmFold* gx_fold) {
+  if (gx_fold) *gx_fold = GemmFold{};
   FR_CHECK(m->R > 0, "cnet_backward: call frcnn_cnet_forward first");
   const int R = m->R;
   const float* w = weights;
   const int nf = m->cls.empty() ? m->D : m->cls.back().n;
   const int nc = m->d.class_count + 1;
   const float* feat = m->cls.empty() ? m->cnet_x : m->cls.back().post.f();
+  auto g_rec = [&](ClsLayer& L) -> float* {
+    return ((L.x_form & 6) && gemm_f16_on() && L.am.bytes >= (size_t)5 * AMAX_REC * 4) ? L.am.f() + AMAX_REC : nullptr;
+  };
   if (m->frozen_blocks >= (int)m->blocks.size()) gx = nullptr;
   FR_TRY(cw_join(m, s));
   const bool async = g_cnet_wgrad_async && !deterministic();
@@ -1821,6 +1851,7 @@
       const bool drop = m->training && T.p_drop > 0.f;
       post.pre = T.lin.f(); post.mask = drop ? T.mask.f() : nullptr; post.inv_keep = drop ? 1.0f / (1.0f - T.p_drop) : 1.f;
       post.slope = w + T.a_off; post.gslope = grad + T.a_off;
+      post.rec = g_rec(T);
       dst = T.g.f();
       top_act_done = true;
     }
@@ -1838,32 +1869,39 @@
   FR_TRY(gemm_f32(m->glog.f(), 1, nc, feat, nf, 1, grad + m->clsw_off, nf, nc, nf, R, OUT_ADD, nullptr, ws, wslot));
   FR_TRY(channel_sum_cols(m->glog.f(), R, nc, grad + m->clsb_off, ws));
   const float* g = m->feat_g.f();
+  bool top_rec = false;
+  if (top_act_done) top_rec = g_rec(m->cls.back()) != nullptr;
   GemmFold gfold;
   for (int l = (int)m->cls.size() - 1; l >= 0; --l) {
     ClsLayer& L = m->cls[l];
     const float* pre = L.bn ? L.pre.f() : L.lin.f();
     const bool drop = m->training && L.p_drop > 0.f;
+    bool have_rg = false;
     if (top_act_done && l == (int)m->cls.size() - 1) {
+      have_rg = top_rec;
     } else if (L.bn && cnet_fuse()) {
       FR_TRY(cnet_act_bn_backward(g, gfold, pre, L.xhat.f(), L.invstd.f(), w + L.bnw_off, w + L.a_off, drop ? L.mask.f() : nullptr,
                                   drop ? 1.0f / (1.0f - L.p_drop) : 1.f, R, L.n, m->training, L.g.f(), grad + L.bnw_off,
-                                  grad + L.bnb_off, grad + L.a_off, s));
+                                  grad + L.bnb_off, grad + L.a_off, s, g_rec(L)));
+      have_rg = g_rec(L) != nullptr;
     } else {
       FR_TRY(prelu_dropout_backward(g, pre, (long)R * L.n, w + L.a_off, drop ? L.mask.f() : nullptr,
-                                    drop ? 1.0f / (1.0f - L.p_drop) : 1.f, L.g.f(), grad + L.a_off, s));
+                                    drop ? 1.0f / (1.0f - L.p_drop) : 1.f, L.g.f(), grad + L.a_off, s, L.bn ? nullptr : g_rec(L)));
+      have_rg = !L.bn && g_rec(L) != nullptr;
       if (L.bn)
         FR_TRY(bn_backward(L.g.f(), L.xhat.f(), L.invstd.f(), w + L.bnw_off, R, L.n, m->training, L.g.f(),
                            grad + L.bnw_off, grad + L.bnb_off, s));
     }
     gfold = GemmFold{};
     GemmFold* gdefer = (cnet_fuse() && async && l > 0 && m->cls[l - 1].bn) ? &gfold : nullptr;
+    if (l == 0 && gx_fold && cnet_fuse() && async) gdefer = gx_fold;
     FR_TRY(fork());
     const float* in = l == 0 ? m->cnet_x : m->cls[l - 1].post.f();
     float* gin = l == 0 ? gx : L.gin.f();
     const bool xw = (L.x_form & 4) != 0, xd = (L.x_form & 2) != 0 && gin;
     if (xd && gemm_f16_on() && L.am_w_of == w) {
       float* rg = L.am.f() + AMAX_REC;
-      FR_TRY(tensor_absmax(L.g.f(), (long)R * L.n, rg, s));
+      if (!have_rg) FR_TRY(tensor_absmax(L.g.f(), (long)R * L.n, rg, s));
       FR_TRY(split_planes(L.g.f(), R, L.n, L.gp.p, nullptr, s, rg));
       FR_TRY(linear_x_dgrad(L.gp.p, R, L.n, w + L.w_off, L.in, gin, OUT_STORE, s, 0, gdefer, rg, L.am.f() + 2 * AMAX_REC));
     } else if (xd) {
@@ -1875,7 +1913,8 @@
     static const bool wgrad_f16 = !(getenv("FRCNN_GEMM_WGRAD_F16") && atoi(getenv("FRCNN_GEMM_WGRAD_F16")) == 0);
     if (xw && wgrad_f16 && gemm_f16_on() && L.am.bytes >= (size_t)5 * AMAX_REC * 4) {
       float *rgT = L.am.f() + 3 * AMAX_REC, *rxT = L.am.f() + 4 * AMAX_REC;
-      FR_TRY(tensor_absmax(L.g.f(), (long)R * L.n, rgT, ws));
+      if (have_rg) rgT = L.am.f() + AMAX_REC;
+      else FR_TRY(tensor_absmax(L.g.f(), (long)R * L.n, rgT, ws));
       if ((L.x_form & 1) && L.am_w_of == w) rxT = L.am.f();
       else FR_TRY(tensor_absmax(in, (long)R * L.in, rxT, ws));
       FR_TRY(split_planes(L.g.f(), R, L.n, nullptr, L.gpT.p, ws, rgT));
@@ -1899,4 +1938,35 @@
   return FRCNN_OK;
 }
 
-}
+int frcnn_cnet_backward(frcnn_model* m, const float* weights, const float* g_bbox, const float* g_cls, float* gx,
+                        float* grad, void* stream) {
+  return cnet_backward_run(m, weights, g_bbox, g_cls, gx, grad, S(stream), nullptr);
+}
+
+int frcnn_cnet_backward_pooled(frcnn_model* m, const float* weights, const float* g_bbox, const float* g_cls, float* grad,
+                               float* gmap, int C, int H, int W, const int* idx, int kh, int kw, void* stream) {
+  hipStream_t s = S(stream);
+  FR_CHECK(m && weights && g_bbox && g_cls && grad && gmap && idx, "cnet_backward_pooled: NULL argument");
+  FR_CHECK(m->R > 0, "cnet_backward_pooled: call frcnn_cnet_forward_pooled first");
+  FR_CHECK(C >= 1 && H >= 1 && W >= 1 && kh >= 1 && kw >= 1 && (long)C * kh * kw == m->D,
+           "cnet_backward_pooled: %d channels pooled to %d x %d are not the net's %d inputs", C, kh, kw, m->D);
+  const int R = m->R;
+  if (m->frozen_blocks >= (int)m->blocks.size())
+    return cnet_backward_run(m, weights, g_bbox, g_cls, nullptr, grad, s, nullptr);
+  float* gx = nullptr;
+  if (m->cls.empty()) {
+    FR_TRY(m->gx_pooled.ensure((size_t)R * m->D * 4));
+    gx = m->gx_pooled.f();
+  } else {
+    gx = m->cls[0].gin.f();
+  }
+  if (deterministic() || m->cls.empty()) {
+    FR_TRY(cnet_backward_run(m, weights, g_bbox, g_cls, gx, grad, s, nullptr));
+    return roi_pool_backward(gmap, C, H, W, gx, idx, R, kh, kw, s);
+  }
+  GemmFold fold;
+  FR_TRY(cnet_backward_run(m, weights, g_bbox, g_cls, gx, grad, s, &fold));
+  return roi_pool_backward(gmap, C, H, W, gx, idx, R, kh, kw, s, &fold);
+}
+
+}
diff --git a/faster-rcnn.torch_amd/csrc/roi.hip b/faster-rcnn.torch_amd/csrc/roi.hip
--- a/faster-rcnn.torch_amd/csrc/roi.hip
+++ b/faster-rcnn.torch_amd/csrc/roi.hip
@@ -1,4 +1,5 @@
 #include "kernels.h"
+#include "amax.h"
 #include "roi_fix.h"
 
 namespace frcnn {
@@ -32,78 +33,97 @@
   }
 }
 
+template <bool REC>
 __global__ __launch_bounds__(256) void roi_pool_forward_cells_kernel(const float* __restrict__ fmap, int C, int H, int W,
                                                                      const int* __restrict__ wins, int kh, int kw,
-                                                                     float* __restrict__ out, int* __restrict__ idx) {
+                                                                     float* __restrict__ out, int* __restrict__ idx,
+                                                                     float* __restrict__ rec) {
   const int r = blockIdx.x, cells = kh * kw, groups = blockDim.x / cells;
   const int tid = threadIdx.x;
-  if (tid >= groups * cells) return;
-  const int cg = tid / cells, cell = tid - cg * cells;
-  const int i = cell / kw, j = cell - i * kw;
-  const int* wn = wins + 4 * r;
-  const int r0 = wn[0] - 1, c0 = wn[2] - 1;
-  const int h = wn[1] - wn[0] + 1, w = wn[3] - wn[2] + 1;
-  const int ys = (i * h) / kh, ye = ((i + 1) * h + kh - 1) / kh;
-  const int xs = (j * w) / kw, xe = ((j + 1) * w + kw - 1) / kw;
-  const int HW = H * W;
-  const int base = (r0 + ys) * W + c0 + xs, nx = xe - xs, ny = ye - ys;
-  if (HW >= 4) {
-    for (int c = blockIdx.y * groups + cg; c < C; c += gridDim.y * groups) {
-      const float* ip = fmap + (size_t)c * HW;
-      float best = -3.402823466e+38f;
-      int bi = -1;
-      for (int y = 0, o = base; y < ny; ++y, o += W)
-        for (int x = 0; x < nx; x += 4) {
-          const int q = min(o + x, HW - 4);
-          float v[4];
-          __builtin_memcpy(v, ip + q, 16);
+  float am = 0.f;
+  if (tid < groups * cells) {
+    const int cg = tid / cells, cell = tid - cg * cells;
+    const int i = cell / kw, j = cell - i * kw;
+    const int* wn = wins + 4 * r;
+    const int r0 = wn[0] - 1, c0 = wn[2] - 1;
+    const int h = wn[1] - wn[0] + 1, w = wn[3] - wn[2] + 1;
+    const int ys = (i * h) / kh, ye = ((i + 1) * h + kh - 1) / kh;
+    const int xs = (j * w) / kw, xe = ((j + 1) * w + kw - 1) / kw;
+    const int HW = H * W;
+    const int base = (r0 + ys) * W + c0 + xs, nx = xe - xs, ny = ye - ys;
+    if (HW >= 4) {
+      for (int c = blockIdx.y * groups + cg; c < C; c += gridDim.y * groups) {
+        const float* ip = fmap + (size_t)c * HW;
+        float best = -3.402823466e+38f;
+        int bi = -1;
+        for (int y = 0, o = base; y < ny; ++y, o += W)
+          for (int x = 0; x < nx; x += 4) {
+            const int q = min(o + x, HW - 4);
+            float v[4];
+            __builtin_memcpy(v, ip + q, 16);
 #pragma unroll
-          for (int e = 0; e < 4; ++e) {
-            const int at = q + e;
-            if (at >= o && at < o + nx && v[e] > best) { best = v[e]; bi = at; }
+            for (int e = 0; e < 4; ++e) {
+              const int at = q + e;
+              if (at >= o && at < o + nx && v[e] > best) { best = v[e]; bi = at; }
+            }
           }
-        }
-      const size_t t = ((size_t)r * C + c) * cells + cell;
-      out[t] = best;
-      if (idx) idx[t] = bi;
+        const size_t t = ((size_t)r * C + c) * cells + cell;
+        out[t] = best;
+        if (idx) idx[t] = bi;
+        if (REC) am = fmaxf(am, fabsf(best));
+      }
+    } else {
+      for (int c = blockIdx.y * groups + cg; c < C; c += gridDim.y * groups) {
+        const float* ip = fmap + (size_t)c * HW;
+        float best = -3.402823466e+38f;
+        int bi = -1;
+        for (int y = 0, o = base; y < ny; ++y, o += W)
+          for (int x = 0; x < nx; ++x) {
+            const float v = ip[o + x];
+            if (v > best) { best = v; bi = o + x; }
+          }
+        const size_t t = ((size_t)r * C + c) * cells + cell;
+        out[t] = best;
+        if (idx) idx[t] = bi;
+        if (REC) am = fmaxf(am, fabsf(best));
+      }
     }
-    return;
-  }
-  for (int c = blockIdx.y * groups + cg; c < C; c += gridDim.y * groups) {
-    const float* ip = fmap + (size_t)c * HW;
-    float best = -3.402823466e+38f;
-    int bi = -1;
-    for (int y = 0, o = base; y < ny; ++y, o += W)
-      for (int x = 0; x < nx; ++x) {
-        const float v = ip[o + x];
-        if (v > best) { best = v; bi = o + x; }
-      }
-    const size_t t = ((size_t)r * C + c) * cells + cell;
-    out[t] = best;
-    if (idx) idx[t] = bi;
-  }
+  }
+  if (REC) amax_store_block_at(am, rec, tid, blockDim.x, blockIdx.y * gridDim.x + blockIdx.x, gridDim.x * gridDim.y);
 }
 
 int roi_pool_forward(const float* fmap, int C, int H, int W, const int* wins, int R, int kh, int kw,
-                     float* out, int* idx, hipStream_t s) {
+                     float* out, int* idx, hipStream_t s, float* rec) {
   if (R <= 0) return FRCNN_OK;
   long total = (long)R * C * kh * kw;
   if (kh * kw <= 256) {
     const int groups = 256 / (kh * kw);
     const int slices = std::max(1, std::min(cdiv(C, groups), (int)cdivl(4096, R)));
-    FR_LAUNCH(KC_ROI, 0, total * 8.0, s, roi_pool_forward_cells_kernel, dim3(R, slices), dim3(256), 0, fmap, C, H, W,
-              wins, kh, kw, out, idx);
+    if (rec && (long)R * slices <= AMAX_MAX_BLOCKS) {
+      FR_LAUNCH(KC_ROI, 0, total * 8.0, s, roi_pool_forward_cells_kernel<true>, dim3(R, slices), dim3(256), 0, fmap, C, H, W,
+                wins, kh, kw, out, idx, rec);
+      FR_LAUNCH_CHECK();
+      return FRCNN_OK;
+    }
+    FR_LAUNCH(KC_ROI, 0, total * 8.0, s, roi_pool_forward_cells_kernel<false>, dim3(R, slices), dim3(256), 0, fmap, C, H, W,
+              wins, kh, kw, out, idx, (float*)nullptr);
     FR_LAUNCH_CHECK();
-    return FRCNN_OK;
+    return rec ? tensor_absmax(out, total, rec, s) : FRCNN_OK;
   }
   int grid = (int)std::min<long>(cdivl(total, 256), 4096);
   FR_LAUNCH(KC_ROI, 0, total * 8.0, s, roi_pool_forward_kernel, dim3(grid), dim3(256), 0, fmap, C, H, W,
             wins, R, kh, kw, out, idx);
   FR_LAUNCH_CHECK();
-  return FRCNN_OK;
-}
-
-__global__ void roi_pool_backward_lds_kernel(float* __restrict__ gmap, int C, int HW, const float* __restrict__ gout,
+  return rec ? tensor_absmax(out, total, rec, s) : FRCNN_OK;
+}
+
+__device__ __forceinline__ float roi_gout_value(const float* __restrict__ gout, int nSplit, size_t slab, size_t t) {
+  if (nSplit == 0) return gout[t];
+  float v = 0.f;
+  for (int sI = 0; sI < nSplit; ++sI) v += gout[(size_t)sI * slab + t];
+  return v;
+}
+__global__ void roi_pool_backward_lds_kernel(float* __restrict__ gmap, int C, int HW, const float* __restrict__ gout, int nSplit,
                                              const int* __restrict__ idx, int R, int cell) {
   extern __shared__ float plane[];
   const int c = blockIdx.x;
@@ -111,11 +131,12 @@
   __syncthreads();
   const long D = (long)C * cell;
   const int total = R * cell;
+  const size_t slab = (size_t)R * D;
   for (int e = threadIdx.x; e < total; e += blockDim.x) {
     const int r = e / cell, j = e - r * cell;
     const long t = (long)r * D + (long)c * cell + j;
     const int bi = idx[t];
-    const float g = gout[t];
+    const float g = roi_gout_value(gout, nSplit, slab, (size_t)t);
     if (bi >= 0 && g != 0.f) atomicAdd(&plane[bi], g);
   }
   __syncthreads();
@@ -172,21 +193,26 @@
 }
 
 __global__ void roi_pool_backward_kernel(float* __restrict__ gmap, int C, long HW,
-                                         const float* __restrict__ gout, const int* __restrict__ idx,
+                                         const float* __restrict__ gout, int nSplit, const int* __restrict__ idx,
                                          long total, int cell) {
   for (long t = (long)blockIdx.x * blockDim.x + threadIdx.x; t < total; t += (long)gridDim.x * blockDim.x) {
     int c = (int)((t / cell) % C);
     int bi = idx[t];
-    float g = gout[t];
+    float g = roi_gout_value(gout, nSplit, (size_t)total, (size_t)t);
     if (bi >= 0 && g != 0.f) unsafeAtomicAdd(gmap + (size_t)c * HW + bi, g);
   }
 }
 
 int roi_pool_backward(float* gmap, int C, int H, int W, const float* gout, const int* idx, int R,
-                      int kh, int kw, hipStream_t s) {
+                      int kh, int kw, hipStream_t s, const GemmFold* src) {
   if (R <= 0) return FRCNN_OK;
   long total = (long)R * C * kh * kw;
+  const int nSplit = src ? src->nSplit : 0;
+  FR_CHECK(nSplit == 0 || (src->slab && !src->bias), "roi_pool_backward: a deferred product needs its slabs and has no bias");
+  if (nSplit) gout = src->slab;
+  FR_CHECK(gout != nullptr, "roi_pool_backward: NULL gradient");
   if (deterministic()) {
+    FR_CHECK(nSplit == 0, "roi_pool_backward: deterministic mode takes a folded gradient");
     if ((size_t)H * W * 8 <= 64 * 1024) {
       FR_LAUNCH(KC_ROI, 0, total * 12.0, s, roi_pool_backward_lds_det_kernel, dim3(C), dim3(256), (size_t)H * W * 8, gmap, C,
                 H * W, gout, idx, R, kh * kw);
@@ -206,13 +232,13 @@
   }
   if ((size_t)H * W * 4 <= 64 * 1024) {
     FR_LAUNCH(KC_ROI, 0, total * 12.0, s, roi_pool_backward_lds_kernel, dim3(C), dim3(1024), (size_t)H * W * 4, gmap, C,
-              H * W, gout, idx, R, kh * kw);
+              H * W, gout, nSplit, idx, R, kh * kw);
     FR_LAUNCH_CHECK();
     return FRCNN_OK;
   }
   int grid = (int)std::min<long>(cdivl(total, 256), 4096);
   FR_LAUNCH(KC_ROI, 0, total * 12.0, s, roi_pool_backward_kernel, dim3(grid), dim3(256), 0, gmap, C,
-            (long)H * W, gout, idx, total, kh * kw);
+            (long)H * W, gout, nSplit, idx, total, kh * kw);
   FR_LAUNCH_CHECK();
   return FRCNN_OK;
 }
diff --git a/faster-rcnn.torch_amd/model_utilities.py b/faster-rcnn.torch_amd/model_utilities.py
--- a/faster-rcnn.torch_amd/model_utilities.py
+++ b/faster-rcnn.torch_amd/model_utilities.py
@@ -244,6 +244,27 @@
         self._pending = (self._input, grad_outputs[0], grad_outputs[1])
         return gx
 
+    def forward_pooled(self, fmap, fm_shape, wins_ptr, R, kh, kw, cinput, pidx, out=None):
+        nat = self.native
+        fmC, fmH, fmW = fm_shape
+        nc = nat.desc.class_count + 1
+        bbox, cls = out if out is not None else (self._buf("bbox", (R, 4)), self._buf("cls", (R, nc)))
+        arr, keep = _mask_ptrs(self.drop_masks, nat.desc.ncls)
+        nat.seed += 1
+        self._input = cinput
+        _lib.call("frcnn_cnet_forward_pooled", nat.h, ptr(nat.weights), ptr(fmap), fmC, fmH, fmW, wins_ptr, R, kh, kw,
+                  ptr(cinput), ptr(pidx), 1 if self.train else 0, C.cast(arr, C.c_void_p) if arr is not None else None,
+                  nat.seed, ptr(nat.bn_running), ptr(bbox), ptr(cls), stream_ptr())
+        self.output = [bbox, cls]
+        return self.output
+
+    def backward_pooled(self, grad_outputs, gmap, fm_shape, pidx, kh, kw):
+        nat = self.native
+        fmC, fmH, fmW = fm_shape
+        _lib.call("frcnn_cnet_backward_pooled", nat.h, ptr(nat.weights), ptr(grad_outputs[0]), ptr(grad_outputs[1]),
+                  ptr(nat.gradient), ptr(gmap), fmC, fmH, fmW, ptr(pidx), kh, kw, stream_ptr())
+        self._pending = (self._input, grad_outputs[0], grad_outputs[1], pidx)
+
     def join_backward(self):
         _lib.call("frcnn_cnet_backward_join", self.native.h, stream_ptr())
         self._pending = None
diff --git a/faster-rcnn.torch_amd/objective.py b/faster-rcnn.torch_amd/objective.py
--- a/faster-rcnn.torch_amd/objective.py
+++ b/faster-rcnn.torch_amd/objective.py
@@ -442,7 +442,11 @@
                 pnet.anchor_loss_wait()
             elif E > 0:
                 cinput = scratch.get("cinput", (E, D))
-                if align:
+                pooled = not align and not trunk_frozen
+                if pooled:
+                    pidx = scratch.get("pidx", (E, D), np.int32)
+                    coutputs = cnet.forward_pooled(fm, (fmC, fmH, fmW), C.c_void_p(d_wins), E, kh, kw, cinput, pidx)
+                elif align:
                     debug["rects"] = wins
                     _lib.call("frcnn_roi_align_forward", ptr(fm), fmC, fmH, fmW, C.c_void_p(d_wins), None, E, inv_sx, inv_sy,
                               kh, kw, sampling, ptr(cinput), s)
@@ -450,20 +454,21 @@
                     pidx = scratch.get("pidx", (E, D), np.int32)
                     _lib.call("frcnn_roi_pool_forward", ptr(fm), fmC, fmH, fmW, C.c_void_p(d_wins), E, kh, kw,
                               ptr(cinput), ptr(pidx), s)
-                coutputs = cnet.forward(cinput)
+                if not pooled:
+                    coutputs = cnet.forward(cinput)
                 crout, ccout = coutputs
                 crdelta = scratch.get("crdelta", (E, 4))
                 ccdelta = scratch.get("ccdelta", (E, ncls))
                 pnet.anchor_loss_wait()
                 _lib.call("frcnn_cnet_losses", ptr(crout), ptr(crtarget), ptr(ccout), ptr(cctarget), E, npos, ncls,
                           ptr(crdelta), ptr(ccdelta), C.c_void_p(acc_dev.ptr + 4 * 8), s)
-                post_roi_delta = cnet.backward(cinput, [crdelta, ccdelta])
-                if not trunk_frozen and align:
-                    _lib.call("frcnn_roi_align_backward", ptr(delta_outputs[4]), fmC, fmH, fmW, ptr(post_roi_delta),
-                              C.c_void_p(d_wins), None, E, inv_sx, inv_sy, kh, kw, sampling, s)
-                elif not trunk_frozen:
-                    _lib.call("frcnn_roi_pool_backward", ptr(delta_outputs[4]), fmC, fmH, fmW, ptr(post_roi_delta),
-                              ptr(pidx), E, kh, kw, s)
+                if pooled:
+                    cnet.backward_pooled([crdelta, ccdelta], delta_outputs[4], (fmC, fmH, fmW), pidx, kh, kw)
+                else:
+                    post_roi_delta = cnet.backward(cinput, [crdelta, ccdelta])
+                    if align and not trunk_frozen:
+                        _lib.call("frcnn_roi_align_backward", ptr(delta_outputs[4]), fmC, fmH, fmW, ptr(post_roi_delta),
+                                  C.c_void_p(d_wins), None, E, inv_sx, inv_sy, kh, kw, sampling, s)
             if E == 0:
                 for l in range(4):
                     _lib.call("frcnn_pnet_set_sparse_deltas", native.h, l + 1, None, 0)
diff --git a/include/frcnn_hip.h b/include/frcnn_hip.h
--- a/include/frcnn_hip.h
+++ b/include/frcnn_hip.h
@@ -100,6 +100,10 @@
                            int kw, float *out, int *idx, void *stream);
 int frcnn_roi_pool_backward(float *gmap, int C, int H, int W, const float *gout, const int *idx,
                             int R, int kh, int kw, void *stream);
+int frcnn_roi_pool_forward_rec(const float *fmap, int C, int H, int W, const int *wins, int R, int kh,
+                               int kw, float *out, int *idx, float *rec, void *stream);
+int frcnn_roi_pool_backward_slabs(float *gmap, int C, int H, int W, const float *slabs, int nsplit,
+                                  const int *idx, int R, int kh, int kw, void *stream);
 
 int frcnn_roi_align_forward(const float *fmap, int C, int H, int W, const double *rect, const long long *pick, int R,
                             double inv_sx, double inv_sy, int kh, int kw, int g, float *out, void *stream);
@@ -232,6 +236,13 @@
 int frcnn_cnet_backward_join(frcnn_model *, void *stream);
 int frcnn_cnet_backward(frcnn_model *, const float *weights, const float *g_bbox,
                         const float *g_cls, float *gx, float *grad, void *stream);
+int frcnn_cnet_forward_pooled(frcnn_model *, const float *weights, const float *fmap, int C, int H, int W,
+                              const int *wins, int R, int kh, int kw, float *x_out, int *idx_out, int training,
+                              const float *const *drop_masks_host, unsigned long long seed, float *bn_running,
+                              float *bbox_out, float *cls_out, void *stream);
+int frcnn_cnet_backward_pooled(frcnn_model *, const float *weights, const float *g_bbox, const float *g_cls,
+                               float *grad, float *gmap, int C, int H, int W, const int *idx, int kh, int kw,
+                               void *stream);
 int frcnn_cnet_losses(float *crout, const float *crtarget, const float *ccout,
                       const float *cctarget, int R, int npos, int ncls, float *crdelta,
                       float *ccdelta, double *loss2, void *stream);
```

New measurement: 501.0, median of 4. No clear change (+0.4%).
